# SegataLab/metamlst

Measured on AMD Instinct MI355X. Metric: Mreads/s aligned+ST-typed, metamlstDB_2022; ST concordance vs CPU ref, higher is better.
Workload: dtype int32

## Files before the change

include/mlst_debug.h:

```cpp
#ifndef MLST_DEBUG_H
#define MLST_DEBUG_H

#include "mlst.h"

#ifdef __cplusplus
extern "C" {
#endif

int mlst_selftest_inflate(const uint8_t* in, uint64_t n_in, uint8_t* out, uint64_t cap, uint64_t* produced);

int mlst_selftest_inflate_device(mlst_handle* h, const uint8_t* data, uint64_t n_bytes, uint8_t* out, uint64_t cap, uint64_t* produced, double* kernel_ms);

int mlst_debug_inflate_paths(mlst_handle* h, uint64_t* n_blocks, uint64_t* left_to_wave);

int mlst_selftest_bgzf_crc(mlst_handle* h, const uint8_t* data, uint64_t n_bytes, uint32_t* crc_out, uint64_t cap, uint64_t* n_blocks, double* kernel_ms);

int mlst_selftest_inflate_canon(const uint8_t* in, uint64_t n_in, uint8_t* out, uint64_t cap, uint64_t* produced, int* left_to_other_kernel);

int mlst_debug_bgzf_walk(const uint8_t* data, uint64_t n_bytes, uint64_t* n_blocks, uint64_t* text_bytes, int* lists_taken);

int mlst_get_route_trace(mlst_handle* h, uint64_t* out, uint64_t cap_words, uint64_t* n_words);
int mlst_debug_route_realloc(mlst_handle* h, uint64_t pad_bytes);

int mlst_debug_route_probe(mlst_handle* h, uint64_t* ring_full, uint32_t* cand, uint64_t cap, uint64_t* n_cand);

int mlst_debug_bam_split(mlst_handle* h, uint32_t force_miss_every, uint64_t* cells_rewalked_out);

int mlst_debug_last_packed(mlst_handle* h, uint32_t* packed, uint64_t cap_words, uint8_t* qrows, uint64_t cap_q, uint16_t* lens, uint64_t cap_reads,
                           uint64_t out[3] );

int mlst_debug_fasta_info(mlst_handle* h, uint64_t out[4]);

#ifdef __cplusplus
}
#endif
#endif
```

metamlst_amd/csrc/mlst_engine.hip:

```cpp
#include <hip/hip_runtime.h>
#include <algorithm>
#include <cmath>
#include <cstdarg>
#include <cstdio>
#include <cstdlib>
#include <cstring>
#include <cstddef>
#include <functional>
#include <atomic>
#include <memory>
#include <mutex>
#include <string>
#include <thread>
#include <vector>
#include <chrono>
#include <unistd.h>

#include "mlst.h"
#include "mlst_debug.h"
#include "bgzf_host.h"
#include "inflate_dev.h"
#include "inflate_wave.h"
#include "inflate_lane.h"
#include "inflate_canon.h"
// ... 1874 lines not shown
            auto rb = E.ret_bases.g() + (u64)ret_k * RW; auto rq = E.ret_quals.g() + (u64)ret_k * RQ;
            qmid[k] = k < n_live ? (u32)rq[n_k >> 1] : 0u;
            #pragma unroll
            for (int t = 0; t < KT; t++) {
                const int i = lane + 64 * t, sp = (k < n_live && i < n_k) ? (strand_k ? n_k - 1 - i : i) : 0;
                qv[k][t] = rq[sp]; bw[k][t] = rb[sp >> 4];
            }
        }
        const int kk = lane >> 4, tt = lane & 15;
        const int diag_g = __shfl(it.diag, kk); const u32 pbl_g = __shfl(L.pblocks, kk), hoff_g = __shfl(L.hblk_off, kk), hok_g = __shfl(L.hap_ok, kk);
        u32 hbv = 0;
        if (kk < n_live && tt <= X::NBA && hok_g) { int q = (diag_g >> 5) + tt; q = q < 0 ? 0 : (q > (int)pbl_g ? (int)pbl_g : q); hbv = E.hap_blk[hoff_g + (u32)q]; }
        #pragma unroll
        for (int k = 0; k < B; k++) { tie_all<KT>(qv[k]); tie_all<KT>(bw[k]); }
        tie_all<B>(qmid); TIE1(hbv);
        int pen_def_k[B];
        #pragma unroll
        for (int k = 0; k < B; k++) {
            const int n_k = __shfl(n_l, k); const int strand_k = __shfl((int)it.strand, k);
            const u8 pd = (qmid[k] >> 7) ? (u8)P.n_penalty : s_pentab[qmid[k] & 0x7Fu];
            pen_def_k[k] = (int)pd;
            #pragma unroll
            for (int t = 0; t < KT; t++) {
                const int i = lane + 64 * t; u32 b = 0, isn = 0, odd = 0;
                if (k < n_live && i < n_k) {
                    const int sp = strand_k ? n_k - 1 - i : i;
                    b = (bw[k][t] >> (2 * (sp & 15))) & 3u; if (strand_k) b ^= 3u;
                    isn = qv[k][t] >> 7;
                    const u8 pen = isn ? (u8)P.n_penalty : s_pentab[qv[k][t] & 0x7Fu];
                    odd = pen != pd;
                }
                const u64 bl = __ballot(b & 1u), bh = __ballot(b >> 1), bn = __ballot(isn != 0), bo = __ballot(odd != 0);
                if (lane == 0) {
                    s_pl[wv][k][0][2 * t] = (u32)bl; s_pl[wv][k][0][2 * t + 1] = (u32)(bl >> 32); s_pl[wv][k][1][2 * t] = (u32)bh; s_pl[wv][k][1][2 * t + 1] = (u32)(bh >> 32);
                    s_pl[wv][k][2][2 * t] = (u32)bn; s_pl[wv][k][2][2 * t + 1] = (u32)(bn >> 32); s_pl[wv][k][3][2 * t] = (u32)bo; s_pl[wv][k][3][2 * t + 1] = (u32)(bo >> 32);
                }
            }
        }
        u32 any = 0;
        const int n_g = __shfl(n_l, kk);
        if (kk < n_live) {
            u32* w = s_w[wv][kk];
            const u32 rs = 32u - ((u32)diag_g & 31u);
            if (tt <= X::NBA) w[X::HB + tt] = hbv;
            if (tt <= NB) {
                auto sh = [&](const u32* A) { const u64 v2 = ((u64)(tt < NB ? A[tt] : 0u) << 32) | (u64)(tt > 0 ? A[tt - 1] : 0u); return (u32)(v2 >> rs); };
                auto vw = [&](int j) { const int c = n_g - 32 * j; return (j < 0 || j >= NB) ? 0u : (c >= 32 ? 0xFFFFFFFFu : (c > 0 ? ((1u << c) - 1u) : 0u)); };
                const u32 rn_t = sh(s_pl[wv][kk][2]), od_t = sh(s_pl[wv][kk][3]);
                w[X::PL + 4 * tt] = sh(s_pl[wv][kk][0]); w[X::PL + 4 * tt + 1] = sh(s_pl[wv][kk][1]); w[X::PL + 4 * tt + 2] = rn_t; w[X::PL + 4 * tt + 3] = od_t;
                w[X::VR + tt] = (u32)((((u64)vw(tt) << 32) | (u64)vw(tt - 1)) >> rs);
                any = rn_t | od_t;
            }
        }
        #pragma unroll
        for (int o = 8; o > 0; o >>= 1) any |= __shfl_xor(any, o);
        const u32 special_l = __shfl(any, lane * 16);
        if (mine) {
            u32* w = s_w[wv][lane];
            if (!L.hap_ok) { for (int j = 0; j < 32; j++) w[j] = 0; }
            else {
                const bool res_ok = it.res_off + L.n_pad <= E.cap_res;
                w[0] = ((st & IS_SINGLE) ? XF_SINGLE : 0u) | (res_ok ? XF_RESOK : 0u) | XF_HAPOK | ((lw & 0x8000u) ? XF_READN : 0u)
                     | ((special_l || L.has_n) ? XF_SPECIAL : 0u) | (it.strand ? XF_STRAND : 0u);
                int pd = pen_def_k[0];
                #pragma unroll
                for (int k = 1; k < B; k++) pd = lane == k ? pen_def_k[k] : pd;
                w[1] = (u32)n_l | ((u32)pd << 16); w[2] = (u32)it.diag; w[3] = it.ret; w[4] = it.locus; w[5] = (u32)it.res_off; w[6] = (u32)(it.res_off >> 32);
                w[7] = L.a_begin; w[8] = L.n_alleles; w[9] = L.n_pad; w[10] = L.hap_off; w[11] = (u32)L.hid_off; w[12] = (u32)(L.hid_off >> 32);
                w[13] = (u32)floor_l; w[14] = L.pblocks; w[15] = L.hap_win[NB > 5 ? 1 : 0];
            }
            w[31] = (u32)(i0 + lane);
        }
        #pragma unroll
        for (int k = 0; k < B; k++) {
            if (k >= n_live) break;
            u32* dst = xrec + (i0 + k - begin) * X::WORDS;
            for (int j = lane; j < X::WORDS; j += 64) dst[j] = s_w[wv][k][j];
        }
    }
}

__device__ inline int4 hap_summary(const KParams& P, const HapRec h, u32 rl, u32 rh, u32 rn, u32 od, u32 vr, const u8* s_pen, int pen_base,
                                   int pen_def, bool special_any) {
    const int MA = P.match_bonus << MLST_P_SHIFT, negMA = -MA;
    const u32 lm = h.len >= 32u ? 0xFFFFFFFFu : ((1u << h.len) - 1u);
    const u32 valid = vr & lm;
    u32 M = ((h.lo ^ rl) | (h.hi ^ rh) | rn | h.nm) & valid;
    const int lo_c = __ffs((int)valid) - 1, hi_c = lo_c + __popc(valid);
    int gu = mad24(lo_c, negMA, 0), gf = NEGP, Pm = NEGP, B = NEGP;
    const int PDM = (pen_def << MLST_P_SHIFT) + 1 + MA, floorv = P0 - MA;
    if (special_any) {
        const u32 special = od | h.nm;
        while (M) {
            const int bit = __ffs((int)M) - 1; M &= M - 1;
            const int tu = mad24(bit, MA, gu), tf = mad24(bit, MA, gf);
            Pm = tu > Pm ? tu : Pm; B = tf > B ? tf : B;
            int dm = PDM;
            if ((special >> bit) & 1u) dm = ((((h.nm >> bit) & 1u) ? P.n_penalty : (int)s_pen[pen_base + bit]) << MLST_P_SHIFT) + 1 + MA;
            gu -= dm;
            int x = tf - dm; x = x > floorv ? x : floorv;
            gf = mad24(bit, negMA, x);
        }
    } else {
        while (M) {
            const int bit = __ffs((int)M) - 1; M &= M - 1;
            const int tu = mad24(bit, MA, gu), tf = mad24(bit, MA, gf);
            Pm = tu > Pm ? tu : Pm; B = tf > B ? tf : B;
            gu -= PDM;
            int x = tf - PDM; x = x > floorv ? x : floorv;
            gf = mad24(bit, negMA, x);
        }
    }
    return make_int4(mad24(hi_c, MA, gu), mad24(hi_c, MA, gf), Pm, B);
}

#ifdef MLST_EXT_TRACE
__device__ u32 g_ext_skip;
#define XSKIP(b) (xskip_ & (b))
extern "C" int mlst_debug_ext_skip(uint32_t v) { return hipMemcpyToSymbol(HIP_SYMBOL(g_ext_skip), &v, 4) == hipSuccess ? 0 : -1; }
__device__ u64 g_ext_trace[8];
__device__ u64 g_ext_cnt[8];
extern "C" int mlst_debug_ext_cnt(uint64_t out[8], int reset) {
    if (hipMemcpyFromSymbol(out, HIP_SYMBOL(g_ext_cnt), 64) != hipSuccess) return -1;
    if (reset) { u64 z[8] = {0, 0, 0, 0, 0, 0, 0, 0}; if (hipMemcpyToSymbol(HIP_SYMBOL(g_ext_cnt), z, 64) != hipSuccess) return -1; }
    return 0;
}
#define XC(k, v) do { if ((threadIdx.x & 63) == 0) atomicAdd(&g_ext_cnt[k], (u64)(v)); } while (0)
#if MLST_EXT_TRACE > 1
#define XT_DECL u64 xt_[6] = {0, 0, 0, 0, 0, 0}; u64 xt_items = 0; u64 xt_t = __builtin_readcyclecounter(); const u32 xskip_ = __builtin_amdgcn_readfirstlane(g_ext_skip)
#define XT(k) do { const u64 now_ = __builtin_readcyclecounter(); xt_[k] += now_ - xt_t; xt_t = now_; } while (0)
#define XT_ITEM xt_items++
#define XT_FLUSH do { if ((threadIdx.x & 63) == 0) { for (int k_ = 0; k_ < 6; k_++) atomicAdd(&g_ext_trace[k_], xt_[k_]); atomicAdd(&g_ext_trace[6], xt_items); atomicAdd(&g_ext_trace[7], 1ull); } } while (0)
#else
#define XT_DECL const u32 xskip_ = __builtin_amdgcn_readfirstlane(g_ext_skip)
#define XT(k)
#define XT_ITEM
#define XT_FLUSH
#endif
extern "C" int mlst_debug_ext_trace(uint64_t out[8], int reset) {
    if (hipMemcpyFromSymbol(out, HIP_SYMBOL(g_ext_trace), 64) != hipSuccess) return -1;
    if (reset) { u64 z[8] = {0, 0, 0, 0, 0, 0, 0, 0}; if (hipMemcpyToSymbol(HIP_SYMBOL(g_ext_trace), z, 64) != hipSuccess) return -1; }
    return 0;
}
#else
#define XC(k, v)
#define XSKIP(b) false
#define XT_DECL
#define XT(k)
#define XT_ITEM
#define XT_FLUSH
#endif
#define R_TRACK 0x10000000u

template <int NB>
__device__ __forceinline__ void extend_body(const EngineDev* __restrict__ Ep, const KParams& P, const u32 lds_recs, const u32 acc_cap, const u32* __restrict__ xrec, const u64 cap_xrec) {
    typedef XRec<NB> X;
    const EngineDev& E = *Ep;
    extern __shared__ int4 s_hap[];
    __shared__ u32 s_rl[RW / 2 + 2]; __shared__ u32 s_rh[RW / 2 + 2]; __shared__ u32 s_rn[RW / 2 + 2]; __shared__ u32 s_odd[RW / 2 + 2];
    __shared__ u8 s_pen[RQ]; __shared__ u8 s_pentab[128];
    __shared__ u32 s_cnt[16][3];
    __shared__ __attribute__((aligned(16))) u32 s_x[2][X::WORDS];
    __shared__ u64 s_ii[2];
    const int tid = threadIdx.x, nthr = blockDim.x, nwv = blockDim.x >> 6;
    for (int i = tid; i < 128; i += nthr) s_pentab[i] = E.pen_tab[i];
    u64 c_tot = 0, c_ign = 0;
    u64 N;
    { const u64 b0 = E.ctr->items_done, e0 = E.ctr->n_items < E.cap_items ? E.ctr->n_items : E.cap_items; N = e0 - b0; if (N > cap_xrec) N = cap_xrec; }
    const u64 QB = (N + EXT_Q - 1) / EXT_Q;
    u32 myq = blockIdx.x % EXT_Q, tried = 0;
    auto place = [&](u32 q, u64 ticket) -> u64 { const u64 pl = (u64)q * QB + ticket; return (ticket < QB && pl < N) ? pl : N; };
    auto resolve = [&](u64 ticket) -> u64 {
        u64 nx = place(myq, ticket);
        while (nx >= N && ++tried < EXT_Q) {
            myq = (myq + 1) % EXT_Q;
            const u64 seen = __hip_atomic_load((u64*)&E.ctr->ext_q[myq][0], __ATOMIC_RELAXED, __HIP_MEMORY_SCOPE_AGENT);
            nx = place(myq, seen) < N ? place(myq, atomicAdd(&E.ctr->ext_q[myq][0], 1ull)) : N;
        }
        if (nx < N) tried = 0;
        return nx;
    };
    if (tid == 0) {
        s_ii[0] = resolve(atomicAdd(&E.ctr->ext_q[myq][0], 1ull));
        s_ii[1] = tried < EXT_Q ? resolve(atomicAdd(&E.ctr->ext_q[myq][0], 1ull)) : N;
    }
    u16* const s_pend = reinterpret_cast<u16*>(s_hap + lds_recs + 1);
    const bool packed_acc = E.cap_items < (1ull << 24);
    __syncthreads();
    u64 pp = uniform_u64(s_ii[0]);
    if (pp < N) for (int j = tid; j < X::WORDS; j += nthr) s_x[0][j] = xrec[pp * X::WORDS + j];
    __syncthreads();
    int cur = 0;
    XT_DECL;
    while (pp < N) {
        XT_ITEM;
        const u64 pp_next = uniform_u64(s_ii[cur ^ 1]);
        u32 pf[(X::WORDS + 63) / 64];
        #pragma unroll
        for (int k = 0; k < (X::WORDS + 63) / 64; k++) { pf[k] = 0; if (pp_next < N && tid + 64 * k < X::WORDS && tid < 64) pf[k] = xrec[pp_next * X::WORDS + tid + 64 * k]; }
        u64 ticket = 0;
        if (tid == 0 && tried < EXT_Q) ticket = atomicAdd(&E.ctr->ext_q[myq][0], 1ull);
        asm volatile("" ::: "memory");
        const u32* x = s_x[cur];
        const uint4 h0 = *reinterpret_cast<const uint4*>(x), h1 = *reinterpret_cast<const uint4*>(x + 4), h2 = *reinterpret_cast<const uint4*>(x + 8), h3 = *reinterpret_cast<const uint4*>(x + 12);
        const u32 flags = __builtin_amdgcn_readfirstlane(h0.x);
        const u64 ii = (u64)(u32)__builtin_amdgcn_readfirstlane(x[31]);
        const int n = __builtin_amdgcn_readfirstlane(h0.y & 0xFFFFu), pen_def = __builtin_amdgcn_readfirstlane(h0.y >> 16);
        const int diag = __builtin_amdgcn_readfirstlane((int)h0.z);
        const u32 ret = __builtin_amdgcn_readfirstlane(h0.w);
        const u64 res_off = ((u64)(u32)__builtin_amdgcn_readfirstlane(h1.z) << 32) | (u32)__builtin_amdgcn_readfirstlane(h1.y);
        const u32 a_begin = __builtin_amdgcn_readfirstlane(h1.w), n_alleles = __builtin_amdgcn_readfirstlane(h2.x), n_pad = __builtin_amdgcn_readfirstlane(h2.y);
        const int floor_n = __builtin_amdgcn_readfirstlane((int)h3.y);
        const bool res_ok = flags & XF_RESOK, read_has_n = flags & XF_READN;
        const bool use_hap = res_ok && (flags & XF_HAPOK) && (u32)__builtin_amdgcn_readfirstlane(h3.w) <= lds_recs;
        u32 nrec = 0, ndp = 0, ntrack = 0;
        bool parked = false;
        auto park = [&]() {
            #pragma unroll
            for (int k = 0; k < (X::WORDS + 63) / 64; k++) if (tid < 64 && tid + 64 * k < X::WORDS) s_x[cur ^ 1][tid + 64 * k] = pf[k];
            if (tid == 0) s_ii[cur] = tried < EXT_Q ? resolve(ticket) : N;
            parked = true;
        };
        auto emit_pair = [&](const u32 a, const int score, const int xm, const int xo, bool need_dp, const bool valid) {
            u32 r = pack_result(score, xm, xo);
            need_dp = need_dp && valid;
            const bool is_rec = valid && !need_dp && score >= floor_n && score > 0;
            if (need_dp) r |= R_NEEDDP; else if (is_rec) r |= R_REC;
            nrec += (u32)__popcll(__ballot(is_rec));
            const u64 wm = __ballot(need_dp);
            if (wm) {
                ndp += (u32)__popcll(wm);
                int lane = tid & 63, leader = __ffsll((long long)wm) - 1; u64 base = 0;
                if (lane == leader) base = atomicAdd(&E.ctr->n_dp, (u64)__popcll(wm));
                base = __shfl(base, leader);
                if (need_dp) { u64 slot = base + __popcll(wm & ((1ull << lane) - 1));
                               if (slot < E.cap_dp) E.dp_list[slot] = (ii << 20) | (u64)a; else atomicOr(&E.ctr->err, 8ull); }
            }
            if (valid) E.res[res_off + a] = r;
        };
        auto stage_old = [&]() {
            ItemDev it; it.res_off = res_off; it.ret = ret; it.locus = __builtin_amdgcn_readfirstlane(h1.x); it.diag = diag; it.strand = (flags & XF_STRAND) ? 1 : 0; it.votes = 0;
            __syncthreads();
            stage_read_planes(E, P, it, n, s_rl, s_rh, s_rn, s_odd, s_pen, s_pentab, tid, nthr);
            __syncthreads();
        };
        auto pairs_loop = [&](const bool only_marked) {
            const LocusDev L = E.loci[__builtin_amdgcn_readfirstlane(h1.x)];
            u32 rl[NB], rh[NB], od[NB], rn[NB];
            #pragma unroll
            for (int w = 0; w < NB; w++) {
                rl[w] = __builtin_amdgcn_readfirstlane(s_rl[w]); rh[w] = __builtin_amdgcn_readfirstlane(s_rh[w]);
                od[w] = __builtin_amdgcn_readfirstlane(s_odd[w]);
                rn[w] = read_has_n ? __builtin_amdgcn_readfirstlane(s_rn[w]) : 0u;
            }
            for (u32 a = tid; a < n_alleles; a += nthr) {
                const bool valid = !only_marked || (E.res[res_off + a] & R_TRACK);
                int m = (int)E.allele_len[a_begin + a];
                int mm = 0, bs = 0, be = 0, best = P0;
                if (valid) best = L.has_n ? ungapped_planes<NB, false, true>(E, P, L, a, m, n, diag, rl, rh, od, rn, s_pen, pen_def, read_has_n, mm, bs, be)
                                         : ungapped_planes<NB, false, false>(E, P, L, a, m, n, diag, rl, rh, od, rn, s_pen, pen_def, read_has_n, mm, bs, be);
                const int score = best >> MLST_P_SHIFT, xm = 255 - (best & 0xFF), xo = 127 - ((best >> 8) & 0x7F);
                bool need_dp = P.trig < 0;
                if (valid && !need_dp && mm > P.trig && score >= floor_n) {
                    if (L.has_n) ungapped_planes<NB, true, true>(E, P, L, a, m, n, diag, rl, rh, od, rn, s_pen, pen_def, read_has_n, mm, bs, be);
                    else ungapped_planes<NB, true, false>(E, P, L, a, m, n, diag, rl, rh, od, rn, s_pen, pen_def, read_has_n, mm, bs, be);
                    need_dp = gap_trigger(P, mm, xm, score, floor_n, m, n, diag, bs, be);
                }
                emit_pair(a, score, xm, xo, need_dp, valid);
            }
        };
        XT(0);
        bool done_fast = false;
        if (use_hap) {
            const int q0 = diag >> 5;
            const u32 pblocks = __builtin_amdgcn_readfirstlane(h3.z);
            const u64 hid_off = ((u64)(u32)__builtin_amdgcn_readfirstlane(h3.x) << 32) | (u32)__builtin_amdgcn_readfirstlane(h2.w);
            constexpr int NR = (NB + 3) / 2;
            GP<const u32>::G* idrow[NR];
            #pragma unroll
            for (int j = 0; j < NR; j++) { int r = (q0 >> 1) + j; const int nrows = (int)((pblocks + 1) >> 1); r = r < 0 ? 0 : (r >= nrows ? nrows - 1 : r); idrow[j] = E.hap_id.g() + hid_off + (u64)(u32)r * n_pad; }
            const u32 odd16 = ((u32)q0 & 1u) * 16u;
            auto load_ids = [&](const u32 a, u32 (&w)[NR]) {
                const u32 ac = a < n_alleles ? a : n_alleles - 1;
                if (XSKIP(8u)) { for (int j = 0; j < NR; j++) w[j] = 0; return; }
                #pragma unroll
                for (int j = 0; j < NR; j++) w[j] = ld_row(idrow[j], ac * 4u);
            };
            u32 hb[NB + 2];
            #pragma unroll
            for (int t = 0; t <= NB + 1; t++) hb[t] = __builtin_amdgcn_readfirstlane(x[X::HB + t]);
            auto recs = E.hap_rec.g() + __builtin_amdgcn_readfirstlane(h2.z);
            u32 maxcnt = 0;
            #pragma unroll
            for (int t = 0; t <= NB; t++) { const u32 c = hb[t + 1] - hb[t]; maxcnt = c > maxcnt ? c : maxcnt; }
            const bool special_any = flags & XF_SPECIAL;
            if (special_any) {
                auto rq = E.ret_quals.g() + (u64)ret * RQ;
                for (int i = tid; i < n; i += nthr) { const u8 qb = rq[(flags & XF_STRAND) ? n - 1 - i : i]; s_pen[i] = (qb >> 7) ? (u8)P.n_penalty : s_pentab[qb & 0x7F]; }
            }
            u32 Wn[NR], Wn2[NR], Wn3[NR], Wn4[NR];
            load_ids((u32)tid, Wn); load_ids((u32)tid + nthr, Wn2); load_ids((u32)tid + 2 * nthr, Wn3); load_ids((u32)tid + 3 * nthr, Wn4);
            const u32 ident = hb[NB + 1] - hb[0];
            u32 sbase[NB + 1], wid[NB + 1];
            #pragma unroll
            for (int t = 0; t <= NB; t++) { const bool present = hb[t + 1] != hb[t]; sbase[t] = present ? hb[t] - hb[0] : ident; wid[t] = present ? 16u : 0u; }
            if (tid == 0) s_hap[ident] = make_int4(0, NEGP, NEGP, NEGP);
            if (special_any) lds_barrier();
            XT(1);
            for (u32 hb0 = 0; hb0 < maxcnt && !XSKIP(1u); hb0 += nthr) {
                const u32 hh = hb0 + tid;
                uint4 rc[NB + 1];
                #pragma unroll
                for (int t = 0; t <= NB; t++) {
                    rc[t] = make_uint4(0, 0, 0, 0);
                    if (hh < hb[t + 1] - hb[t]) rc[t] = *reinterpret_cast<GP<const uint4>::G*>(recs + hb[t] + hh);
                }
                #pragma unroll
                for (int t = 0; t <= NB; t++) { TIE4(rc[t].x, rc[t].y, rc[t].z, rc[t].w); }
                #pragma unroll
                for (int t = 0; t <= NB; t++) {
                    if (hh < hb[t + 1] - hb[t]) {
                        const uint4 sp = *reinterpret_cast<const uint4*>(x + X::PL + 4 * t); HapRec hr; hr.lo = rc[t].x; hr.hi = rc[t].y; hr.nm = rc[t].z; hr.len = rc[t].w;
                        s_hap[(hb[t] - hb[0]) + hh] = hap_summary(P, hr, sp.x, sp.y, sp.z, sp.w, x[X::VR + t], s_pen, 32 * t - (int)((u32)diag & 31u), pen_def, special_any);
                    }
                }
            }
            park();
            lds_barrier();
            XT(2);
            auto compose = [&](const u32 (&w)[NR], int& best, int& mm) {
                u32 wp[NB / 2 + 1];
                #pragma unroll
                for (int k = 0; k <= NB / 2; k++) wp[k] = __builtin_amdgcn_alignbit(k + 1 < NR ? w[k + 1 < NR ? k + 1 : 0] : 0u, w[k], odd16);
                int4 S[NB + 1];
                #pragma unroll
                for (int t = 0; t <= NB; t++) S[t] = s_hap[sbase[t] + __builtin_amdgcn_ubfe(wp[t >> 1], 16u * (t & 1), wid[t])];
                int v = P0, ts = 0; best = P0;
                #pragma unroll
                for (int t = 0; t <= NB; t++) {
                    const int c1 = v + S[t].z; best = c1 > best ? c1 : best; best = S[t].w > best ? S[t].w : best;
                    const int c2 = v + S[t].x; v = c2 > S[t].y ? c2 : S[t].y; ts += S[t].x;
                }
                best = v > best ? v : best;
                mm = (-ts) & 0xFFFF;
            };
            auto span_needs_dp = [&](const u32 (&w)[NR], const int mm, const int xm, const int score) -> bool {
                const int MA = P.match_bonus << MLST_P_SHIFT, PD = (pen_def << MLST_P_SHIFT) + 1;
                int cur = P0, best = P0, cs = 0, last = 0, blen = 0, overlap = 0, i1 = 0; bool first = true;
                #pragma unroll
                for (int t = 0; t <= NB; t++) {
                    if (hb[t + 1] == hb[t]) continue;
                    const u32 k = (u32)t + (odd16 >> 4);
                    const u32 id = (w[k >> 1] >> (16u * (k & 1u))) & 0xFFFFu;
                    const uint4 rc = *reinterpret_cast<GP<const uint4>::G*>(recs + hb[t] + id);
                    const uint4 sp = *reinterpret_cast<const uint4*>(x + X::PL + 4 * t);
                    const u32 lm = rc.w >= 32u ? 0xFFFFFFFFu : ((1u << rc.w) - 1u), valid = x[X::VR + t] & lm;
                    if (!valid) continue;
                    u32 M = ((rc.x ^ sp.x) | (rc.y ^ sp.y) | sp.z | rc.z) & valid;
                    const int lo_c = __ffs((int)valid) - 1, nv = __popc(valid);
                    if (first) { cs = last = 32 * t + lo_c; first = false; }
                    overlap += nv; i1 = 32 * t + lo_c + nv;
                    const u32 special = sp.w | rc.z;
                    while (M) {
                        const int bit = __ffs((int)M) - 1; M &= M - 1;
                        const int i = 32 * t + bit;
                        cur += (i - last) * MA;
                        if (cur > best) { best = cur; blen = i - cs; }
                        int dec = PD;
                        if ((special >> bit) & 1u) dec = ((((rc.z >> bit) & 1u) ? P.n_penalty : (int)s_pen[32 * t - (int)((u32)diag & 31u) + bit]) << MLST_P_SHIFT) + 1;
                        cur -= dec;
                        if (cur <= P0) { cur = P0; cs = i + 1; }
                        last = i + 1;
                    }
                }
                cur += (i1 - last) * MA;
                if (cur > best) blen = i1 - cs;
                const int clipped = overlap - blen;
                return mm > P.trig && score >= floor_n && clipped >= P.clip && 2 * (mm - xm) >= clipped;
            };
            const bool single = (flags & XF_SINGLE) != 0;
            bool slow = P.trig < 0 || n_alleles > acc_cap;
            if (!slow) {
                u16* const s_acc = s_pend;
                const bool n_ok = n >= P.min_read_len;
                u32 nacc = 0;
                for (u32 a = tid; a < n_alleles && !XSKIP(2u); a += nthr) {
                    u32 W[NR];
                    #pragma unroll
                    for (int j = 0; j < NR; j++) { W[j] = Wn[j]; Wn[j] = Wn2[j]; Wn2[j] = Wn3[j]; Wn3[j] = Wn4[j]; }
                    load_ids(a + 4 * nthr, Wn4);
                    asm volatile("" ::: "memory");
                    int best, mm; compose(W, best, mm);
                    const int score = best >> MLST_P_SHIFT, xm = 255 - (best & 0xFF);
                    const bool cand = score >= floor_n && score > 0;
                    bool track = cand && mm > P.trig;
                    if (track) track = span_needs_dp(W, mm, xm, score);
                    const bool rec = cand && !track, ok = rec && n_ok && score >= P.minscore && xm <= P.max_xm;
                    nrec += (u32)__popcll(__ballot(rec)); nacc += (u32)__popcll(__ballot(ok)); ntrack += (u32)__popcll(__ballot(track));
                    s_acc[a] = ok ? (u16)score : (u16)0;
                }
                u32 tot_rec = __builtin_amdgcn_readfirstlane(nrec), tot_acc = __builtin_amdgcn_readfirstlane(nacc), tot_track = __builtin_amdgcn_readfirstlane(ntrack);
                if (nwv > 1) {
                    if ((tid & 63) == 0) { s_cnt[tid >> 6][0] = tot_rec; s_cnt[tid >> 6][1] = tot_acc; s_cnt[tid >> 6][2] = tot_track; }
                    __syncthreads();
                    tot_rec = tot_acc = tot_track = 0;
                    for (int w = 0; w < nwv; w++) { tot_rec += s_cnt[w][0]; tot_acc += s_cnt[w][1]; tot_track += s_cnt[w][2]; }
                    __syncthreads();
                }
                if (tot_track == 0 && !(P.quirk && tot_rec == 1)) {
                    if (tot_acc) for (u32 a = tid; a < n_alleles; a += nthr) {
                        const u32 sc = s_acc[a];
                        if (sc && !XSKIP(4u)) {
                            if (packed_acc) atomicAdd(&E.acc64[a_begin + a], (1ull << 40) | (u64)sc);
                            else { atomicAdd((u64*)&E.sum_score[a_begin + a], (u64)sc); atomicAdd(&E.n_hits[a_begin + a], 1u); }
                        }
                    }
                    if (tid == 0) {
                        if (tot_rec) atomicAdd(&E.ret_nrec[ret], tot_rec);
                        c_tot += tot_rec; c_ign += tot_rec - tot_acc;
                        E.item_state[ii] = (u8)((single ? IS_SINGLE : 0) | IS_DONE | (tot_acc ? IS_ACC : 0));
                    }
                    done_fast = true;
                } else { slow = true; nrec = 0; ntrack = 0; }
            }
            if (slow) {
                load_ids((u32)tid, Wn);
                for (u32 a = tid; a < n_alleles; a += nthr) {
                    u32 W[NR];
                    #pragma unroll
                    for (int j = 0; j < NR; j++) W[j] = Wn[j];
                    load_ids(a + nthr, Wn);
                    asm volatile("" ::: "memory");
                    int best, mm; compose(W, best, mm);
                    const int score = best >> MLST_P_SHIFT, xm = 255 - (best & 0xFF), xo = 127 - ((best >> 8) & 0x7F);
                    const bool track = P.trig >= 0 && mm > P.trig && score >= floor_n;
                    const u64 tm = __ballot(track);
                    if (tm) { ntrack += (u32)__popcll(tm); if (track) E.res[res_off + a] = R_TRACK; }
                    emit_pair(a, score, xm, xo, P.trig < 0, !track);
                }
                ntrack = __builtin_amdgcn_readfirstlane(ntrack);
                if (nwv > 1) {
                    if ((tid & 63) == 0) s_cnt[tid >> 6][2] = ntrack;
                    __syncthreads();
                    ntrack = 0; for (int w = 0; w < nwv; w++) ntrack += s_cnt[w][2];
                }
                if (ntrack) { stage_old(); pairs_loop(true); }
            }
        }
        XT(3);
        if (!done_fast && use_hap) {
        if ((tid & 63) == 0) { s_cnt[tid >> 6][0] = nrec; s_cnt[tid >> 6][1] = ndp; }
        __syncthreads();
        u32 tot_rec = 0, tot_dp = 0;
        for (int w = 0; w < nwv; w++) { tot_rec += s_cnt[w][0]; tot_dp += s_cnt[w][1]; }
        if (tid == 0 && tot_rec) atomicAdd(&E.ret_nrec[ret], tot_rec);
        if (res_ok && tot_dp == 0 && ((flags & XF_SINGLE) || !P.quirk || tot_rec != 1)) {
            bool use_xo = P.quirk && tot_rec == 1;
            u32 acc = 0, ign = 0;
            for (u32 a = tid; a < n_alleles; a += nthr) {
                u32 r = E.res[res_off + a];
                const bool rec = r & R_REC, ok = rec && accept_rec(P, r, n, use_xo);
                if (ok) {
                    if (packed_acc) atomicAdd(&E.acc64[a_begin + a], (1ull << 40) | (u64)(r & 0x3FF));
                    else { atomicAdd((u64*)&E.sum_score[a_begin + a], (u64)(r & 0x3FF)); atomicAdd(&E.n_hits[a_begin + a], 1u); }
                }
                acc += (u32)__popcll(__ballot(ok)); ign += (u32)__popcll(__ballot(rec && !ok));
            }
            __syncthreads();
            if ((tid & 63) == 0) { s_cnt[tid >> 6][0] = acc; s_cnt[tid >> 6][1] = ign; }
            __syncthreads();
            if (tid == 0) {
                u32 A = 0, I = 0;
                for (int w = 0; w < nwv; w++) { A += s_cnt[w][0]; I += s_cnt[w][1]; }
                c_tot += tot_rec; c_ign += I;
                const u8 state = (u8)((flags & XF_SINGLE) ? IS_SINGLE : 0);
                E.item_state[ii] = (u8)(state | IS_DONE | (A ? IS_ACC : 0));
            }
        }
        }
        XT(4);
        if (!parked) park();
        lds_barrier();
        pp = pp_next; cur ^= 1;
        XT(5);
    }
    XT_FLUSH;
    if (tid == 0) {
        if (c_tot) atomicAdd(&E.ctr->cnt[MLST_CNT_TOTAL_RECORDS], c_tot);
        if (c_ign) atomicAdd(&E.ctr->cnt[MLST_CNT_IGNORED], c_ign);
    }
}

__global__ __launch_bounds__(1024) void k_extend_160(const EngineDev* __restrict__ Ep, KParams P, u32 lds_recs, u32 acc_cap, const u32* __restrict__ xrec, u64 cap_xrec) { extend_body<5>(Ep, P, lds_recs, acc_cap, xrec, cap_xrec); }
__global__ __launch_bounds__(512) void k_extend_320(const EngineDev* __restrict__ Ep, KParams P, u32 lds_recs, u32 acc_cap, const u32* __restrict__ xrec, u64 cap_xrec) { extend_body<RW / 2>(Ep, P, lds_recs, acc_cap, xrec, cap_xrec); }

template <int CTRL, int ROW_MASK = 0xF> __device__ inline int dpp_i32(int old, int src) {
    return __builtin_amdgcn_update_dpp(old, src, CTRL, ROW_MASK, 0xF, false);
}
__device__ inline int seg32_prefix_max(int v) {
    int t;
    t = dpp_i32<DPP_ROW_SHR(1)>(NEGP, v); v = t > v ? t : v;
    t = dpp_i32<DPP_ROW_SHR(2)>(NEGP, v); v = t > v ? t : v;
    t = dpp_i32<DPP_ROW_SHR(4)>(NEGP, v); v = t > v ? t : v;
    t = dpp_i32<DPP_ROW_SHR(8)>(NEGP, v); v = t > v ? t : v;
    t = dpp_i32<DPP_ROW_BCAST15, 0xA>(NEGP, v); v = t > v ? t : v;
    return v;
}

template <bool TRACE>
__device__ inline int banded(const EngineDev& E, const KParams& P, const ItemDev& it, const LocusDev& L, u32 a_local,
                             int n, const u8* s_pentab, u8* TB, int& bi, int& bb) {
    const int W = P.band_w, BW = 2 * W + 1, G = P.gbar, d = it.diag;
    const int m = (int)E.allele_len[L.a_begin + a_local];
    const int OPEN = P.open_p, EXT = P.ext_p, MA = P.match_bonus << MLST_P_SHIFT;
    auto rb = E.ret_bases.g() + (u64)it.ret * RW;
    auto rq = E.ret_quals.g() + (u64)it.ret * RQ;
    int Hp[2 * MAX_W + 2], Fp[2 * MAX_W + 2];
    #pragma unroll
    for (int b = 0; b < 2 * MAX_W + 2; b++) { Hp[b] = P0; Fp[b] = NEGP; }
    int best = P0; bi = -1; bb = -1;
    int jb = d - W;
    int q = jb >> 4;
    u32 w0 = arena_word(E, L, q, a_local), w1 = arena_word(E, L, q + 1, a_local), w2 = arena_word(E, L, q + 2, a_local);
    u8 qb_next = rq[it.strand ? n - 1 : 0];
    u32 rword = 0; int rword_idx = -1;
    for (int i = 0; i < n; i++, jb++) {
        int s = it.strand ? n - 1 - i : i;
        u8 qb = qb_next;
        if (i + 1 < n) qb_next = rq[it.strand ? n - 2 - i : i + 1];
        if ((s >> 4) != rword_idx) { rword_idx = s >> 4; rword = rb[rword_idx]; }
        bool rn = (qb & 0x80) != 0;
        u32 rbase = (rword >> (2 * (s & 15))) & 3u; if (it.strand) rbase ^= 3u;
        int pen = rn ? P.n_penalty : (int)s_pentab[qb & 0x7F];
        bool gap_ok = (i >= G && i < n - G);
        if ((jb >> 4) != q) { q++; w0 = w1; w1 = w2; w2 = arena_word(E, L, q + 2, a_local); }
        int sh = 2 * (jb - 16 * q);
        u64 lo64 = (u64)w0 | ((u64)w1 << 32);
        u64 rowbits = sh ? ((lo64 >> sh) | ((u64)w2 << (64 - sh))) : lo64;
        int Hleft = P0, Eleft = NEGP;
        #pragma unroll
        for (int b = 0; b < 2 * MAX_W + 1; b++) {
            if (b < BW) {
                int j = jb + b;
                bool exists = (j >= 0 && j < m);
                u32 ab = (u32)(rowbits >> (2 * b)) & 3u;
                bool an = L.has_n && exists && allele_is_n(E, L, j, a_local);
                int delta = (!rn && !an && rbase == ab) ? MA : -(((rn || an) ? P.n_penalty : pen) << MLST_P_SHIFT) - 1;
                int diag = Hp[b] + delta;
                int e = NEGP, f = NEGP; u8 tb = 0;
                if (gap_ok && b > 0) { int e1 = Hleft - OPEN, e2 = Eleft - EXT; if (e2 > e1) { e = e2; tb |= 4; } else e = e1; }
                if (gap_ok && b < BW - 1) { int f1 = Hp[b + 1] - OPEN, f2 = Fp[b + 1] - EXT; if (f2 > f1) { f = f2; tb |= 8; } else f = f1; }
                int h = P0; u8 src = 0;
                if (diag > h) { h = diag; src = 1; }
                if (e > h) { h = e; src = 2; }
                if (f > h) { h = f; src = 3; }
                if (!exists) { h = P0; e = NEGP; f = NEGP; src = 0; tb = 0; }
                if (TRACE) TB[i * (2 * MAX_W + 1) + b] = tb | src;
                if (h > best) { best = h; bi = i; bb = b; }
                Hp[b] = h; Fp[b] = f; Hleft = h; Eleft = e;
            }
        }
    }
    return best;
}

__global__ __launch_bounds__(256) void k_banded(const EngineDev* __restrict__ Ep, KParams P) {
    const EngineDev& E = *Ep;
    __shared__ u8 s_pentab[128];
    __shared__ u16 s_info[8][RQ];
    __shared__ u32 s_aw[8][32];
    if (threadIdx.x < 128) s_pentab[threadIdx.x] = E.pen_tab[threadIdx.x];
    __syncthreads();
    const int b = threadIdx.x & 31, gl = threadIdx.x >> 5;
    const u64 grp = ((u64)blockIdx.x * blockDim.x + threadIdx.x) >> 5, ngrp = ((u64)gridDim.x * blockDim.x) >> 5;
    const u64 begin = E.ctr->dp_done, end = E.ctr->n_dp < E.cap_dp ? E.ctr->n_dp : E.cap_dp;
    const int W = P.band_w, BW = 2 * W + 1, G = P.gbar;
    const int OPEN = P.open_p, EXT = P.ext_p, MA = P.match_bonus << MLST_P_SHIFT;
    const u64 n_iter = (end - begin + ngrp - 1) / ngrp;
    for (u64 itx = 0; itx < n_iter; itx++) {
        u64 k = begin + itx * ngrp + grp;
        bool live = k < end;
        u64 e = live ? E.dp_list[k] : 0; u64 ii = e >> 20; u32 a_local = (u32)(e & 0xFFFFFu);
        ItemDev it; it.res_off = 0; it.ret = 0; it.locus = 0; it.diag = 0; it.strand = 0; it.votes = 0;
        if (live) it = E.items[ii];
        const LocusDev L = E.loci[it.locus];
        int n = live ? (int)(E.ret_len[it.ret] & 0x7FFFu) : 0;
        int nmax = n; { int o = __shfl_xor(nmax, 32); nmax = o > nmax ? o : nmax; }
        const int d = it.diag;
        const int m = live ? (int)E.allele_len[L.a_begin + a_local] : 0;
        __syncthreads();
        {
            auto gq = E.ret_quals.g() + (u64)it.ret * RQ;
            auto gb = E.ret_bases.g() + (u64)it.ret * RW;
            for (int i = b; i < n; i += 32) {
                int s = it.strand ? n - 1 - i : i;
                u8 qb = gq[s]; u32 isn = qb >> 7;
                u32 rbase = (gb[s >> 4] >> (2 * (s & 15))) & 3u; if (it.strand) rbase ^= 3u;
                u32 pen = isn ? (u32)P.n_penalty : (u32)s_pentab[qb & 0x7F];
                s_info[gl][i] = (u16)(pen | (isn << 8) | (rbase << 9));
            }
            s_aw[gl][b] = arena_word(E, L, ((d - W) >> 4) + b, a_local);
        }
        __syncthreads();
        int Hp = P0, Fp = NEGP, best = P0;
        int jb = d - W, q = jb >> 4;
        const int q0 = q;
        u32 w0 = s_aw[gl][0], w1 = s_aw[gl][1], w2 = s_aw[gl][2], w3 = s_aw[gl][3];
        u32 info_next = n > 0 ? (u32)s_info[gl][0] : 0u;
        for (int i = 0; i < nmax; i++, jb++) {
            bool row = i < n;
            u32 info = info_next;
            if (i + 1 < n) info_next = s_info[gl][i + 1];
            bool rn = (info >> 8) & 1u;
            u32 rbase = (info >> 9) & 3u;
            int pen = (int)(info & 0xFFu);
            bool gap_ok = row && (i >= G && i < n - G);
            if (row && (jb >> 4) != q) { q++; w0 = w1; w1 = w2; w2 = w3; w3 = s_aw[gl][(q + 3 - q0) & 31]; }
            int sh = 2 * (jb - 16 * q);
            u64 lo64 = (u64)w0 | ((u64)w1 << 32);
            u64 rowbits = sh ? ((lo64 >> sh) | ((u64)w2 << (64 - sh))) : lo64;
            int j = jb + b;
            bool exists = row && b < BW && j >= 0 && j < m;
            u32 ab = (u32)(rowbits >> (2 * b)) & 3u;
            bool an = L.has_n && exists && allele_is_n(E, L, j, a_local);
            int delta = (!rn && !an && rbase == ab) ? MA : -(((rn || an) ? P.n_penalty : pen) << MLST_P_SHIFT) - 1;
            int diag = Hp + delta;
            int Hup = dpp_i32<DPP_WAVE_SHL1>(Hp, Hp), Fup = dpp_i32<DPP_WAVE_SHL1>(Fp, Fp);
            int f = NEGP;
            if (gap_ok && b < BW - 1) { int f1 = Hup - OPEN, f2 = Fup - EXT; f = f2 > f1 ? f2 : f1; }
            int h1 = P0; if (diag > h1) h1 = diag; if (f > h1) h1 = f;
            if (!exists) { h1 = P0; f = NEGP; }
            int g = h1 + EXT * b;
            int x = dpp_i32<DPP_WAVE_SHR1>(NEGP, g); if (b < 1) x = NEGP;
            x = seg32_prefix_max(x);
            int ee = (gap_ok && b > 0) ? x - OPEN - EXT * (b - 1) : NEGP;
            int h = h1; if (ee > h) h = ee;
            if (!exists) h = P0;
            if (row) { if (h > best) best = h; Hp = h; Fp = f; }
        }
        #pragma unroll
        for (int o = 16; o > 0; o >>= 1) { int y = __shfl_xor(best, o, 32); best = y > best ? y : best; }
        if (live && b == 0) {
            int score = best >> MLST_P_SHIFT, xm = 255 - (best & 0xFF), xo = 127 - ((best >> 8) & 0x7F);
            u32 r = pack_result(score, xm, xo) | R_USEDDP;
            if (score >= E.floor_tab[n] && score > 0) { r |= R_REC; atomicAdd(&E.ret_nrec[it.ret], 1u); }
            E.res[it.res_off + a_local] = r;
        }
// ... 462 lines not shown
        const u64 s0 = seq_off[k], sn = seq_off[k + 1] - s0;
        long long r = rec_pos[k]; u64 q = 0;
        for (u64 c = cig_off[k]; c < cig_off[k + 1]; c++) {
            const u32 ln = cig[c] >> 4, op = cig[c] & 15u;
            if (op == 0 || op == 7 || op == 8) {
                for (u32 t = 0; t < ln && q + t < sn; t++) {
                    const u8 ch = seq[s0 + q + t] & 0xDF;
                    const int b = ch == 'A' ? 0 : ch == 'C' ? 1 : ch == 'G' ? 2 : ch == 'T' ? 3 : -1;
                    const long long col = r + t;
                    if (b >= 0 && (int)qual[s0 + q + t] >= minqual && col >= 0 && col < alen)
                        atomicAdd(&counts[((u64)base + (u64)col) * 4 + b], 1u);
                }
                r += ln; q += ln;
            } else if (op == 1 || op == 4) q += ln;
            else if (op == 2 || op == 3) r += ln;
        }
    }
}

__host__ __device__ inline long long round_tenths(long long p, u32 q) {
    const long long p10 = 10 * p, qq = (long long)q;
    long long m = p10 / qq; if ((p10 % qq) < 0) m -= 1;
    const long long rem = p10 - m * qq;
    if (2 * rem < qq) return m;
    if (2 * rem > qq) return m + 1;
    const double d = (double)p / (double)q;
    const double sgn = fma(d, 20.0, -(double)(2 * m + 1));
    if (sgn > 0.0) return m + 1;
    if (sgn < 0.0) return m;
    return (m & 1) ? m + 1 : m;
}
__global__ __launch_bounds__(256) void k_choose(const EngineDev* __restrict__ Ep, const int* __restrict__ allele_no, int penalty,
                                                int* __restrict__ chosen) {
    const EngineDev& E = *Ep;
    __shared__ u32 s_max[4]; __shared__ long long s_r[4]; __shared__ int s_no[4]; __shared__ int s_a[4];
    const u32 l = blockIdx.x; const LocusDev L = E.loci[l];
    const int lane = threadIdx.x & 63, wv = threadIdx.x >> 6;
    if (l == 0 && threadIdx.x == 0) E.ctr->n_pl_dp = 0;
    u32 mx = 0;
    for (u32 k = threadIdx.x; k < L.n_alleles; k += 256) { u32 v = E.n_hits[L.a_begin + k]; mx = v > mx ? v : mx; }
    for (int o = 32; o > 0; o >>= 1) { u32 y = __shfl_xor(mx, o); mx = y > mx ? y : mx; }
    if (lane == 0) s_max[wv] = mx;
    __syncthreads();
    mx = s_max[0]; for (int k = 1; k < 4; k++) mx = s_max[k] > mx ? s_max[k] : mx;
    long long br = 0; int bno = 0x7FFFFFFF, ba = -1;
    for (u32 k = threadIdx.x; k < L.n_alleles; k += 256) {
        const u32 a = L.a_begin + k; const u32 nh = E.n_hits[a];
        if (!nh) continue;
        const long long local = E.sum_score[a] - (long long)(mx - nh) * (long long)penalty;
        const long long r = round_tenths(local, nh); const int no = allele_no[a];
        if (ba < 0 || r > br || (r == br && (no < bno || (no == bno && (int)a < ba)))) { br = r; bno = no; ba = (int)a; }
    }
    for (int o = 32; o > 0; o >>= 1) {
        long long r2 = __shfl_xor(br, o); int no2 = __shfl_xor(bno, o); int a2 = __shfl_xor(ba, o);
        if (a2 >= 0 && (ba < 0 || r2 > br || (r2 == br && (no2 < bno || (no2 == bno && a2 < ba))))) { br = r2; bno = no2; ba = a2; }
    }
    if (lane == 0) { s_r[wv] = br; s_no[wv] = bno; s_a[wv] = ba; }
    __syncthreads();
    if (threadIdx.x == 0) {
        for (int k = 1; k < 4; k++) if (s_a[k] >= 0 && (ba < 0 || s_r[k] > br || (s_r[k] == br && (s_no[k] < bno || (s_no[k] == bno && s_a[k] < ba))))) { br = s_r[k]; bno = s_no[k]; ba = s_a[k]; }
        chosen[l] = ba;
    }
}

__global__ __launch_bounds__(256) void k_hamming(const u8* __restrict__ ascii, const u64* __restrict__ aoff, u32 a_begin,
                                                 u32 n_alleles, const u8* __restrict__ query, u32 qlen, u32* __restrict__ dist) {
    extern __shared__ u8 s_q[];
    for (u32 i = threadIdx.x; i < qlen; i += blockDim.x) s_q[i] = query[i];
    __syncthreads();
    u32 a = blockIdx.x * blockDim.x + threadIdx.x;
    if (a >= n_alleles) return;
    u64 o = aoff[a_begin + a]; u32 m = (u32)(aoff[a_begin + a + 1] - o);
    u32 len = m < qlen ? m : qlen, c = 0;
    for (u32 i = 0; i < len; i++) c += (ascii[o + i] != s_q[i]);
    dist[a] = c;
}

__global__ void k_export(const EngineDev* __restrict__ Ep, long long* d_sum, long long* d_min) {
    const EngineDev& E = *Ep;
    u64 nA = E.n_alleles, nL = E.n_loci;
    u64 total = 2 * nA + nL + MLST_CNT_N;
    for (u64 i = (u64)blockIdx.x * blockDim.x + threadIdx.x; i < total + nL; i += (u64)gridDim.x * blockDim.x) {
        if (i < nA) d_sum[i] = E.sum_score[i];
        else if (i < 2 * nA) d_sum[i] = (long long)E.n_hits[i - nA];
        else if (i < 2 * nA + nL) d_sum[i] = (long long)E.locus_len[i - 2 * nA];
        else if (i < total) d_sum[i] = (long long)E.ctr->cnt[i - 2 * nA - nL];
        else { u64 l = i - total; u64 f = E.locus_first[l]; d_min[l] = f > 0x7FFFFFFFFFFFFFFFull ? 0x7FFFFFFFFFFFFFFFll : (long long)f; }
    }
}
__global__ void k_import(const EngineDev* __restrict__ Ep, const long long* d_sum, const long long* d_min) {
    const EngineDev& E = *Ep;
    u64 nA = E.n_alleles, nL = E.n_loci;
    u64 total = 2 * nA + nL + MLST_CNT_N;
    for (u64 i = (u64)blockIdx.x * blockDim.x + threadIdx.x; i < total + nL; i += (u64)gridDim.x * blockDim.x) {
        if (i < nA) E.sum_score[i] = d_sum[i];
        else if (i < 2 * nA) E.n_hits[i - nA] = (u32)d_sum[i];
        else if (i < 2 * nA + nL) E.locus_len[i - 2 * nA] = (u64)d_sum[i];
        else if (i < total) E.ctr->cnt[i - 2 * nA - nL] = (u64)d_sum[i];
        else { u64 l = i - total; long long f = d_min[l]; E.locus_first[l] = f == 0x7FFFFFFFFFFFFFFFll ? 0xFFFFFFFFFFFFFFFFull : (u64)f; }
    }
}
__global__ void k_fill_u64(u64* p, u64 n, u64 v) {
    for (u64 i = (u64)blockIdx.x * blockDim.x + threadIdx.x; i < n; i += (u64)gridDim.x * blockDim.x) p[i] = v;
}

#include "bam_dev.h"
#include "sam_dev.h"
#include "bam_reads.h"
#include "fasta_dev.h"
#include "fastq_tile.h"
#include "bam_tile.h"
#include "msa_dev.h"
#include "aln_export.h"
#include "read_names.h"
#include "aln_text.h"

struct EvPair { hipEvent_t a, b; int which; };

struct mlst_handle {
    int device = 0;
    hipStream_t stream = nullptr;
    mlst_params prm;
    KParams kp;
    std::string err;
    std::vector<LocusDev> loci;
    std::vector<u64> aoff;
    u32 n_alleles = 0, n_loci = 0;
    std::vector<u32> allele_locus;
    u32* d_arena = nullptr; u32* d_planes = nullptr; u32* d_nmask = nullptr; u16* d_allele_len = nullptr; u32* d_allele_locus = nullptr;
    LocusDev* d_loci = nullptr; uint4* d_sieve = nullptr; u32* d_bitmap = nullptr; u32* d_gbitmap = nullptr; u64* d_keys = nullptr; u32* d_vals = nullptr; u32* d_posts = nullptr;
    int* d_floor = nullptr; u8* d_pen = nullptr; u8* d_ascii = nullptr; u64* d_aoff = nullptr;
    HapRec* d_hap_rec = nullptr; u32* d_hap_blk = nullptr; u32* d_hap_id = nullptr; u64 bytes_hap = 0, n_hap_rec = 0; u32 hap_win_max[2] = {0, 0}, hap_loci = 0;
    u32 ext_lds_recs[2] = {0, 0};
    u32 ext_acc_cap = 0;
    u8* h_qc = nullptr; u8* d_qc = nullptr; u64 cap_hostq = 0, cap_qc = 0;
    u64* d_acc64 = nullptr;
    u32* d_xrec[2] = {nullptr, nullptr}; u64 cap_xrec[2] = {0, 0};
    u64 bytes_arena = 0, bytes_sieve = 0, bytes_table = 0; double bitmap_fill = 0.0;
    EngineDev E; EngineDev* d_E = nullptr;
    bool have_ref = false, have_state = false;
    u32* d_cand = nullptr; u64 cap_cand = 0;
    int sieve_kind = 0; u32 sieve_chain = 0; u64 n_keys = 0;
    u32* d_rfilter = nullptr; u32* d_rt_arena = nullptr; u64 cap_rt_arena = 0; u32* d_rt_counts = nullptr; u32* d_rt_emitted = nullptr; u64 cap_rt_emitted = 0;
    u32 rt_prod = 0, rt_cap = 0, rt_tiles_max = 0, rt_nw = 16, rt_pf = 2, rt_exam = RT_EXAM_DEFAULT, rt_wo = 1; u64 rt_slice = 0;
    u64* d_rt_parked = nullptr; u64 cap_rt_parked = 0;
    u64* d_rt_trace = nullptr; bool rt_trace_on = false; const void* rt_last_packed = nullptr;
    std::vector<void*> dbg_pads;
    u32* d_bin_flags = nullptr; u64 cap_bin_flags = 0;
    u8* d_in_bases = nullptr; u8* d_in_quals = nullptr; u64* d_in_off = nullptr; u64 cap_in_bytes = 0, cap_in_reads = 0;
    u32* d_packed = nullptr; u8* d_qrows = nullptr; u16* d_lens = nullptr; u64 cap_packed_words = 0, cap_qrow_bytes = 0, cap_lens = 0;
    u64 reads_seen = 0;
    u32 max_wpr = 0;
    int ext_threads = 64, ext_blocks = 5120;
    int extp_threads = 256, extp_blocks = 1792; u32 pair_loci = 0;
    int sieve_g_blocks = 256 * 5;
    u8* d_fq_text = nullptr;
    u32* d_fq_blk = nullptr; u64 cap_fq_blk = 0;
    u8* d_bgzf = nullptr; u64 cap_bgzf = 0; void* d_bgzf_blk = nullptr; u64 cap_bgzf_blk = 0; u8* d_fq_carry = nullptr; u64 cap_fq_carry = 0, fq_carry_len = 0;
    u64* d_fq_lines = nullptr; u64 cap_fq_lines = 0; u64* d_fq_soff = nullptr; u64* d_fq_qoff = nullptr; u64 cap_fq_reads = 0; u64* d_fq_meta = nullptr;
    int* d_locus_chosen = nullptr; u64* d_locus_colbase = nullptr; u64* d_pl_list = nullptr; u8* d_tb = nullptr;
    u32* d_itok = nullptr; u32* d_intok = nullptr; u64 cap_itok_blocks = 0; int inflate_mode = 0;
    u64 dbg_infl_blocks = 0, dbg_infl_left = 0; bool dbg_infl_known = false;
    struct BlkList { BgzfBlk* d = nullptr; BgzfBlk* h = nullptr; u64 cap = 0; };
    struct BzSlot { BlkList blk; hipEvent_t ev_copied = nullptr, ev_inflated = nullptr; u32* d_err = nullptr; u32* h_err = nullptr; };
    BzSlot bz[2]; int bz_slot = 0, bz_mode = -1; hipStream_t infl_stream = nullptr;
    bool bgzf_verify = false; struct { u32* d_out = nullptr; hipEvent_t e0 = nullptr, e1 = nullptr; } crc_hook;
    enum { BZ_SUB = 8 };
    struct BzChunk { u8* d = nullptr; u64 cap = 0; hipEvent_t ev[BZ_SUB] = {}; u64 upto[BZ_SUB] = {}; int n_ev = 0; hipEvent_t ev_used = nullptr; bool used = false; };
    BzChunk bzc[2]; int bz_chunk = 0;
    struct { bool on = false, counted = false; int slot = 0, tslot = 0, paired = 0; u64 text_bytes = 0; u32 blk_base = 0 ; } bz_pend;
    u8* d_pc[2] = {nullptr, nullptr}; u64 cap_pc[2] = {0, 0}, pc_len[2] = {0, 0}; bool pair_open = false; u64* d_pr_meta = nullptr;
    struct BzPair { bool on = false, counted = false; int slot = 0, tslot = 0; u32 nblk1 = 0; u64 base[2] = {0, 0}, head[2] = {0, 0}, text[2] = {0, 0}; } bzp;
    u32 depth_cap = 0; u64* d_capbuf = nullptr; u64 cap_capcols = 0;
    u32* d_counts = nullptr; u64 cap_counts = 0;
    int* d_allele_no = nullptr; int* d_auto_chosen = nullptr; u64* d_fixed_colbase = nullptr; std::vector<u64> fixed_colbase; u64 fixed_cols = 0;
    u32* d_auto_counts = nullptr; u8* d_auto_letters = nullptr; bool auto_pending = false;
    u8* h_tstats[2] = {nullptr, nullptr}; u8* h_tauto[2] = {nullptr, nullptr}; int t_slot = 0, t_last = 0, t_ready = -1;
    u64* d_compact_colbase = nullptr; int* d_compact_chosen = nullptr; u64* d_compact_info = nullptr; u64 off_compact_info = 0; bool compact_pending = false;
    hipStream_t copy_stream = nullptr; hipEvent_t stage_done = nullptr;
    u8* d_fq_slot[2] = {nullptr, nullptr}; u64 cap_fq_slot[2] = {0, 0}; hipEvent_t ev_packed[2] = {nullptr, nullptr}; int fq_slot = 0;
    u32* d_fq_nl[2] = {nullptr, nullptr};
    int cu_split = 1, cu_part = 0;
    hipStream_t own_stream = nullptr;
    u32* d_dist = nullptr; u8* d_query = nullptr; u64 cap_dist = 0, cap_query = 0;
    u8* d_stats = nullptr; u8* h_stats = nullptr; u64 stats_bytes = 0, stats_zero_bytes = 0;
    u64 off_sum = 0, off_len = 0, off_ctr = 0, off_hits = 0, off_first = 0;
    u8* h_pin = nullptr; u64 cap_pin = 0;
    bool profiling = false;
    bool window = false;
    struct GraphSlot { hipGraphExec_t exec = nullptr; std::vector<u64> sig; };
    GraphSlot g_submit, g_typing; bool use_graphs = true;
    std::vector<EvPair> events;
    std::vector<hipEvent_t> ev_pool;
    double k_ms[20] = {0}; u64 k_n[20] = {0};
    double wall_khz = 100000.0;
    struct BamStream* bam = nullptr;
    u32 bam_force_miss = 0; u64 bam_max_entries = 0;
    struct { u64 n_reads = 0; u32 wpr = 0, qstride = 0; } last_pack;
    struct { FaDev* d_desc = nullptr; FaMeta* d_meta = nullptr; u8* h_fa = nullptr; u8* d_flat = nullptr; u64 cap_flat = 0;
             u32* d_kind = nullptr; u64* d_cseq = nullptr; u64* d_chdr = nullptr; u64 cap_cells = 0; u64* d_cstart = nullptr; u64* d_wcnt = nullptr; u64 cap_contigs = 0;
             u64 last_cells = 0, last_contigs = 0; u32 last_passes = 0; } fa;
    struct { u32 read_len = 0, stride = 0; u64 round = 16ull << 20; u64 info[4] = {0, 0, 0, 0};
             FqtDev* d_desc = nullptr; FqtMeta* d_meta = nullptr; u8* h_fqt = nullptr; u64* d_rlen = nullptr; u64* d_wex = nullptr; u64 cap_recs = 0;
             u64* d_gsum = nullptr; u64 cap_groups = 0; u64* d_soff = nullptr; u64* d_qoff = nullptr; u64 cap_win = 0; } tile;
    struct { u64 batch_bytes = 1ull << 30; bool done = false; u32 n = 0, width = 0;
             u8* d_seq = nullptr; u64 cap_seq = 0; u64* d_off = nullptr; u64 cap_off = 0; u16* d_tab = nullptr; u64 cap_tab = 0;
             u32* d_slot = nullptr; u8* d_end = nullptr; u64 cap_end = 0; u32* d_tb = nullptr; u64 cap_tb = 0; u8* d_rows = nullptr; u64 cap_rows = 0;
             u32* h_width = nullptr; } msa;
    struct { bool done = false; u64 n_rec = 0, n_cig = 0, n_seq = 0; int* d_lc = nullptr; u64 cap_lc = 0; AxItem* d_meta = nullptr; u64* d_dp = nullptr;
             u64* d_off = nullptr; u64 cap_items = 0; u64* d_gs = nullptr; u64 cap_groups = 0; u8* d_desc = nullptr; u8* h_tot = nullptr;
             u8* d_out = nullptr; u64 cap_out = 0; AxOut out; } ax;
    struct AtState { bool open = false, ready = false, with_names = false, md = false, with_md = false; u16* d_mdw = nullptr; size_t next = 0; std::vector<AtRound> rounds; u64 round_bytes = 0, round_recs = 0, max_pairs = 0;
             u32* d_perm = nullptr; u64* d_pair_off = nullptr; u32* d_item_read = nullptr; u64* d_read_first = nullptr; u8* d_names = nullptr; u64* d_name_off = nullptr;
             AtPair* d_meta = nullptr; AtRead* d_reads = nullptr; u64* d_wex = nullptr; u64* d_gsum = nullptr; u64* d_dp = nullptr; u8* d_desc = nullptr;
             u8* d_text = nullptr; u64 cap_text = 0; u8* h_tot = nullptr; } at;
    struct { bool on = false; u64 want_bytes = 256ull << 20; RnCtr* d_ctr = nullptr; u8* d_bytes = nullptr; u64 cap_bytes = 0; u64* d_off = nullptr; u16* d_len = nullptr;
             RnSrc src = {nullptr, nullptr, 0}; } rn;
};

static std::string g_create_err;

static int fail(mlst_handle* h, int code, const char* fmt, ...) {
    char buf[512]; va_list ap; va_start(ap, fmt); vsnprintf(buf, sizeof buf, fmt, ap); va_end(ap);
    if (h) h->err = buf; else g_create_err = buf;
    return code;
}
#define HIPCHK(h, call) do { hipError_t e_ = (call); if (e_ != hipSuccess) return fail(h, MLST_E_HIP, "%s: %s", #call, hipGetErrorString(e_)); } while (0)

static int bz_flush(mlst_handle* h);
static int bzp_finish(mlst_handle* h, bool whole, uint64_t* n_reads_out);
static void bz_free(mlst_handle* h);
static int bam_flush(mlst_handle* h);
static void bam_drop(mlst_handle* h, bool release);
static bool bam_is_open(const mlst_handle* h);
static int rn_refuse(mlst_handle* h, const char* entry);
static void at_free(mlst_handle* h);
static const char* bam_kind(const mlst_handle* h);
template <typename T> static hipError_t dmalloc(T** p, u64 n) { return hipMalloc((void**)p, (n ? n : 1) * sizeof(T)); }
template <typename T> static hipError_t dmalloc(GP<T>* p, u64 n) { return hipMalloc((void**)&p->p, (n ? n : 1) * sizeof(T)); }

static hipEvent_t ev_get(mlst_handle* h) {
    if (!h->ev_pool.empty()) { hipEvent_t e = h->ev_pool.back(); h->ev_pool.pop_back(); return e; }
    hipEvent_t e; if (hipEventCreateWithFlags(&e, hipEventDisableSystemFence) != hipSuccess) hipEventCreate(&e); return e;
}
__global__ void k_nop() {}
struct Prof {
    mlst_handle* h; int which; hipEvent_t a = nullptr, b = nullptr;
    Prof(mlst_handle* h_, int w) : h(h_), which(w) {
        if (h->profiling) { a = ev_get(h); b = ev_get(h); hipLaunchKernelGGL(k_nop, dim3(1), dim3(64), 0, h->stream); hipEventRecord(a, h->stream); }
    }
    ~Prof() { if (h->profiling) { hipEventRecord(b, h->stream); h->events.push_back({a, b, which}); } }
};
static void drain_events(mlst_handle* h) {
    if (h->events.empty()) return;
    hipStreamSynchronize(h->stream);
    for (auto& e : h->events) { float ms = 0; hipEventElapsedTime(&ms, e.a, e.b); h->k_ms[e.which] += ms; h->k_n[e.which]++; h->ev_pool.push_back(e.a); h->ev_pool.push_back(e.b); }
    h->events.clear();
}

static int graph_enter(mlst_handle* h, mlst_handle::GraphSlot& g, const std::vector<u64>& sig) {
    if (!h->use_graphs || h->profiling || h->stream != h->own_stream) return 0;
    if (g.exec && g.sig == sig) return hipGraphLaunch(g.exec, h->stream) == hipSuccess ? 1 : 0;
    if (g.exec) { hipGraphExecDestroy(g.exec); g.exec = nullptr; }
    if (g.sig != sig) { g.sig = sig; return 0; }
    if (hipStreamBeginCapture(h->stream, hipStreamCaptureModeThreadLocal) != hipSuccess) { h->use_graphs = false; return 0; }
    return 2;
}
static int graph_leave(mlst_handle* h, mlst_handle::GraphSlot& g) {
    hipGraph_t graph = nullptr;
    if (hipStreamEndCapture(h->stream, &graph) != hipSuccess || !graph) { h->use_graphs = false; return fail(h, MLST_E_HIP, "hipStreamEndCapture failed"); }
    hipError_t e = hipGraphInstantiate(&g.exec, graph, nullptr, nullptr, 0);
    hipGraphDestroy(graph);
    if (e != hipSuccess) { g.exec = nullptr; h->use_graphs = false; return fail(h, MLST_E_HIP, "hipGraphInstantiate: %s", hipGetErrorString(e)); }
    HIPCHK(h, hipGraphLaunch(g.exec, h->stream));
    return MLST_OK;
}

extern "C" void mlst_default_params(mlst_params* p) {
    memset(p, 0, sizeof *p);
    p->minscore = MLST_DEF_MINSCORE; p->max_xm = MLST_DEF_MAX_XM; p->min_read_len = MLST_DEF_MIN_READ_LEN;
    p->minqual = MLST_DEF_MINQUAL; p->mincov = MLST_DEF_MINCOV; p->match_bonus = MLST_DEF_MATCH_BONUS;
    p->mm_max = MLST_DEF_MM_MAX; p->mm_min = MLST_DEF_MM_MIN; p->n_penalty = MLST_DEF_N_PENALTY;
    p->gap_open = MLST_DEF_GAP_OPEN; p->gap_ext = MLST_DEF_GAP_EXT; p->gbar = MLST_DEF_GBAR; p->band_w = MLST_DEF_BAND_W;
    p->gap_trigger_mm = MLST_DEF_GAP_TRIGGER_MM; p->xm_field_quirk = MLST_DEF_XM_FIELD_QUIRK; p->gap_trigger_clip = MLST_DEF_GAP_TRIGGER_CLIP;
    p->minscore_const = MLST_DEF_MINSCORE_CONST; p->minscore_coef = MLST_DEF_MINSCORE_COEF;
}

extern "C" const char* mlst_last_error(const mlst_handle* h) { return h ? h->err.c_str() : g_create_err.c_str(); }

extern "C" int mlst_create(int device, const mlst_params* p, mlst_handle** out) {
    if (!out) return fail(nullptr, MLST_E_INVALID, "out is NULL");
    *out = nullptr;
    int ndev = 0;
    if (hipGetDeviceCount(&ndev) != hipSuccess || ndev <= 0)
        return fail(nullptr, MLST_E_NOGPU, "no HIP device visible: this library has no CPU path");
    if (device < 0 || device >= ndev) return fail(nullptr, MLST_E_INVALID, "device %d out of range (%d devices)", device, ndev);
    mlst_params prm; if (p) prm = *p; else mlst_default_params(&prm);
    if (prm.band_w < 1 || prm.band_w > MAX_W) return fail(nullptr, MLST_E_INVALID, "band_w must be in 1..%d", MAX_W);
    if (prm.max_xm > 254 || prm.minscore > 1000) return fail(nullptr, MLST_E_INVALID, "max_xm/minscore out of range");
    if (prm.match_bonus < 1 || prm.match_bonus > 127) return fail(nullptr, MLST_E_INVALID, "match_bonus must be in 1..127");
    {
        const int pmin = std::min(prm.n_penalty, prm.mm_min), gap1 = prm.gap_open + prm.gap_ext;
        if (pmin < 0 || prm.mm_max < prm.mm_min || prm.gap_open < 0 || prm.gap_ext < 0) return fail(nullptr, MLST_E_INVALID, "penalties must not be negative, mm_max not below mm_min");
        if (prm.match_bonus * MLST_MAX_READ_LEN >= 1024)
            return fail(nullptr, MLST_E_LIMIT, "match_bonus %d: the score of a %d-base read does not fit 10 bits", prm.match_bonus, MLST_MAX_READ_LEN);
        if (prm.match_bonus > 4 * pmin)
// ... 282 lines not shown
            for (int k = 0; k < 2; k++) H->hap_win_max[k] = std::max(H->hap_win_max[k], L.hap_win[k]);
            H->hap_loci++;
            H->hap_rec.insert(H->hap_rec.end(), lhrec[l].begin(), lhrec[l].end()); H->hap_blk.insert(H->hap_blk.end(), hb.begin(), hb.end());
            H->hap_id.insert(H->hap_id.end(), lhid[l].begin(), lhid[l].end());
            std::vector<HapRec>().swap(lhrec[l]); std::vector<u32>().swap(lhid[l]);
        }
        if (H->hap_rec.empty()) H->hap_rec.push_back(HapRec{0, 0, 0, 0}); if (H->hap_blk.empty()) H->hap_blk.push_back(0); if (H->hap_id.empty()) H->hap_id.push_back(0);
    }
    for (u32 l = 0; l < n_loci; l++) if (!lnpos[l].empty()) { loci[l].has_n = 1; loci[l].nmask_off = nmask_words; nmask_words += (u64)loci[l].nwords * loci[l].n_pad; }
    std::vector<u32>& nmask = H->nmask; nmask.assign(nmask_words ? nmask_words : 1, 0);
    if (nmask.size() * 4 >= (1ull << 32)) return bad(MLST_E_LIMIT, "N-mask arena exceeds 4 GB (32-bit offsets in k_extend)");
    for (u32 l = 0; l < n_loci; l++) for (auto& ap : lnpos[l]) nmask[loci[l].nmask_off + (u64)(ap.second >> 5) * loci[l].n_pad + ap.first] |= 1u << (ap.second & 31);
    std::vector<KP> kp;
    { u64 tot = 0; for (auto& v : lkp) tot += v.size(); kp.reserve(tot); for (auto& v : lkp) { kp.insert(kp.end(), v.begin(), v.end()); std::vector<KP>().swap(v); } }
    std::sort(kp.begin(), kp.end(), [](const KP& x, const KP& y) { return x.key != y.key ? x.key < y.key : x.post < y.post; });
    std::vector<u64> ukeys; std::vector<u32> uval; std::vector<u32>& posts = H->posts;
    for (size_t i = 0; i < kp.size();) {
        size_t j = i; while (j < kp.size() && kp[j].key == kp[i].key) j++;
        size_t cnt = j - i;
        if (cnt <= MLST_MAX_POSTINGS) {
            ukeys.push_back(kp[i].key);
            if (cnt == 1) uval.push_back(0x80000000u | kp[i].post);
            else {
                if (posts.size() >= (1ull << 26)) return bad(MLST_E_LIMIT, "posting list exceeds 2^26 entries");
                uval.push_back(((u32)posts.size() << 5) | (u32)cnt);
                for (size_t t = i; t < j; t++) posts.push_back(kp[t].post);
            }
        }
        i = j;
    }
    std::vector<KP>().swap(kp);
    const u64 nk = ukeys.size(); H->n_keys = nk;
    u64 tcap = 1024; while (tcap < 2 * nk) tcap <<= 1;
    if (tcap > (1ull << 32)) return bad(MLST_E_LIMIT, "seed table too large");
    std::vector<u64>& tkeys = H->tkeys; std::vector<u32>& tvals = H->tvals; tkeys.assign(tcap, KEY_EMPTY); tvals.assign(tcap, 0);
    const u32 tmask = (u32)(tcap - 1); H->tmask = tmask;
    for (u64 i = 0; i < nk; i++) {
        u32 lo = (u32)ukeys[i], hi = (u32)(ukeys[i] >> 32);
        u32 hh = table_hash(lo, hi) & tmask;
        while (tkeys[hh] != KEY_EMPTY) hh = (hh + 1) & tmask;
        tkeys[hh] = ukeys[i]; tvals[hh] = uval[i];
    }
    u64 nb = 256; while (nb * 4 < nk) nb <<= 1;
    for (;;) {
        if (nb > (1ull << 31)) return bad(MLST_E_LIMIT, "sieve too large");
        std::vector<u16>& sv = H->sv; sv.assign(nb * 8, 0); const u32 smask = (u32)(nb - 1);
        u32 sshift_h = 32; for (u64 t = nb; t > 1; t >>= 1) sshift_h--;
        u32 longest = 0;
        for (u64 i = 0; i < nk; i++) {
            u32 lo = (u32)ukeys[i], hi = (u32)(ukeys[i] >> 32);
            u32 fp = sieve_fp(lo, hi); u32 b = sieve_bucket_hash(lo, hi) >> sshift_h;
            for (u64 step = 0; step < nb; step++) {
                u16* B = &sv[(u64)b * 8]; int k; bool done = false;
                for (k = 0; k < 8; k++) { if (B[k] == fp) { done = true; break; } if (B[k] == 0) { B[k] = (u16)fp; done = true; break; } }
                if (done) { if ((u32)step > longest) longest = (u32)step; break; }
                b = (b + 1) & smask;
            }
        }
        H->nb = nb; H->smask = smask; H->sieve_chain = longest;
        if (longest <= 32) break;
        nb <<= 1;
    }
    int kind = want_kind;
    if (kind < 0 || kind == MLST_SIEVE_LDS) {
        const u64 nbits = 1ull << BITMAP_BITS;
        if (nk <= 4 * nbits) {
            std::vector<u32>& bitmap = H->bitmap; bitmap.assign(nbits / 32, 0);
            u64 set = 0;
            for (u64 i = 0; i < nk; i++) {
                for (int o = 0; o < 2; o++) {
                    u32 L, R; sieve_halves_of(o ? revcomp40(ukeys[i]) : ukeys[i], L, R);
                    R += SV_HALF_BITS;
                    if (!((bitmap[L >> 5] >> (L & 31)) & 1u)) { bitmap[L >> 5] |= 1u << (L & 31); set++; }
                    if (!((bitmap[R >> 5] >> (R & 31)) & 1u)) { bitmap[R >> 5] |= 1u << (R & 31); set++; }
                }
            }
            H->bitmap_fill = (double)set / (double)nbits;
            if (set * 2 > nbits) { bitmap.clear(); H->bitmap_fill = 0.0; }
        }
        kind = H->bitmap.empty() ? MLST_SIEVE_ROUTED : MLST_SIEVE_LDS;
    }
    if (nk == 0) kind = H->bitmap.empty() ? MLST_SIEVE_GLOBAL : MLST_SIEVE_LDS;
    if (kind == MLST_SIEVE_GLOBAL && nk > 0) {
        const char* gsw = getenv("MLST_GBM_BITS");
        u32 gbits = gsw ? (u32)atoi(gsw) : 25u;
        if (gbits >= 16 && gbits <= 31 && nk <= (1ull << gbits)) {
            H->gbitmap.assign((1ull << gbits) / 32, 0); H->gbits = gbits;
            for (u64 i = 0; i < nk; i++) { u32 bi = bitmap_hash_bits((u32)ukeys[i], (u32)(ukeys[i] >> 32), gbits); H->gbitmap[bi >> 5] |= 1u << (bi & 31); }
        }
    }
    if (kind == MLST_SIEVE_ROUTED) {
        H->rfilter.assign((u64)RT_OWNERS * RT_FWORDS, 0u);
        for (u64 i = 0; i < nk; i++) {
            u32 ow, hh, b0, b1, k0, k1; rt_hash((u32)ukeys[i], (u32)(ukeys[i] >> 32), ow, hh); rt_filter_addr(hh, b0, k0, b1, k1);
            H->rfilter[(u64)ow * RT_FWORDS + b0] |= k0; H->rfilter[(u64)ow * RT_FWORDS + b1] |= k1;
        }
    }
    H->kind = kind;
    return H;
}

static std::mutex g_index_mu;
static std::shared_ptr<HostIndex> g_index_last; static u64 g_index_key[5] = {0, 0, 0, 0, 0};

static std::mutex g_refcache_mu; static std::string g_refcache_path;
extern "C" int mlst_set_reference_cache(const char* path) { std::lock_guard<std::mutex> lk(g_refcache_mu); g_refcache_path = path ? path : ""; return MLST_OK; }
#define REFCACHE_MAGIC 0x3146455254534C4Dull
#define REFCACHE_VERSION 3u
template <typename T> static bool rc_put(FILE* f, const std::vector<T>& v) { const u64 n = v.size(); return fwrite(&n, 8, 1, f) == 1 && (!n || fwrite(v.data(), sizeof(T), n, f) == n); }
template <typename T> static bool rc_get(FILE* f, std::vector<T>& v) {
    u64 n = 0; if (fread(&n, 8, 1, f) != 1 || n > (1ull << 36) / sizeof(T)) return false;
    v.resize(n); return !n || fread(v.data(), sizeof(T), n, f) == n;
}
struct RefCacheHead { u64 magic; u32 version, sz_locus, sz_hap, pad; u64 key[5]; u32 hap_win_max[2], hap_loci, tmask, smask, sieve_chain, gbits, n_loci; int kind; u32 pad2; u64 nb, n_keys; double bitmap_fill; };
static bool refcache_store(const std::string& path, const u64 key[5], const HostIndex& H) {
    const std::string tmp = path + "." + std::to_string((long)getpid()) + ".tmp";
    FILE* f = fopen(tmp.c_str(), "wb"); if (!f) return false;
    RefCacheHead hd; memset(&hd, 0, sizeof hd);
    hd.magic = REFCACHE_MAGIC; hd.version = REFCACHE_VERSION; hd.sz_locus = (u32)sizeof(LocusDev); hd.sz_hap = (u32)sizeof(HapRec); memcpy(hd.key, key, sizeof hd.key);
    hd.hap_win_max[0] = H.hap_win_max[0]; hd.hap_win_max[1] = H.hap_win_max[1]; hd.hap_loci = H.hap_loci; hd.tmask = H.tmask; hd.smask = H.smask; hd.sieve_chain = H.sieve_chain;
    hd.gbits = H.gbits; hd.n_loci = H.n_loci; hd.kind = H.kind; hd.nb = H.nb; hd.n_keys = H.n_keys; hd.bitmap_fill = H.bitmap_fill;
    bool ok = fwrite(&hd, sizeof hd, 1, f) == 1 && rc_put(f, H.loci) && rc_put(f, H.alen) && rc_put(f, H.arena) && rc_put(f, H.nmask) && rc_put(f, H.planes) && rc_put(f, H.hap_rec)
              && rc_put(f, H.hap_blk) && rc_put(f, H.hap_id) && rc_put(f, H.tkeys) && rc_put(f, H.tvals) && rc_put(f, H.posts) && rc_put(f, H.sv) && rc_put(f, H.bitmap)
              && rc_put(f, H.gbitmap) && rc_put(f, H.rfilter);
    ok = (fclose(f) == 0) && ok;
    if (ok) ok = rename(tmp.c_str(), path.c_str()) == 0;
    if (!ok) remove(tmp.c_str());
    return ok;
}
static std::shared_ptr<HostIndex> refcache_load(const std::string& path, const u64 key[5]) {
    FILE* f = fopen(path.c_str(), "rb"); if (!f) return nullptr;
    auto H = std::make_shared<HostIndex>();
    RefCacheHead hd;
    bool ok = fread(&hd, sizeof hd, 1, f) == 1 && hd.magic == REFCACHE_MAGIC && hd.version == REFCACHE_VERSION && hd.sz_locus == sizeof(LocusDev) && hd.sz_hap == sizeof(HapRec)
              && memcmp(hd.key, key, sizeof hd.key) == 0;
    ok = ok && rc_get(f, H->loci) && rc_get(f, H->alen) && rc_get(f, H->arena) && rc_get(f, H->nmask) && rc_get(f, H->planes) && rc_get(f, H->hap_rec) && rc_get(f, H->hap_blk)
         && rc_get(f, H->hap_id) && rc_get(f, H->tkeys) && rc_get(f, H->tvals) && rc_get(f, H->posts) && rc_get(f, H->sv) && rc_get(f, H->bitmap) && rc_get(f, H->gbitmap) && rc_get(f, H->rfilter);
    fclose(f);
    if (!ok || H->loci.size() != hd.n_loci) return nullptr;
    H->hap_win_max[0] = hd.hap_win_max[0]; H->hap_win_max[1] = hd.hap_win_max[1]; H->hap_loci = hd.hap_loci; H->tmask = hd.tmask; H->smask = hd.smask; H->sieve_chain = hd.sieve_chain;
    H->gbits = hd.gbits; H->n_loci = hd.n_loci; H->kind = hd.kind; H->nb = hd.nb; H->n_keys = hd.n_keys; H->bitmap_fill = hd.bitmap_fill;
    return H;
}

static int sieve_kind_from_env() {
    const char* s = getenv("MLST_SIEVE");
    if (!s || !s[0]) return -1;
    if (!strcmp(s, "lds")) return MLST_SIEVE_LDS;
    if (!strcmp(s, "global")) return MLST_SIEVE_GLOBAL;
    if (!strcmp(s, "routed")) return MLST_SIEVE_ROUTED;
    return -1;
}

static size_t ext_lds_bytes(const mlst_handle* h, int k) { return (size_t)(h->ext_lds_recs[k] + 1) * 16 + (size_t)h->ext_acc_cap * 2; }
extern "C" int mlst_load_reference(mlst_handle* h, const uint8_t* ascii, const uint64_t* off, const uint32_t* locus_id,
                                   const uint32_t* species_id, const int32_t* allele_no, uint32_t n_alleles) {
    if (!h || !off || !locus_id) return fail(h, MLST_E_INVALID, "NULL argument");
    hipSetDevice(h->device);
    hipStreamSynchronize(h->stream);
    free_ref(h); free_state(h);
    for (auto* g : {&h->g_submit, &h->g_typing}) { if (g->exec) { hipGraphExecDestroy(g->exec); g->exec = nullptr; } g->sig.clear(); }
    h->n_alleles = n_alleles;
    const int want_kind = sieve_kind_from_env();
    std::shared_ptr<HostIndex> HI;
    {
        u64 key[5];
        key[3] = n_alleles; key[4] = off[n_alleles];
        key[0] = fnv1a(off, ((u64)n_alleles + 1) * 8, 0xCBF29CE484222325ull ^ n_alleles);
        key[1] = fnv1a(ascii, off[n_alleles], fnv1a(locus_id, (u64)n_alleles * 4, 0x9E3779B97F4A7C15ull));
        key[2] = (u64)(want_kind + 2);
        for (const char* v : {"MLST_GBM_BITS"}) { const char* e = getenv(v); if (e) key[2] = fnv1a(e, strlen(e), key[2]); }
        if (species_id) key[2] = fnv1a(species_id, (u64)n_alleles * 4, key[2]);
        std::lock_guard<std::mutex> lk(g_index_mu);
        const char* nocache = getenv("MLST_INDEX_CACHE");
        if (nocache && nocache[0] == '0') g_index_last.reset();
        if (g_index_last && memcmp(g_index_key, key, sizeof key) == 0) HI = g_index_last;
        else {
            std::string rc_path; { std::lock_guard<std::mutex> lk2(g_refcache_mu); rc_path = g_refcache_path; }
            if (!rc_path.empty()) HI = refcache_load(rc_path, key);
            if (!HI) {
                HI = build_host_index(ascii, off, locus_id, species_id, n_alleles, want_kind);
                if (HI->err_code) return fail(h, HI->err_code, "%s", HI->err.c_str());
                if (!rc_path.empty()) refcache_store(rc_path, key, *HI);
            }
            if (!(nocache && nocache[0] == '0')) { g_index_last = HI; memcpy(g_index_key, key, sizeof key); }
        }
    }
    const u32 n_loci = HI->n_loci; h->n_loci = n_loci;
    const std::vector<LocusDev>& loci = HI->loci; const std::vector<u16>& alen = HI->alen;
    const std::vector<u32>&arena = HI->arena, &nmask = HI->nmask, &planes = HI->planes, &posts = HI->posts, &tvals = HI->tvals, &bitmap = HI->bitmap, &gbitmap = HI->gbitmap;
    const std::vector<u64>& tkeys = HI->tkeys; const std::vector<u16>& sv = HI->sv;
    const u64 tcap = tkeys.size(), nb = HI->nb; const u32 tmask = HI->tmask, smask = HI->smask, gbits = HI->gbits;
    h->allele_locus.assign(locus_id, locus_id + n_alleles);
    h->sieve_kind = HI->kind; h->sieve_chain = HI->sieve_chain; h->n_keys = HI->n_keys;
    std::vector<int> floor_tab(MLST_MAX_READ_LEN + 1);
    for (int n = 0; n <= MLST_MAX_READ_LEN; n++) {
        double f = h->prm.minscore_const + h->prm.minscore_coef * log((double)(n > 0 ? n : 1));
        long v = (long)f; if (v < 0) v = 0; floor_tab[n] = (int)v;
    }
    std::vector<u8> pen_tab(256);
    for (int q = 0; q < 256; q++) { int qq = q > 40 ? 40 : q; pen_tab[q] = (u8)(h->prm.mm_min + ((h->prm.mm_max - h->prm.mm_min) * qq) / 40); }
    HIPCHK(h, dmalloc(&h->d_arena, arena.size())); HIPCHK(h, hipMemcpy(h->d_arena, arena.data(), arena.size() * 4, hipMemcpyHostToDevice));
    HIPCHK(h, dmalloc(&h->d_planes, planes.size())); HIPCHK(h, hipMemcpy(h->d_planes, planes.data(), planes.size() * 4, hipMemcpyHostToDevice));
    HIPCHK(h, dmalloc(&h->d_nmask, nmask.size())); HIPCHK(h, hipMemcpy(h->d_nmask, nmask.data(), nmask.size() * 4, hipMemcpyHostToDevice));
    HIPCHK(h, dmalloc(&h->d_allele_len, (u64)n_alleles)); HIPCHK(h, hipMemcpy(h->d_allele_len, alen.data(), (u64)n_alleles * 2, hipMemcpyHostToDevice));
    HIPCHK(h, dmalloc(&h->d_allele_locus, (u64)n_alleles)); HIPCHK(h, hipMemcpy(h->d_allele_locus, locus_id, (u64)n_alleles * 4, hipMemcpyHostToDevice));
    HIPCHK(h, dmalloc(&h->d_loci, (u64)n_loci)); HIPCHK(h, hipMemcpy(h->d_loci, loci.data(), (u64)n_loci * sizeof(LocusDev), hipMemcpyHostToDevice));
    HIPCHK(h, dmalloc(&h->d_sieve, nb)); HIPCHK(h, hipMemcpy(h->d_sieve, sv.data(), nb * 16, hipMemcpyHostToDevice));
    if (!bitmap.empty()) { HIPCHK(h, dmalloc(&h->d_bitmap, (u64)bitmap.size())); HIPCHK(h, hipMemcpy(h->d_bitmap, bitmap.data(), bitmap.size() * 4, hipMemcpyHostToDevice)); }
    if (!HI->rfilter.empty()) { HIPCHK(h, dmalloc(&h->d_rfilter, (u64)HI->rfilter.size())); HIPCHK(h, hipMemcpy(h->d_rfilter, HI->rfilter.data(), HI->rfilter.size() * 4, hipMemcpyHostToDevice)); }
    if (!gbitmap.empty()) { HIPCHK(h, dmalloc(&h->d_gbitmap, (u64)gbitmap.size())); HIPCHK(h, hipMemcpy(h->d_gbitmap, gbitmap.data(), gbitmap.size() * 4, hipMemcpyHostToDevice)); }
    HIPCHK(h, dmalloc(&h->d_keys, tcap)); HIPCHK(h, hipMemcpy(h->d_keys, tkeys.data(), tcap * 8, hipMemcpyHostToDevice));
    HIPCHK(h, dmalloc(&h->d_vals, tcap)); HIPCHK(h, hipMemcpy(h->d_vals, tvals.data(), tcap * 4, hipMemcpyHostToDevice));
    HIPCHK(h, dmalloc(&h->d_posts, (u64)posts.size())); if (!posts.empty()) HIPCHK(h, hipMemcpy(h->d_posts, posts.data(), posts.size() * 4, hipMemcpyHostToDevice));
    HIPCHK(h, dmalloc(&h->d_floor, (u64)floor_tab.size())); HIPCHK(h, hipMemcpy(h->d_floor, floor_tab.data(), floor_tab.size() * 4, hipMemcpyHostToDevice));
    HIPCHK(h, dmalloc(&h->d_pen, (u64)256)); HIPCHK(h, hipMemcpy(h->d_pen, pen_tab.data(), 256, hipMemcpyHostToDevice));
    u64 abytes = off[n_alleles];
    HIPCHK(h, dmalloc(&h->d_ascii, abytes)); if (abytes) HIPCHK(h, hipMemcpy(h->d_ascii, ascii, abytes, hipMemcpyHostToDevice));
    HIPCHK(h, dmalloc(&h->d_aoff, (u64)n_alleles + 1)); HIPCHK(h, hipMemcpy(h->d_aoff, off, ((u64)n_alleles + 1) * 8, hipMemcpyHostToDevice));
    HIPCHK(h, dmalloc(&h->d_hap_rec, (u64)HI->hap_rec.size())); HIPCHK(h, hipMemcpy(h->d_hap_rec, HI->hap_rec.data(), HI->hap_rec.size() * sizeof(HapRec), hipMemcpyHostToDevice));
    HIPCHK(h, dmalloc(&h->d_hap_blk, (u64)HI->hap_blk.size())); HIPCHK(h, hipMemcpy(h->d_hap_blk, HI->hap_blk.data(), HI->hap_blk.size() * 4, hipMemcpyHostToDevice));
    HIPCHK(h, dmalloc(&h->d_hap_id, (u64)HI->hap_id.size())); HIPCHK(h, hipMemcpy(h->d_hap_id, HI->hap_id.data(), HI->hap_id.size() * 4, hipMemcpyHostToDevice));
    h->bytes_hap = HI->hap_rec.size() * sizeof(HapRec) + HI->hap_blk.size() * 4 + HI->hap_id.size() * 4; h->n_hap_rec = HI->hap_rec.size();
    h->hap_win_max[0] = HI->hap_win_max[0]; h->hap_win_max[1] = HI->hap_win_max[1]; h->hap_loci = HI->hap_loci;
    h->bytes_arena = arena.size() * 4 + planes.size() * 4 + nmask.size() * 4; h->bytes_sieve = nb * 16 + bitmap.size() * 4 + gbitmap.size() * 4 + HI->rfilter.size() * 4; h->bytes_table = tcap * 12 + posts.size() * 4;
    h->aoff.assign(off, off + n_alleles + 1);
    {
        HIPCHK(h, dmalloc(&h->d_allele_no, (u64)n_alleles)); HIPCHK(h, hipMemcpy(h->d_allele_no, allele_no, (u64)n_alleles * 4, hipMemcpyHostToDevice));
        h->fixed_colbase.assign(n_loci + 1, 0);
        for (u32 l = 0; l < n_loci; l++) h->fixed_colbase[l + 1] = h->fixed_colbase[l] + loci[l].max_len;
        h->fixed_cols = h->fixed_colbase[n_loci];
        HIPCHK(h, dmalloc(&h->d_fixed_colbase, (u64)n_loci + 1)); HIPCHK(h, hipMemcpy(h->d_fixed_colbase, h->fixed_colbase.data(), ((u64)n_loci + 1) * 8, hipMemcpyHostToDevice));
        HIPCHK(h, dmalloc(&h->d_auto_chosen, (u64)n_loci));
        HIPCHK(h, dmalloc(&h->d_auto_counts, h->fixed_cols * 4 + 4)); HIPCHK(h, dmalloc(&h->d_auto_letters, h->fixed_cols + 16));
        h->off_compact_info = (((u64)n_loci * 4 + 15) & ~15ull) + ((h->fixed_cols + 15) & ~15ull);
        for (int k = 0; k < 2; k++) { if (h->h_tauto[k]) hipHostFree(h->h_tauto[k]); HIPCHK(h, hipHostMalloc((void**)&h->h_tauto[k], h->off_compact_info + 64, hipHostMallocDefault)); }
        HIPCHK(h, dmalloc(&h->d_compact_colbase, (u64)n_loci + 1)); HIPCHK(h, dmalloc(&h->d_compact_chosen, (u64)n_loci + 1)); HIPCHK(h, dmalloc(&h->d_compact_info, 2));
    }
    EngineDev& E = h->E;
    E.arena = h->d_arena; E.planes = h->d_planes; E.nmask = h->d_nmask; E.allele_len = h->d_allele_len; E.allele_locus = h->d_allele_locus; E.loci = h->d_loci;
    h->bitmap_fill = HI->bitmap_fill;
    E.sieve = h->d_sieve; E.sieve_mask = smask; E.bitmap = h->d_bitmap; E.gbitmap = h->d_gbitmap; E.gbitmap_bits = gbitmap.empty() ? 0 : gbits; E.keys = h->d_keys; E.vals = h->d_vals; E.posts = h->d_posts; E.table_mask = tmask;
    E.floor_tab = h->d_floor; E.pen_tab = h->d_pen; E.n_alleles = n_alleles; E.n_loci = n_loci;
    E.hap_rec = h->d_hap_rec; E.hap_blk = h->d_hap_blk; E.hap_id = h->d_hap_id;
    E.cap_ret = h->prm.max_retained_reads; E.cap_items = h->prm.max_items; E.cap_res = h->prm.max_pair_results; E.cap_dp = h->prm.max_items * 4;
    {
        u64 o = 0;
        h->off_sum = o; o += (u64)n_alleles * 8;
        h->off_len = o; o += (u64)n_loci * 8;
        h->off_ctr = o; o += (sizeof(Counters) + 7) & ~7ull;
        h->off_hits = o; o += ((u64)n_alleles * 4 + 7) & ~7ull;
        h->stats_zero_bytes = o;
        h->off_first = o; o += (u64)n_loci * 8;
        h->stats_bytes = o ? o : 8;
        HIPCHK(h, dmalloc(&h->d_stats, h->stats_bytes));
        HIPCHK(h, hipHostMalloc((void**)&h->h_stats, h->stats_bytes, hipHostMallocDefault));
        for (int k = 0; k < 2; k++) { if (h->h_tstats[k]) hipHostFree(h->h_tstats[k]); HIPCHK(h, hipHostMalloc((void**)&h->h_tstats[k], h->stats_bytes, hipHostMallocDefault)); }
        h->t_slot = 0; h->t_ready = -1;
        E.sum_score = (long long*)(h->d_stats + h->off_sum); E.locus_len = (u64*)(h->d_stats + h->off_len);
        E.ctr = (Counters*)(h->d_stats + h->off_ctr); E.n_hits = (u32*)(h->d_stats + h->off_hits);
        E.locus_first = (u64*)(h->d_stats + h->off_first);
    }
    HIPCHK(h, dmalloc(&E.ret_bases, E.cap_ret * RW)); HIPCHK(h, dmalloc(&E.ret_quals, E.cap_ret * RQ));
    HIPCHK(h, dmalloc(&E.ret_len, E.cap_ret)); HIPCHK(h, dmalloc(&E.ret_ridx, E.cap_ret)); HIPCHK(h, dmalloc(&E.ret_nrec, E.cap_ret));
    HIPCHK(h, dmalloc(&E.ret_mate, E.cap_ret)); HIPCHK(h, dmalloc(&E.ret_item0, E.cap_ret)); HIPCHK(h, dmalloc(&E.ret_nitems, E.cap_ret)); HIPCHK(h, dmalloc(&E.ret_cpos, E.cap_ret));
    HIPCHK(h, dmalloc(&E.items, E.cap_items)); HIPCHK(h, dmalloc(&E.item_state, E.cap_items)); HIPCHK(h, dmalloc(&E.res, E.cap_res)); HIPCHK(h, dmalloc(&E.dp_list, E.cap_dp));
    HIPCHK(h, dmalloc(&h->d_locus_colbase, (u64)n_loci * 2 + 2));
    HIPCHK(h, dmalloc(&h->d_pl_list, E.cap_items));
    HIPCHK(h, dmalloc(&h->d_tb, (u64)64 * 64 * MLST_MAX_READ_LEN * (2 * MAX_W + 1)));
    HIPCHK(h, dmalloc(&h->d_acc64, (u64)n_alleles)); HIPCHK(h, hipMemset(h->d_acc64, 0, (u64)(n_alleles ? n_alleles : 1) * 8)); E.acc64 = h->d_acc64;
    HIPCHK(h, dmalloc(&h->d_E, (u64)1)); HIPCHK(h, hipMemcpy(h->d_E, &h->E, sizeof(EngineDev), hipMemcpyHostToDevice));
    {
        u32 hap_max = 512; const char* e0 = getenv("MLST_EXT_HAP_MAX"); if (e0 && atoi(e0) >= 0) hap_max = (u32)atoi(e0);
        u32 budget_kb = 96; const char* e4 = getenv("MLST_EXT_LDS_KB"); if (e4 && atoi(e4) >= 0 && atoi(e4) <= 150) budget_kb = (u32)atoi(e4);
        std::vector<LocusDev> lc = loci;
        u32 mx_hap = 0, mx_pair = 0, n_hap = 0, n_pair = 0; h->hap_win_max[0] = h->hap_win_max[1] = 0;
        for (auto& L : lc) {
            const bool take = L.hap_ok && L.n_alleles <= hap_max && (u64)L.hap_win[1] * 16 <= (u64)budget_kb * 1024;
            L.hap_ok = take ? 1u : 0u;
            if (take) { n_hap++; mx_hap = std::max(mx_hap, L.n_alleles); for (int k = 0; k < 2; k++) h->hap_win_max[k] = std::max(h->hap_win_max[k], L.hap_win[k]); }
            else { n_pair++; mx_pair = std::max(mx_pair, L.n_alleles); }
        }
        h->loci = lc; h->hap_loci = n_hap; h->pair_loci = n_pair;
        HIPCHK(h, hipMemcpy(h->d_loci, lc.data(), (u64)n_loci * sizeof(LocusDev), hipMemcpyHostToDevice));
        int thr = mx_hap <= 512 ? 64 : 256;
        const char* e1 = getenv("MLST_EXT_THREADS"); if (e1 && atoi(e1) >= 64 && atoi(e1) <= 1024 && atoi(e1) % 64 == 0) thr = atoi(e1);
        int blocks = 1280 * 256 / thr;
        const char* e2 = getenv("MLST_EXT_BLOCKS"); if (e2 && atoi(e2) > 0) blocks = atoi(e2);
        h->ext_threads = thr; h->ext_blocks = blocks;
        int thr2 = mx_pair <= 512 ? 64 : 256;
        const char* e5 = getenv("MLST_EXTP_THREADS"); if (e5 && atoi(e5) >= 64 && atoi(e5) <= 1024 && atoi(e5) % 64 == 0) thr2 = atoi(e5);
        int blocks2 = 1792 * 256 / thr2;
        const char* e6 = getenv("MLST_EXTP_BLOCKS"); if (e6 && atoi(e6) > 0) blocks2 = atoi(e6);
        h->extp_threads = thr2; h->extp_blocks = blocks2;
        h->ext_acc_cap = std::min<u32>((mx_hap + 63u) & ~63u, 16384u);
        for (int k = 0; k < 2; k++) {
            h->ext_lds_recs[k] = h->hap_win_max[k];
            if (ext_lds_bytes(h, k) > 48u * 1024u)
                HIPCHK(h, hipFuncSetAttribute(k ? (const void*)k_extend_320 : (const void*)k_extend_160, hipFuncAttributeMaxDynamicSharedMemorySize, (int)ext_lds_bytes(h, k)));
        }
        const char* e3 = getenv("MLST_SIEVE_BLOCKS"); if (e3 && atoi(e3) > 0) h->sieve_g_blocks = atoi(e3);
        const char* e7 = getenv("MLST_RT_SLICE"); h->rt_slice = (e7 && atoll(e7) > 0) ? (u64)atoll(e7) : 0;
    }
    h->have_ref = h->have_state = true;
    int rc = reset_sample_state(h); if (rc) return rc;
    HIPCHK(h, hipStreamSynchronize(h->stream));
    return MLST_OK;
}

extern "C" int mlst_set_read_index_base(mlst_handle* h, uint64_t base) {
    if (!h || !h->have_state) return fail(h, MLST_E_INVALID, "no reference loaded");
    h->reads_seen = base;
    return MLST_OK;
}

extern "C" int mlst_reset_sample(mlst_handle* h) {
    if (!h || !h->have_state) return fail(h, MLST_E_INVALID, "no reference loaded");
    hipSetDevice(h->device);
    drain_events(h);
    if (h->bz_pend.on || h->bzp.on) { if (h->infl_stream) hipStreamSynchronize(h->infl_stream); h->bz_pend.on = false; h->bzp.on = false; }
    return reset_sample_state(h);
}

static int grid_for(u64 n_units, int per_block, int cap = 2048) {
    u64 g = (n_units + per_block - 1) / per_block; if (g < 1) g = 1; if (g > (u64)cap) g = cap; return (int)g;
}
static void zero_words(mlst_handle* h, void* p, u64 n_words) {
    if (!n_words) return;
    hipLaunchKernelGGL(k_zero, dim3(grid_for((n_words + 255) / 256, 1, 1024)), dim3(256), 0, h->stream, (u32*)p, n_words);
}

extern "C" int mlst_pack_reads_device(mlst_handle* h, const uint8_t* d_bases, const uint8_t* d_quals, const uint64_t* d_off,
                                      uint64_t n_reads, uint32_t* d_packed, uint8_t* d_qrows, uint16_t* d_lens,
                                      uint32_t wpr, uint32_t qstride) {
    if (!h) return MLST_E_INVALID;
    hipSetDevice(h->device);
    if (wpr == 0 || wpr > RW || (wpr & 1)) return fail(h, MLST_E_INVALID, "words_per_read must be even and in 2..%d", RW);
    if (qstride < 4 || qstride > RQ || (qstride & 3)) return fail(h, MLST_E_INVALID, "qual_stride must be a multiple of 4 in 4..%d", RQ);
    if (((uintptr_t)d_qrows & 3) != 0) return fail(h, MLST_E_INVALID, "quality rows must be 4-byte aligned");
    if (n_reads == 0) return MLST_OK;
    Prof pf(h, 6);
    hipLaunchKernelGGL(k_pack, dim3(grid_for((n_reads + 63) / 64, 1, 8192)), dim3(256), 0, h->stream, d_bases, d_quals, (const u64*)d_off, (u64)n_reads,
                       d_packed, d_qrows, d_lens, wpr, qstride);
    HIPCHK(h, hipGetLastError());
    return MLST_OK;
}

static int ensure_route_buffers(mlst_handle* h, u64 n_reads, u32 wpr, u64 n_reads_flags = 0) {
    u32 nw = 16;
    { const char* e = getenv("MLST_ROUTE_WAVES"); if (e && atoi(e) == 8) nw = 8; }
    { const char* e = getenv("MLST_ROUTE_WRITEOUT"); h->rt_wo = (e && e[0] == '0' && e[1] == 0) ? 0u : 1u; }
    { const char* e = getenv("MLST_PROBE_PF"); h->rt_pf = (e && atoi(e) == 4) ? 4u : 2u; }
    { const char* e = getenv("MLST_PROBE_EXAM_WAVES"); const int v = e ? atoi(e) : RT_EXAM_DEFAULT; h->rt_exam = (v == 0 || v == 1 || v == 2 || v == 4) ? (u32)v : (u32)RT_EXAM_DEFAULT; }
    const u64 tile = (u64)nw * 64, n_tiles = (n_reads + tile - 1) / tile;
    u32 prod = (wpr <= 10 ? 512u : 256u) * (16u / nw) / (u32)h->cu_split;
    { const char* e = getenv("MLST_ROUTE_BLOCKS"); if (e && atoi(e) > 0) prod = (u32)atoi(e); }
    if (prod > RT_MAXP) prod = RT_MAXP;
    if (prod > n_tiles) prod = (u32)(n_tiles ? n_tiles : 1);
    u64 tiles_max = (n_tiles + prod - 1) / prod * 3 / 2 + 8;
    u64 cap = (u64)((double)tiles_max * ((double)tile / 256.0 * (wpr - 1) + 0.15 * nw + 2.0) * 1.25) + 256; cap = (cap + 31) & ~31ull;
    if (h->rt_prod == prod && h->rt_nw == nw && h->rt_cap >= cap && h->rt_tiles_max >= tiles_max) { cap = h->rt_cap; tiles_max = h->rt_tiles_max; }
    if (cap >= (1ull << 31) || tiles_max > 0xFFFFull || (u64)RT_OWNERS * prod * (cap / 16) >= (1ull << 32)) return fail(h, MLST_E_LIMIT, "batch too large for the routed sieve (%llu tiles per producer workgroup)", (unsigned long long)tiles_max);
    const u64 need = (u64)RT_OWNERS * prod * cap;
    if (h->cap_rt_arena < need || h->rt_prod != prod || h->rt_cap != (u32)cap) {
        hipStreamSynchronize(h->stream);
        if (h->cap_rt_arena < need) { hipFree(h->d_rt_arena); h->d_rt_arena = nullptr; HIPCHK(h, dmalloc(&h->d_rt_arena, need)); h->cap_rt_arena = need; }
        hipFree(h->d_rt_counts); h->d_rt_counts = nullptr; HIPCHK(h, dmalloc(&h->d_rt_counts, (u64)RT_OWNERS * prod));
        h->rt_prod = prod; h->rt_cap = (u32)cap;
    }
    const u64 need_e = (u64)prod * (tiles_max + 1);
    if (h->cap_rt_emitted < need_e) { hipStreamSynchronize(h->stream); hipFree(h->d_rt_emitted); h->d_rt_emitted = nullptr; HIPCHK(h, dmalloc(&h->d_rt_emitted, need_e)); h->cap_rt_emitted = need_e; }
    h->rt_tiles_max = (u32)tiles_max; h->rt_nw = nw;
    if (h->rt_trace_on && !h->d_rt_trace) { hipStreamSynchronize(h->stream); HIPCHK(h, dmalloc(&h->d_rt_trace, (u64)(RT_MAXP + RT_OWNERS) * 4)); HIPCHK(h, hipMemsetAsync(h->d_rt_trace, 0, (u64)(RT_MAXP + RT_OWNERS) * 32, h->stream)); }
    const u64 need_p = std::max<u64>(n_reads / 4, 1ull << 16);
    if (h->cap_rt_parked < need_p) { hipStreamSynchronize(h->stream); hipFree(h->d_rt_parked); h->d_rt_parked = nullptr; HIPCHK(h, dmalloc(&h->d_rt_parked, need_p)); h->cap_rt_parked = need_p; }
    const u64 n_flag_words = ((n_reads_flags > n_reads ? n_reads_flags : n_reads) + 31) >> 5;
    if (h->cap_bin_flags < n_flag_words) { hipStreamSynchronize(h->stream); hipFree(h->d_bin_flags); h->d_bin_flags = nullptr; HIPCHK(h, dmalloc(&h->d_bin_flags, n_flag_words)); h->cap_bin_flags = n_flag_words;
                                            HIPCHK(h, hipMemsetAsync(h->d_bin_flags, 0, n_flag_words * 4, h->stream)); }
    return MLST_OK;
}

static int submit_impl(mlst_handle* h, const uint32_t* d_packed, const uint8_t* d_qrows, const uint16_t* d_lens,
                       uint64_t n_reads, uint32_t wpr, uint32_t qstride, int paired, int phase);
extern "C" int mlst_submit_packed_device(mlst_handle* h, const uint32_t* d_packed, const uint8_t* d_qrows, const uint16_t* d_lens,
                                         uint64_t n_reads, uint32_t wpr, uint32_t qstride, int paired) {
    { int rc_ = rn_refuse(h, "mlst_submit_packed_device"); if (rc_) return rc_; }
    return submit_impl(h, d_packed, d_qrows, d_lens, n_reads, wpr, qstride, paired, 0);
}
static int submit_impl(mlst_handle* h, const uint32_t* d_packed, const uint8_t* d_qrows, const uint16_t* d_lens,
                       uint64_t n_reads, uint32_t wpr, uint32_t qstride, int paired, int phase) {
    if (!h || !h->have_state) return fail(h, MLST_E_INVALID, "no reference loaded");
    hipSetDevice(h->device);
    if (wpr == 0 || wpr > RW || (wpr & 1)) return fail(h, MLST_E_INVALID, "words_per_read must be even and in 2..%d", RW);
    if (qstride < 4 || qstride > RQ || (qstride & 3)) return fail(h, MLST_E_INVALID, "qual_stride must be a multiple of 4 in 4..%d", RQ);
    if (phase != 1 && (!d_qrows || ((uintptr_t)d_qrows & 3) != 0)) return fail(h, MLST_E_INVALID, "quality rows must be 4-byte aligned");
    if (n_reads >= (1ull << 32)) return fail(h, MLST_E_LIMIT, "a batch holds at most 2^32-1 reads");
    if (((uintptr_t)d_packed & 15) != 0) return fail(h, MLST_E_INVALID, "packed rows must be 16-byte aligned");
    if (n_reads == 0) return MLST_OK;
    paired = paired ? 1 : 0;
    if (paired && ((n_reads | h->reads_seen) & 1ull)) return fail(h, MLST_E_INVALID, "paired submissions hold whole pairs (reads 2k, 2k+1) and start at an even read index");
    if (h->cap_cand < n_reads) { hipStreamSynchronize(h->stream); hipFree(h->d_cand); h->d_cand = nullptr; HIPCHK(h, dmalloc(&h->d_cand, n_reads)); h->cap_cand = n_reads; }
    EngineDev& E = h->E;
    if (wpr > h->max_wpr) h->max_wpr = wpr;
    u64 rt_slice = 0;
    if (h->sieve_kind == MLST_SIEVE_ROUTED && h->rt_slice) { rt_slice = (h->rt_slice + 1023) & ~1023ull; if (rt_slice >= n_reads) rt_slice = 0; }
    if (h->sieve_kind == MLST_SIEVE_ROUTED) { int rc = ensure_route_buffers(h, rt_slice ? rt_slice : n_reads, wpr, n_reads); if (rc) return rc; }
    {
        const int k = wpr <= 10 ? 0 : 1; const u64 words = k ? (u64)XRec<RW / 2>::WORDS : (u64)XRec<5>::WORDS;
        if (h->hap_loci && !h->d_xrec[k]) { hipStreamSynchronize(h->stream); HIPCHK(h, dmalloc(&h->d_xrec[k], h->E.cap_items * words)); h->cap_xrec[k] = h->E.cap_items; }
    }
    const int gs = phase ? 0 : graph_enter(h, h->g_submit, {(u64)(uintptr_t)d_packed, (u64)(uintptr_t)d_qrows, (u64)(uintptr_t)d_lens, (u64)n_reads, (u64)wpr,
                                               (u64)qstride, (u64)h->reads_seen, (u64)(uintptr_t)h->d_cand,
                                               (u64)(uintptr_t)h->d_bin_flags, (u64)(uintptr_t)h->d_rt_arena, (u64)(uintptr_t)h->d_rt_counts,
                                               (u64)(uintptr_t)h->d_rt_emitted, (u64)h->rt_cap, (u64)h->rt_prod, (u64)h->rt_nw, (u64)paired, (u64)(uintptr_t)h->d_rt_trace, (u64)(uintptr_t)h->d_rt_parked, (u64)h->cap_rt_parked, (u64)h->rt_pf, rt_slice, (u64)h->rt_exam, (u64)h->rt_wo});
    if (gs == 1) { h->reads_seen += n_reads; return MLST_OK; }
    if (phase != 2) { Prof pf(h, 0);
      if (h->sieve_kind == MLST_SIEVE_LDS) {
        dim3 grid(grid_for((n_reads + 1023) / 1024, 1, 256)), block(1024);
#define SIEVE_CASE(W) case W: hipLaunchKernelGGL((k_sieve_q<W, true>), grid, block, 0, h->stream, d_packed, d_lens, (u64)n_reads, E.sieve, E.sieve_mask, E.bitmap, 0u, h->d_cand, E.ctr, paired); break;
        switch (wpr) { SIEVE_CASE(2) SIEVE_CASE(4) SIEVE_CASE(6) SIEVE_CASE(8) SIEVE_CASE(10) SIEVE_CASE(12) SIEVE_CASE(14)
                       SIEVE_CASE(16) SIEVE_CASE(18) SIEVE_CASE(20) default: return fail(h, MLST_E_INVALID, "words_per_read %u unsupported", wpr); }
#undef SIEVE_CASE
      } else if (h->sieve_kind == MLST_SIEVE_ROUTED) {
        const u64 n_flag_words = (n_reads + 31) >> 5;
        for (u64 sl_first = 0; sl_first < n_reads; sl_first += (rt_slice ? rt_slice : n_reads)) {
        const u64 sl_n = rt_slice ? std::min<u64>(rt_slice, n_reads - sl_first) : n_reads;
        const u32* sl_packed = d_packed + (sl_first >> 6) * 64 * wpr; const u16* sl_lens = d_lens + sl_first;
        if (sl_first) hipLaunchKernelGGL(k_rt_reset, dim3(1), dim3(1), 0, h->stream, E.ctr);
        RouteDev R; R.arena = h->d_rt_arena; R.counts = h->d_rt_counts; R.emitted = h->d_rt_emitted; R.filter = h->d_rfilter; R.flags = h->d_bin_flags + (sl_first >> 5); R.trace = h->d_rt_trace; R.parked = h->d_rt_parked; R.parked_cap = h->cap_rt_parked;
        h->rt_last_packed = d_packed;
        R.cap = h->rt_cap; R.n_prod = h->rt_prod; R.tiles_max = h->rt_tiles_max; R.nw = h->rt_nw;
        { const char* e = getenv("MLST_RT_DEBUG"); R.dbg = e ? (u32)atoi(e) : 0u; if (R.dbg & 2u) R.parked_cap = 0; }
        { Prof pa(h, 9);
#define ROUTE_LAUNCH(W, N, WO) hipLaunchKernelGGL((k_route<W, N, WO>), dim3(h->rt_prod), dim3(N * 64), 0, h->stream, sl_packed, sl_lens, (u64)sl_n, R, E.ctr)
#define SIEVE_CASE(W) case W: if (h->rt_nw == 8) { if (h->rt_wo) ROUTE_LAUNCH(W, 8, true); else ROUTE_LAUNCH(W, 8, false); } \
                              else { if (h->rt_wo) ROUTE_LAUNCH(W, 16, true); else ROUTE_LAUNCH(W, 16, false); } break;
        switch (wpr) { SIEVE_CASE(2) SIEVE_CASE(4) SIEVE_CASE(6) SIEVE_CASE(8) SIEVE_CASE(10) SIEVE_CASE(12) SIEVE_CASE(14)
                       SIEVE_CASE(16) SIEVE_CASE(18) SIEVE_CASE(20) default: return fail(h, MLST_E_INVALID, "words_per_read %u unsupported", wpr); }
#undef SIEVE_CASE
#undef ROUTE_LAUNCH
        }
        { Prof pb(h, 10);
#define PROBE_LAUNCH(W, PF, EX) hipLaunchKernelGGL((k_route_probe<W, PF, EX>), dim3(RT_OWNERS), dim3(1024), 0, h->stream, sl_packed, (u64)sl_n, E.sieve, E.sieve_mask, R, E.ctr)
#define SIEVE_CASE(W) case W: if (h->rt_exam == 1) PROBE_LAUNCH(W, 2, 1); else if (h->rt_exam == 2) PROBE_LAUNCH(W, 2, 2); else if (h->rt_exam == 4) PROBE_LAUNCH(W, 2, 4); \
                              else if (h->rt_pf == 4) PROBE_LAUNCH(W, 4, 0); else PROBE_LAUNCH(W, 2, 0); break;
        switch (wpr) { SIEVE_CASE(2) SIEVE_CASE(4) SIEVE_CASE(6) SIEVE_CASE(8) SIEVE_CASE(10) SIEVE_CASE(12) SIEVE_CASE(14)
                       SIEVE_CASE(16) SIEVE_CASE(18) SIEVE_CASE(20) default: return fail(h, MLST_E_INVALID, "words_per_read %u unsupported", wpr); }
#undef SIEVE_CASE
#undef PROBE_LAUNCH
        }
        { Prof pc(h, 11);
#define SIEVE_CASE(W) case W: hipLaunchKernelGGL(k_route_verify<W>, dim3(2048), dim3(256), 0, h->stream, sl_packed, (u64)sl_n, E.sieve, E.sieve_mask, R, E.ctr); break;
        switch (wpr) { SIEVE_CASE(2) SIEVE_CASE(4) SIEVE_CASE(6) SIEVE_CASE(8) SIEVE_CASE(10) SIEVE_CASE(12) SIEVE_CASE(14)
                       SIEVE_CASE(16) SIEVE_CASE(18) SIEVE_CASE(20) default: return fail(h, MLST_E_INVALID, "words_per_read %u unsupported", wpr); }
#undef SIEVE_CASE
        }
        }
        hipLaunchKernelGGL(k_flag_compact, dim3(grid_for((n_flag_words + FLAG_U - 1) / FLAG_U, 1024, 512)), dim3(1024), 0, h->stream, h->d_bin_flags, (u64)n_reads, h->d_cand, E.ctr, paired);
      } else {
        dim3 grid(grid_for((n_reads + 255) / 256, 1, h->sieve_g_blocks)), block(256);
#define SIEVE_CASE(W) case W: hipLaunchKernelGGL((k_sieve_q<W, false>), grid, block, 0, h->stream, d_packed, d_lens, (u64)n_reads, E.sieve, E.sieve_mask, E.gbitmap.p, E.gbitmap_bits, h->d_cand, E.ctr, paired); break;
        switch (wpr) { SIEVE_CASE(2) SIEVE_CASE(4) SIEVE_CASE(6) SIEVE_CASE(8) SIEVE_CASE(10) SIEVE_CASE(12) SIEVE_CASE(14)
                       SIEVE_CASE(16) SIEVE_CASE(18) SIEVE_CASE(20) default: return fail(h, MLST_E_INVALID, "words_per_read %u unsupported", wpr); }
#undef SIEVE_CASE
      }
    }
    if (phase == 1) { HIPCHK(h, hipGetLastError()); return MLST_OK; }
    { Prof pf(h, 1);
      hipLaunchKernelGGL(k_seed, dim3(1024), dim3(256), 0, h->stream, h->d_E, d_packed, d_qrows, d_lens, wpr, qstride, h->reads_seen, h->d_cand, paired, phase == 2 ? 1 : 0);
      hipLaunchKernelGGL(k_retain, dim3(2048), dim3(256), 0, h->stream, h->d_E, d_packed, d_qrows, wpr, qstride, h->reads_seen, phase == 2 ? 1 : 0); }
    if (h->hap_loci) {
      { Prof pf(h, 12);
        if (wpr <= 10) hipLaunchKernelGGL(k_ext_prep<5>, dim3(2048), dim3(256), 0, h->stream, h->d_E, h->kp, h->d_xrec[0], h->cap_xrec[0]);
        else hipLaunchKernelGGL(k_ext_prep<RW / 2>, dim3(2048), dim3(256), 0, h->stream, h->d_E, h->kp, h->d_xrec[1], h->cap_xrec[1]); }
      { Prof pf(h, 2);
        const int thr = h->ext_threads, blocks = h->ext_blocks;
        if (wpr <= 10) hipLaunchKernelGGL(k_extend_160, dim3(blocks), dim3(thr), ext_lds_bytes(h, 0), h->stream, h->d_E, h->kp, h->ext_lds_recs[0], h->ext_acc_cap, h->d_xrec[0], h->cap_xrec[0]);
        else hipLaunchKernelGGL(k_extend_320, dim3(blocks), dim3(std::min(thr, 512)), ext_lds_bytes(h, 1), h->stream, h->d_E, h->kp, h->ext_lds_recs[1], h->ext_acc_cap, h->d_xrec[1], h->cap_xrec[1]); }
    }
    if (h->pair_loci) { Prof pf(h, 2);
      const int thr = h->extp_threads, blocks = h->extp_blocks;
      if (wpr <= 10) hipLaunchKernelGGL(k_extend_pairs_160, dim3(blocks), dim3(thr), 0, h->stream, h->d_E, h->kp);
      else hipLaunchKernelGGL(k_extend_pairs_320, dim3(blocks), dim3(thr), 0, h->stream, h->d_E, h->kp); }
    { Prof pf(h, 3); hipLaunchKernelGGL(k_banded, dim3(1024), dim3(256), 0, h->stream, h->d_E, h->kp); }
    { Prof pf(h, 4); hipLaunchKernelGGL(k_accumulate, dim3(1024), dim3(256), 0, h->stream, h->d_E, h->kp);
      hipLaunchKernelGGL(k_locus, dim3(128), dim3(1024), 0, h->stream, h->d_E, paired); }
    hipLaunchKernelGGL(k_advance, dim3(1), dim3(1), 0, h->stream, E.ctr, n_reads);
    if (gs == 2) { int rc = graph_leave(h, h->g_submit); if (rc) return rc; }
    HIPCHK(h, hipGetLastError());
    h->reads_seen += n_reads;
    return MLST_OK;
}

static int ensure_pack_buffers(mlst_handle* h, u64 n_reads, u32 wpr, u32 qstride) {
    h->last_pack.n_reads = 0; h->last_pack.wpr = h->last_pack.qstride = 0;
    if (h->cap_packed_words < packed_words(n_reads, wpr) + 4 || h->cap_qrow_bytes < n_reads * qstride || h->cap_lens < n_reads + 2) {
        hipStreamSynchronize(h->stream);
        hipFree(h->d_packed); hipFree(h->d_qrows); hipFree(h->d_lens); h->d_packed = nullptr; h->d_qrows = nullptr; h->d_lens = nullptr;
        HIPCHK(h, dmalloc(&h->d_packed, packed_words(n_reads, wpr) + 4)); HIPCHK(h, dmalloc(&h->d_qrows, n_reads * qstride)); HIPCHK(h, dmalloc(&h->d_lens, n_reads + 2));
        h->cap_packed_words = packed_words(n_reads, wpr) + 4; h->cap_qrow_bytes = n_reads * qstride; h->cap_lens = n_reads + 2;
    }
    return MLST_OK;
}

static int h2d_overlapped(mlst_handle* h, void* d_dst, const void* src, u64 n, hipEvent_t before) {
    if (n == 0) return MLST_OK;
    if (!h->copy_stream) HIPCHK(h, hipStreamCreateWithFlags(&h->copy_stream, hipStreamNonBlocking));
    if (!h->stage_done) HIPCHK(h, hipEventCreateWithFlags(&h->stage_done, hipEventDisableTiming));
    if (before) HIPCHK(h, hipStreamWaitEvent(h->copy_stream, before, 0));
    HIPCHK(h, hipMemcpyAsync(d_dst, src, n, hipMemcpyHostToDevice, h->copy_stream));
    HIPCHK(h, hipEventRecord(h->stage_done, h->copy_stream));
    HIPCHK(h, hipStreamWaitEvent(h->stream, h->stage_done, 0));
    HIPCHK(h, hipStreamSynchronize(h->copy_stream));
    return MLST_OK;
}

extern "C" int mlst_submit_reads_device(mlst_handle* h, const uint8_t* d_bases, const uint8_t* d_quals, const uint64_t* d_off,
                                        uint64_t n_reads, uint32_t max_len, int paired) {
    if (!h || !h->have_state) return fail(h, MLST_E_INVALID, "no reference loaded");
    { int rc_ = rn_refuse(h, "mlst_submit_reads_device"); if (rc_) return rc_; }
    if (bam_is_open(h)) return fail(h, MLST_E_INVALID, "a %s stream is open (its last chunk was not marked final)", bam_kind(h));
    { int rc_ = bz_flush(h); if (rc_) return rc_; }
    hipSetDevice(h->device);
    if (n_reads == 0) return MLST_OK;
    if (max_len > MLST_MAX_READ_LEN) return fail(h, MLST_E_LIMIT, "read longer than %d bases", MLST_MAX_READ_LEN);
    u32 wpr = (max_len + 15) / 16; if (wpr < 2) wpr = 2; wpr = (wpr + 1) & ~1u;
    u32 qstride = (max_len + 7) & ~7u; if (qstride < 8) qstride = 8;
    int rc = ensure_pack_buffers(h, n_reads, wpr, qstride); if (rc) return rc;
    rc = mlst_pack_reads_device(h, d_bases, d_quals, d_off, n_reads, h->d_packed, h->d_qrows, h->d_lens, wpr, qstride); if (rc) return rc;
    return mlst_submit_packed_device(h, h->d_packed, h->d_qrows, h->d_lens, n_reads, wpr, qstride, paired);
}

extern "C" int mlst_submit_reads(mlst_handle* h, const uint8_t* bases, const uint8_t* quals, const uint64_t* off,
                                 uint64_t n_reads, int paired) {
    if (!h || !h->have_state) return fail(h, MLST_E_INVALID, "no reference loaded");
    { int rc_ = rn_refuse(h, "mlst_submit_reads"); if (rc_) return rc_; }
    if (bam_is_open(h)) return fail(h, MLST_E_INVALID, "a %s stream is open (its last chunk was not marked final)", bam_kind(h));
    { int rc_ = bz_flush(h); if (rc_) return rc_; }
    if (n_reads == 0) return MLST_OK;
    if (!bases || !quals || !off) return fail(h, MLST_E_INVALID, "NULL argument");
    hipSetDevice(h->device);
    u64 nbytes = off[n_reads] - off[0]; u32 max_len = 0;
    for (u64 r = 0; r < n_reads; r++) { u64 l = off[r + 1] - off[r]; if (l > MLST_MAX_READ_LEN) return fail(h, MLST_E_LIMIT, "read %llu longer than %d bases", (unsigned long long)r, MLST_MAX_READ_LEN); max_len = std::max(max_len, (u32)l); }
    if (h->cap_in_bytes < nbytes || h->cap_in_reads < n_reads + 1) {
        hipStreamSynchronize(h->stream);
        hipFree(h->d_in_bases); hipFree(h->d_in_quals); hipFree(h->d_in_off); h->d_in_bases = h->d_in_quals = nullptr; h->d_in_off = nullptr;
        HIPCHK(h, dmalloc(&h->d_in_bases, nbytes)); HIPCHK(h, dmalloc(&h->d_in_quals, nbytes)); HIPCHK(h, dmalloc(&h->d_in_off, n_reads + 1));
        h->cap_in_bytes = nbytes; h->cap_in_reads = n_reads + 1;
    }
    hipStreamSynchronize(h->stream);
    std::vector<u64> rel(n_reads + 1); for (u64 r = 0; r <= n_reads; r++) rel[r] = off[r] - off[0];
    HIPCHK(h, hipMemcpyAsync(h->d_in_bases, bases + off[0], nbytes, hipMemcpyHostToDevice, h->stream));
    HIPCHK(h, hipMemcpyAsync(h->d_in_quals, quals + off[0], nbytes, hipMemcpyHostToDevice, h->stream));
    HIPCHK(h, hipMemcpyAsync(h->d_in_off, rel.data(), (n_reads + 1) * 8, hipMemcpyHostToDevice, h->stream));
    HIPCHK(h, hipStreamSynchronize(h->stream));
    return mlst_submit_reads_device(h, h->d_in_bases, h->d_in_quals, (const uint64_t*)h->d_in_off, n_reads, max_len, paired);
}

static int next_text_slot(mlst_handle* h, u64 bytes) {
    const int slot = h->fq_slot ^= 1;
    if (!h->ev_packed[slot]) HIPCHK(h, hipEventCreateWithFlags(&h->ev_packed[slot], hipEventDisableTiming));
    if (h->cap_fq_slot[slot] < bytes) {
        HIPCHK(h, hipEventSynchronize(h->ev_packed[slot]));
        hipFree(h->d_fq_slot[slot]); h->d_fq_slot[slot] = nullptr; HIPCHK(h, dmalloc(&h->d_fq_slot[slot], bytes + 16)); h->cap_fq_slot[slot] = bytes;
        hipFree(h->d_fq_nl[slot]); h->d_fq_nl[slot] = nullptr; HIPCHK(h, dmalloc(&h->d_fq_nl[slot], bytes / 4096 + 8));
    }
    h->d_fq_text = h->d_fq_slot[slot];
    return MLST_OK;
}

static int fq_pack_submit(mlst_handle* h, u64 n_reads, u32 max_len, int tslot, int paired, uint64_t* n_reads_out);
static int rn_ensure(mlst_handle* h) {
    auto& N = h->rn;
    if (N.d_ctr) return MLST_OK;
    HIPCHK(h, dmalloc(&N.d_ctr, (u64)1)); HIPCHK(h, dmalloc(&N.d_bytes, N.want_bytes)); N.cap_bytes = N.want_bytes;
    HIPCHK(h, dmalloc(&N.d_off, h->E.cap_ret)); HIPCHK(h, dmalloc(&N.d_len, h->E.cap_ret));
    HIPCHK(h, hipMemsetAsync(N.d_ctr, 0, sizeof(RnCtr), h->stream));
    return MLST_OK;
}
static int rn_refuse(mlst_handle* h, const char* entry) {
    if (h && h->rn.on) return fail(h, MLST_E_INVALID, "%s: read names are on (mlst_set_read_names) and only the FASTQ text and BGZF entries carry names", entry);
    return MLST_OK;
}
static int rn_fetch(mlst_handle* h, RnCtr* c) {
    memset(c, 0, sizeof *c);
    if (!h->rn.d_ctr) return MLST_OK;
    HIPCHK(h, hipMemcpyAsync(c, h->rn.d_ctr, sizeof *c, hipMemcpyDeviceToHost, h->stream));
    HIPCHK(h, hipStreamSynchronize(h->stream));
    if (c->err) return fail(h, MLST_E_LIMIT, "the read names need %llu bytes and the arena holds %llu: raise MLST_NAMES_BYTES", (unsigned long long)c->bytes, (unsigned long long)h->rn.cap_bytes);
    return MLST_OK;
}
static int fq_tile_submit(mlst_handle* h, u64 n_bytes, u64 n_lines, u64 n_recs, int tslot, uint64_t* n_reads_out);
static int fastq_pipeline(mlst_handle* h, u64 n_bytes, int paired, bool whole, uint64_t* n_reads_out, u64 pair_boundary = 0, int tslot = -1, u64 skip = 0,
                          u32* ext_blk = nullptr, u64 count_bytes = 0) {
    if (tslot < 0) tslot = h->fq_slot;
    const u64 n_blocks = (n_bytes + FQ_BLOCK - 1) / FQ_BLOCK;
    if (!ext_blk && h->cap_fq_blk < n_blocks) { hipFree(h->d_fq_blk); h->d_fq_blk = nullptr; HIPCHK(h, dmalloc(&h->d_fq_blk, n_blocks + 1)); h->cap_fq_blk = n_blocks; }
    u32* const blk = ext_blk ? ext_blk : h->d_fq_blk;
    HIPCHK(h, hipMemsetAsync(h->d_fq_meta, 0, 16, h->stream));
    Prof pf(h, 6);
    if (!ext_blk) hipLaunchKernelGGL(k_fq_count, dim3((u32)n_blocks), dim3(256), 0, h->stream, h->d_fq_text, (u64)n_bytes, blk);
    else if (count_bytes) hipLaunchKernelGGL(k_fq_count, dim3((u32)(count_bytes / FQ_BLOCK)), dim3(256), 0, h->stream, h->d_fq_text, (u64)count_bytes, blk);
    hipLaunchKernelGGL(k_fq_scan, dim3(1), dim3(1024), 0, h->stream, blk, (u32)n_blocks, h->d_fq_meta, (u64)n_bytes, h->d_fq_text, whole ? 1 : 0);
    u64 n_lines = 0;
    HIPCHK(h, hipMemcpyAsync(&n_lines, h->d_fq_meta, 8, hipMemcpyDeviceToHost, h->stream));
    HIPCHK(h, hipStreamSynchronize(h->stream));
    if (n_lines >= (1ull << 32)) return fail(h, MLST_E_LIMIT, "more than 2^32 lines in one FASTQ chunk");
    if (whole && n_lines % 4 != 0) return fail(h, MLST_E_INVALID, "FASTQ chunk holds %llu lines: not a whole number of 4-line records", (unsigned long long)n_lines);
    const u64 n_reads = n_lines / 4;
    if (h->cap_fq_lines < n_lines + 2) { hipFree(h->d_fq_lines); h->d_fq_lines = nullptr; HIPCHK(h, dmalloc(&h->d_fq_lines, n_lines + 2)); h->cap_fq_lines = n_lines + 2; }
    hipLaunchKernelGGL(k_fq_lines, dim3((u32)n_blocks), dim3(256), 0, h->stream, h->d_fq_text, (u64)n_bytes, blk, h->d_fq_lines, skip);
    h->fq_carry_len = 0;
    if (!whole) {
        u64 end_off = 0;
        HIPCHK(h, hipMemcpyAsync(&end_off, h->d_fq_lines + 4 * n_reads, 8, hipMemcpyDeviceToHost, h->stream));
        HIPCHK(h, hipStreamSynchronize(h->stream));
        if (end_off > n_bytes) return fail(h, MLST_E_HIP, "FASTQ line table inconsistent");
        const u64 keep = n_bytes - end_off;
        if (keep) {
            if (h->cap_fq_carry < keep) { hipFree(h->d_fq_carry); h->d_fq_carry = nullptr; HIPCHK(h, dmalloc(&h->d_fq_carry, keep + 16)); h->cap_fq_carry = keep; }
            HIPCHK(h, hipMemcpyAsync(h->d_fq_carry, h->d_fq_text + end_off, keep, hipMemcpyDeviceToDevice, h->stream));
            h->fq_carry_len = keep;
        }
        n_bytes = end_off; n_lines = 4 * n_reads;
    }
    if (n_reads == 0) { HIPCHK(h, hipEventRecord(h->ev_packed[tslot], h->stream)); return MLST_OK; }
    u64 pair_k = 0;
    if (pair_boundary) {
        if (n_reads & 1) return fail(h, MLST_E_INVALID, "mate files hold different numbers of records (%llu records in all)", (unsigned long long)n_reads);
        pair_k = n_reads / 2;
// ... 2330 lines not shown
    h->cu_split = (int)n_parts; h->cu_part = (int)part;
    for (auto* g : {&h->g_submit, &h->g_typing}) { if (g->exec) { hipGraphExecDestroy(g->exec); g->exec = nullptr; } g->sig.clear(); }
    return MLST_OK;
}
extern "C" int mlst_get_stream(mlst_handle* h, void** stream) {
    if (!h || !stream) return MLST_E_INVALID;
    *stream = (void*)h->own_stream;
    return MLST_OK;
}
extern "C" int mlst_busy(mlst_handle* h) {
    if (!h) return MLST_E_INVALID;
    hipSetDevice(h->device);
    const hipError_t e = hipStreamQuery(h->stream);
    if (e == hipSuccess) return 0;
    if (e == hipErrorNotReady) return 1;
    return fail(h, MLST_E_HIP, "hipStreamQuery: %s", hipGetErrorString(e));
}

extern "C" int mlst_set_stream(mlst_handle* h, void* stream) {
    if (!h) return MLST_E_INVALID;
    hipSetDevice(h->device);
    { int rc_ = bz_flush(h); if (rc_) return rc_; }
    drain_events(h);
    HIPCHK(h, hipStreamSynchronize(h->stream));
    h->stream = stream ? (hipStream_t)stream : h->own_stream;
    return MLST_OK;
}
extern "C" int mlst_export_stats_device_async(mlst_handle* h, int64_t* d_sum, int64_t* d_min) {
    if (!h || !h->have_state) return fail(h, MLST_E_INVALID, "no reference loaded");
    { int rc_ = bz_flush(h); if (rc_) return rc_; }
    hipSetDevice(h->device);
    hipLaunchKernelGGL(k_export, dim3(256), dim3(256), 0, h->stream, h->d_E, (long long*)d_sum, (long long*)d_min);
    HIPCHK(h, hipGetLastError());
    return MLST_OK;
}
extern "C" int mlst_import_stats_device_async(mlst_handle* h, const int64_t* d_sum, const int64_t* d_min) {
    if (!h || !h->have_state) return fail(h, MLST_E_INVALID, "no reference loaded");
    hipSetDevice(h->device);
    hipLaunchKernelGGL(k_import, dim3(256), dim3(256), 0, h->stream, h->d_E, (const long long*)d_sum, (const long long*)d_min);
    HIPCHK(h, hipGetLastError());
    return MLST_OK;
}

static int typing_hand_over(mlst_handle* h, int slot, int64_t* sum_score, uint32_t* n_hits, uint64_t* locus_len, uint64_t* locus_first,
                            uint64_t* counters, int32_t* chosen, uint8_t* letters) {
    const u8* hs = h->h_tstats[slot]; const u8* ha = h->h_tauto[slot];
    Counters* c = (Counters*)(hs + h->off_ctr);
    if (c->err) return fail(h, MLST_E_CAPACITY, "capacity exceeded (flags 0x%llx); raise mlst_params.max_*", (unsigned long long)c->err);
    const u64 nl = h->n_loci;
    if (sum_score) memcpy(sum_score, hs + h->off_sum, (u64)h->n_alleles * 8);
    if (n_hits) memcpy(n_hits, hs + h->off_hits, (u64)h->n_alleles * 4);
    if (locus_len) memcpy(locus_len, hs + h->off_len, nl * 8);
    if (locus_first) memcpy(locus_first, hs + h->off_first, nl * 8);
    note_sieve_window(h, c);
    if (counters) { for (int i = 0; i < MLST_CNT_N; i++) counters[i] = c->cnt[i]; counters[MLST_CNT_RETAINED] = c->n_ret; counters[MLST_CNT_ITEMS] = c->n_items; }
    if (chosen) memcpy(chosen, ha, nl * 4);
    if (letters) memcpy(letters, ha + ((nl * 4 + 15) & ~15ull), h->fixed_cols);
    return MLST_OK;
}
extern "C" int mlst_typing_fetch(mlst_handle* h, int64_t* sum_score, uint32_t* n_hits, uint64_t* locus_len, uint64_t* locus_first,
                                 uint64_t* counters, int32_t* chosen, uint8_t* letters) {
    if (!h || !h->have_state) return fail(h, MLST_E_INVALID, "no reference loaded");
    if (!h->auto_pending) return fail(h, MLST_E_INVALID, "mlst_typing_fetch without mlst_typing_enqueue");
    hipSetDevice(h->device);
    HIPCHK(h, hipStreamSynchronize(h->stream));
    h->auto_pending = false; h->t_ready = h->t_last;
    return typing_hand_over(h, h->t_ready, sum_score, n_hits, locus_len, locus_first, counters, chosen, letters);
}
extern "C" int mlst_typing_wait(mlst_handle* h) {
    if (!h || !h->have_state) return fail(h, MLST_E_INVALID, "no reference loaded");
    if (!h->auto_pending) return fail(h, MLST_E_INVALID, "mlst_typing_wait without mlst_typing_enqueue");
    hipSetDevice(h->device);
    HIPCHK(h, hipStreamSynchronize(h->stream));
    h->auto_pending = false; h->t_ready = h->t_last;
    return MLST_OK;
}
extern "C" int mlst_typing_fetch_waited(mlst_handle* h, int64_t* sum_score, uint32_t* n_hits, uint64_t* locus_len, uint64_t* locus_first,
                                        uint64_t* counters, int32_t* chosen, uint8_t* letters) {
    if (!h || !h->have_state) return fail(h, MLST_E_INVALID, "no reference loaded");
    if (h->t_ready < 0) return fail(h, MLST_E_INVALID, "mlst_typing_fetch_waited without mlst_typing_wait");
    return typing_hand_over(h, h->t_ready, sum_score, n_hits, locus_len, locus_first, counters, chosen, letters);
}

extern "C" int mlst_hamming_all(mlst_handle* h, uint32_t locus, const uint8_t* query, uint32_t len, uint32_t* dist) {
    if (!h || !h->have_ref) return fail(h, MLST_E_INVALID, "no reference loaded");
    if (locus >= h->n_loci) return fail(h, MLST_E_INVALID, "locus %u out of range", locus);
    hipSetDevice(h->device);
    const LocusDev& L = h->loci[locus];
    if (h->cap_dist < L.n_alleles) { hipFree(h->d_dist); h->d_dist = nullptr; HIPCHK(h, dmalloc(&h->d_dist, (u64)L.n_alleles)); h->cap_dist = L.n_alleles; }
    if (h->cap_query < (u64)len + 1) { hipFree(h->d_query); h->d_query = nullptr; HIPCHK(h, dmalloc(&h->d_query, (u64)len + 1)); h->cap_query = (u64)len + 1; }
    if (len > 60000) return fail(h, MLST_E_LIMIT, "query longer than 60000 bytes");
    if (len) HIPCHK(h, hipMemcpyAsync(h->d_query, query, len, hipMemcpyHostToDevice, h->stream));
    hipLaunchKernelGGL(k_hamming, dim3((L.n_alleles + 255) / 256), dim3(256), len ? len : 1, h->stream, h->d_ascii, h->d_aoff, L.a_begin,
                       L.n_alleles, h->d_query, len, h->d_dist);
    HIPCHK(h, hipGetLastError());
    HIPCHK(h, hipMemcpyAsync(dist, h->d_dist, (u64)L.n_alleles * 4, hipMemcpyDeviceToHost, h->stream));
    HIPCHK(h, hipStreamSynchronize(h->stream));
    return MLST_OK;
}

extern "C" int mlst_hamming_le(mlst_handle* h, uint32_t locus, const uint8_t* query, uint32_t len, uint32_t z,
                               int32_t* first_allele_idx, uint32_t* n_within) {
    if (!h || !h->have_ref) return fail(h, MLST_E_INVALID, "no reference loaded");
    if (locus >= h->n_loci) return fail(h, MLST_E_INVALID, "locus %u out of range", locus);
    std::vector<u32> d(h->loci[locus].n_alleles);
    int rc = mlst_hamming_all(h, locus, query, len, d.data()); if (rc) return rc;
    int first = -1; u32 nw = 0;
    for (u32 a = 0; a < d.size(); a++) if (d[a] <= z) { if (first < 0) first = (int)(h->loci[locus].a_begin + a); nw++; }
    if (first_allele_idx) *first_allele_idx = first;
    if (n_within) *n_within = nw;
    return MLST_OK;
}

extern "C" int mlst_get_items(mlst_handle* h, mlst_item* out, uint64_t cap, uint64_t* n) {
    if (!h || !h->have_state) return fail(h, MLST_E_INVALID, "no reference loaded");
    hipSetDevice(h->device);
    Counters c; HIPCHK(h, hipMemcpy(&c, h->E.ctr, sizeof c, hipMemcpyDeviceToHost));
    u64 ni = std::min<u64>(c.n_items, h->E.cap_items);
    if (n) *n = ni;
    u64 k = std::min<u64>(ni, cap);
    if (!k || !out) return MLST_OK;
    std::vector<ItemDev> items(k); HIPCHK(h, hipMemcpy(items.data(), h->E.items, k * sizeof(ItemDev), hipMemcpyDeviceToHost));
    u64 nr = std::min<u64>(c.n_ret, h->E.cap_ret);
    std::vector<u64> ridx(nr ? nr : 1); if (nr) HIPCHK(h, hipMemcpy(ridx.data(), h->E.ret_ridx, nr * 8, hipMemcpyDeviceToHost));
    for (u64 i = 0; i < k; i++) {
        out[i].read_index = items[i].ret < nr ? ridx[items[i].ret] : ~0ull; out[i].locus = items[i].locus; out[i].diag = items[i].diag;
        out[i].strand = items[i].strand; out[i].votes = items[i].votes; out[i].reserved = 0;
    }
    return MLST_OK;
}

extern "C" int mlst_set_profiling(mlst_handle* h, int on) { if (!h) return MLST_E_INVALID; drain_events(h); h->profiling = on == 1; h->window = on != 0; return MLST_OK; }
extern "C" int mlst_get_kernel_time(mlst_handle* h, int which, double* total_ms, uint64_t* launches) {
    if (!h || which < 0 || which >= 20) return MLST_E_INVALID;
    hipSetDevice(h->device); drain_events(h);
    if (total_ms) *total_ms = h->k_ms[which];
    if (launches) *launches = h->k_n[which];
    return MLST_OK;
}
extern "C" int mlst_reset_kernel_time(mlst_handle* h) { if (!h) return MLST_E_INVALID; drain_events(h); for (int i = 0; i < 20; i++) { h->k_ms[i] = 0; h->k_n[i] = 0; } return MLST_OK; }
extern "C" int mlst_get_index_bytes(mlst_handle* h, uint64_t out[4]) {
    if (!h || !out) return MLST_E_INVALID;
    out[0] = h->bytes_arena + h->bytes_hap; out[1] = h->bytes_sieve; out[2] = h->bytes_table; out[3] = (u64)(h->bitmap_fill * 1e6); return MLST_OK;
}
extern "C" int mlst_get_sieve_info(mlst_handle* h, uint64_t out[4]) {
    if (!h || !out || !h->have_ref) return fail(h, MLST_E_INVALID, "no reference loaded");
    out[0] = (u64)h->sieve_kind; out[1] = h->n_keys; out[2] = h->sieve_chain; out[3] = (u64)h->E.sieve_mask + 1; return MLST_OK;
}
extern "C" int mlst_get_extend_info(mlst_handle* h, uint64_t out[8]) {
    if (!h || !out || !h->have_ref) return fail(h, MLST_E_INVALID, "no reference loaded");
    out[0] = h->n_hap_rec; out[1] = h->bytes_hap; out[2] = h->hap_loci; out[3] = h->hap_win_max[0]; out[4] = h->hap_win_max[1];
    out[5] = h->ext_lds_recs[0] ? (u64)ext_lds_bytes(h, 0) : 0; out[6] = h->ext_lds_recs[1] ? (u64)ext_lds_bytes(h, 1) : 0; out[7] = (u64)h->ext_threads; return MLST_OK;
}
extern "C" void mlst_release_index_cache(void) { std::lock_guard<std::mutex> lk(g_index_mu); g_index_last.reset(); memset(g_index_key, 0, sizeof g_index_key); }
extern "C" int mlst_get_route_trace(mlst_handle* h, uint64_t* out, uint64_t cap_words, uint64_t* n_words) {
    if (!h) return MLST_E_INVALID;
    hipSetDevice(h->device);
    if (n_words) *n_words = 0;
    if (!h->rt_trace_on) { h->rt_trace_on = true; return MLST_OK; }
    if (!h->d_rt_trace || !h->rt_prod) return MLST_OK;
    HIPCHK(h, hipStreamSynchronize(h->stream));
    const u64 n_wg = (u64)h->rt_prod + RT_OWNERS, need = 8 + n_wg * 4;
    if (n_words) *n_words = need;
    if (!out || cap_words < need) return MLST_OK;
    out[0] = h->rt_prod; out[1] = (u64)(uintptr_t)h->d_rt_arena; out[2] = (u64)(uintptr_t)h->rt_last_packed; out[3] = (u64)h->wall_khz;
    out[4] = h->rt_cap; out[5] = (u64)(uintptr_t)h->d_rfilter; out[6] = (u64)(uintptr_t)h->d_bin_flags; out[7] = h->cap_rt_arena;
    HIPCHK(h, hipMemcpy(out + 8, h->d_rt_trace, n_wg * 32, hipMemcpyDeviceToHost));
    return MLST_OK;
}
extern "C" int mlst_debug_route_probe(mlst_handle* h, uint64_t* ring_full, uint32_t* cand, uint64_t cap, uint64_t* n_cand) {
    if (!h || !h->have_state) return fail(h, MLST_E_INVALID, "no reference loaded");
    hipSetDevice(h->device);
    Counters* c = nullptr;
    int rc = fetch_stats(h, &c); if (rc) return rc;
    if (ring_full) *ring_full = c->rt_ring_full;
    const u64 n = c->cnt[MLST_CNT_CANDIDATES];
    if (n_cand) *n_cand = n;
    if (cand && n) {
        if (cap < n || h->cap_cand < n || !h->d_cand) return fail(h, MLST_E_INVALID, "candidate list: %llu entries, room for %llu", (unsigned long long)n, (unsigned long long)cap);
        HIPCHK(h, hipMemcpy(cand, h->d_cand, n * 4, hipMemcpyDeviceToHost));
    }
    return MLST_OK;
}
extern "C" int mlst_debug_route_realloc(mlst_handle* h, uint64_t pad_bytes) {
    if (!h) return MLST_E_INVALID;
    hipSetDevice(h->device);
    HIPCHK(h, hipStreamSynchronize(h->stream));
    if (h->g_submit.exec) { hipGraphExecDestroy(h->g_submit.exec); h->g_submit.exec = nullptr; h->g_submit.sig.clear(); }
    if (pad_bytes == ~0ull) { if (h->d_rt_arena) h->dbg_pads.push_back(h->d_rt_arena); }
    else hipFree(h->d_rt_arena);
    h->d_rt_arena = nullptr; h->cap_rt_arena = 0;
    if (pad_bytes && pad_bytes != ~0ull) { void* q = nullptr; HIPCHK(h, hipMalloc(&q, pad_bytes)); h->dbg_pads.push_back(q); }
    return MLST_OK;
}
template <typename T> static int msa_grow(mlst_handle* h, T** p, u64* cap, u64 need) {
    if (*cap >= need && *p) return MLST_OK;
    hipFree(*p); *p = nullptr; *cap = 0;
    HIPCHK(h, dmalloc(p, need)); *cap = need;
    return MLST_OK;
}
extern "C" int mlst_msa_align(mlst_handle* h, const uint8_t* seqs, const uint64_t* off, uint32_t n, uint32_t* center_out, uint32_t* width_out) {
    if (!h) return MLST_E_INVALID;
    if (h->bz_pend.on || h->bzp.on || h->pair_open || h->fq_carry_len) return fail(h, MLST_E_INVALID, "a FASTQ stream is open (its last chunk was not marked final)");
    if (bam_is_open(h)) return fail(h, MLST_E_INVALID, "a %s stream is open (its last chunk was not marked final)", bam_kind(h));
    auto& S = h->msa;
    S.done = false;
    if (n == 0) return fail(h, MLST_E_INVALID, "no sequence to align");
    if (!seqs || !off) return fail(h, MLST_E_INVALID, "NULL argument");
    std::vector<u32> by_len(MLST_MAX_ALLELE_LEN + 1, 0);
    u32 nmax = 0;
    for (u32 r = 0; r < n; r++) {
        if (off[r + 1] < off[r]) return fail(h, MLST_E_INVALID, "offsets must not decrease");
        const u64 len = off[r + 1] - off[r];
        if (len == 0) return fail(h, MLST_E_INVALID, "sequence %u is empty", r);
        if (len > (u64)MLST_MAX_ALLELE_LEN) return fail(h, MLST_E_LIMIT, "sequence %u is longer than %d bases", r, MLST_MAX_ALLELE_LEN);
        for (u64 x = off[r]; x < off[r + 1]; x++) { const u8 c = seqs[x] | 0x20; if (c < 'a' || c > 'z') return fail(h, MLST_E_INVALID, "sequence %u holds a byte that is not an ASCII letter", r); }
        by_len[len]++; nmax = std::max(nmax, (u32)len);
    }
    u32 m = 1;
    for (u32 len = 1; len <= (u32)MLST_MAX_ALLELE_LEN; len++) if (by_len[len] && by_len[len] >= by_len[m]) m = len;
    u32 center = 0;
    while (off[center + 1] - off[center] != m) center++;
    hipSetDevice(h->device);
    const u64 n_bytes = off[n] - off[0], cells = (u64)n * (m + 1);
    { int rc = msa_grow(h, &S.d_seq, &S.cap_seq, n_bytes); if (rc) return rc; }
    { int rc = msa_grow(h, &S.d_off, &S.cap_off, (u64)n + 1); if (rc) return rc; }
    { int rc = msa_grow(h, &S.d_tab, &S.cap_tab, cells * 3); if (rc) return rc; }
    { int rc = msa_grow(h, &S.d_end, &S.cap_end, (u64)n); if (rc) return rc; }
    if (!S.d_slot) HIPCHK(h, dmalloc(&S.d_slot, (u64)2 * (MLST_MAX_ALLELE_LEN + 1) + 1));
    if (!S.h_width) { void* p = nullptr; HIPCHK(h, hipHostMalloc(&p, 4, hipHostMallocDefault)); S.h_width = (u32*)p; }
    MsaDev A;
    A.seq = S.d_seq - off[0]; A.off = S.d_off; A.n = n; A.center = center; A.m = m; A.nmax = nmax;
    A.col = S.d_tab; A.ins_start = S.d_tab + cells; A.ins_len = S.d_tab + 2 * cells;
    A.slot_w = S.d_slot; A.slot_at = S.d_slot + (MLST_MAX_ALLELE_LEN + 1); A.width = S.d_slot + 2 * (MLST_MAX_ALLELE_LEN + 1);
    A.end_state = S.d_end;
    A.T4 = (nmax + 63) / 4 + 1; A.tb_words = (u64)((m + 63) / 64) * A.T4 * 64;
    const u64 per_batch = std::min<u64>(n, std::max<u64>(1, S.batch_bytes / (A.tb_words * 4)));
    { int rc = msa_grow(h, &S.d_tb, &S.cap_tb, per_batch * A.tb_words); if (rc) return rc; }
    A.tb = S.d_tb;
    HIPCHK(h, hipMemcpyAsync(S.d_seq, seqs + off[0], n_bytes, hipMemcpyHostToDevice, h->stream));
    HIPCHK(h, hipMemcpyAsync(S.d_off, off, ((u64)n + 1) * 8, hipMemcpyHostToDevice, h->stream));
    HIPCHK(h, hipMemsetAsync(A.ins_len, 0, cells * 2, h->stream));
    HIPCHK(h, hipMemsetAsync(A.slot_w, 0, (u64)(m + 1) * 4, h->stream));
    u32 wpb = MSA_WPB;
    while (wpb > 1 && (u64)wpb * (nmax + 1) * sizeof(int2) > 49152) wpb >>= 1;
    const size_t lds = (size_t)wpb * (nmax + 1) * sizeof(int2);
    for (u64 r0 = 0; r0 < n; r0 += per_batch) {
        const u32 r1 = (u32)std::min<u64>(n, r0 + per_batch), cnt = r1 - (u32)r0;
        hipLaunchKernelGGL(k_msa_dp, dim3((cnt + wpb - 1) / wpb), dim3(64 * wpb), lds, h->stream, A, (u32)r0, r1);
        hipLaunchKernelGGL(k_msa_trace, dim3((cnt + 63) / 64), dim3(64), 0, h->stream, A, (u32)r0, r1);
    }
    hipLaunchKernelGGL(k_msa_scan, dim3(1), dim3(1024), 0, h->stream, A);
    HIPCHK(h, hipGetLastError());
    HIPCHK(h, hipMemcpyAsync(S.h_width, A.width, 4, hipMemcpyDeviceToHost, h->stream));
    HIPCHK(h, hipStreamSynchronize(h->stream));
    const u32 width = *S.h_width;
    if ((u64)n * width >= (1ull << 32)) return fail(h, MLST_E_LIMIT, "%u rows of %u columns: the alignment does not fit 2^32 bytes", n, width);
    { int rc = msa_grow(h, &S.d_rows, &S.cap_rows, (u64)n * width); if (rc) return rc; }
    hipLaunchKernelGGL(k_msa_rows, dim3(grid_for((u64)n * width, 256, 65536)), dim3(256), 0, h->stream, A, width, S.d_rows);
    HIPCHK(h, hipGetLastError());
    S.n = n; S.width = width; S.done = true;
    if (center_out) *center_out = center;
    if (width_out) *width_out = width;
    return MLST_OK;
}
extern "C" int mlst_msa_fetch(mlst_handle* h, uint8_t* rows) {
    if (!h) return MLST_E_INVALID;
    if (h->bz_pend.on || h->bzp.on || h->pair_open || h->fq_carry_len) return fail(h, MLST_E_INVALID, "a FASTQ stream is open (its last chunk was not marked final)");
    if (bam_is_open(h)) return fail(h, MLST_E_INVALID, "a %s stream is open (its last chunk was not marked final)", bam_kind(h));
    if (!h->msa.done) return fail(h, MLST_E_INVALID, "no finished alignment (mlst_msa_align comes first)");
    if (!rows) return fail(h, MLST_E_INVALID, "NULL argument");
    hipSetDevice(h->device);
    HIPCHK(h, hipMemcpyAsync(rows, h->msa.d_rows, (u64)h->msa.n * h->msa.width, hipMemcpyDeviceToHost, h->stream));
    HIPCHK(h, hipStreamSynchronize(h->stream));
    return MLST_OK;
}

extern "C" int mlst_synchronize(mlst_handle* h) { if (!h) return MLST_E_INVALID; hipSetDevice(h->device); { int rc_ = bz_flush(h); if (rc_) return rc_; } HIPCHK(h, hipStreamSynchronize(h->stream)); return MLST_OK; }
```

metamlst_amd/engine.py:

```python
from __future__ import annotations

import ctypes as C
import dataclasses
import os

import numpy as np

from .index import AlleleIndex
from .typing import SampleStats

_HERE = os.path.dirname(os.path.abspath(__file__))
LIB_PATH = os.environ.get("MLST_LIB", os.path.join(_HERE, "libmlst_hip.so"))

MLST_CNT_N = 8
CNT_TOTAL_RECORDS, CNT_IGNORED, CNT_READS_SEEN, CNT_CANDIDATES, CNT_RETAINED, CNT_ITEMS, CNT_DP_PAIRS = range(7)
KERNELS = ("sieve", "seed", "extend", "banded_sw", "accumulate", "pileup", "pack", "sieve_inkernel", "sieve_wg_longest",
           "sieve_route", "sieve_probe", "sieve_verify", "extend_prep")
SIEVE_KINDS = ("lds", "global", "binned (round 1, removed)", "routed")


class MlstParams(C.Structure):
    _fields_ = [("minscore", C.c_int32), ("max_xm", C.c_int32), ("min_read_len", C.c_int32),
                ("minqual", C.c_int32), ("mincov", C.c_int32), ("match_bonus", C.c_int32),
                ("mm_max", C.c_int32), ("mm_min", C.c_int32), ("n_penalty", C.c_int32),
# ... 44 lines not shown
    def pileup_arrays(self) -> tuple:
        return (self.allele, self.pos0, self.as_, self.xm, self.cigar_off, self.cigar, self.seq_off, self.seq, self.qual)


class BgzfCrcMismatch(MlstError):

    def __init__(self, text: str, file: int | None):
        super().__init__(text)
        self.file = file


class HostPathNeeded(MlstError):
    """The library's "host path needed: <reason> at record <n>" (mlst_submit_bam_bgzf, mlst_submit_sam_text): the BAM or the SAM
    text holds a record the device does not treat; the caller runs samin.AlignmentSample on the file, which raises or answers as
    the reference would.  Also "... at byte
    <n>" (mlst_submit_fasta): a sequence line only Python's strip() treats; the caller tiles the file with fastq.tile_fasta."""


class CorruptInput(Exception):

    def __init__(self, path: str, message: str):
        super().__init__("%s: %s" % (path, message))
        self.path = path


def crc_checked(paths, fn):
    from .fastq import BgzfCrcError
    try:
        return fn()
    except BgzfCrcMismatch as e:
        raise CorruptInput(paths[1] if e.file == 2 else paths[0], str(e)) from e
    except BgzfCrcError as e:
        raise CorruptInput(paths[0], str(e)) from e


_lib = None


def load_library(path: str | None = None):
    global _lib
    if _lib is not None and path is None:
        return _lib
    path = path or LIB_PATH
    try:
        import torch
    except Exception:
        pass
    if not os.path.exists(path):
        raise MlstError("HIP engine library not built: %s is missing (run __graft_entry__.build()); "
                        "there is no CPU fallback" % path)
    lib = C.CDLL(path)
    vp, u8p, u64p, u32p, i32p, i64p, u16p = (C.c_void_p, C.c_void_p, C.c_void_p, C.c_void_p, C.c_void_p, C.c_void_p, C.c_void_p)
    H = C.c_void_p
    sig = {
        "mlst_default_params": (None, [C.POINTER(MlstParams)]),
        "mlst_create": (C.c_int, [C.c_int, C.POINTER(MlstParams), C.POINTER(H)]),
        "mlst_destroy": (None, [H]),
        "mlst_last_error": (C.c_char_p, [H]),
        "mlst_load_reference": (C.c_int, [H, u8p, u64p, u32p, u32p, i32p, C.c_uint32]),
        "mlst_set_reference_cache": (C.c_int, [C.c_char_p]),
        "mlst_submit_reads": (C.c_int, [H, u8p, u8p, u64p, C.c_uint64, C.c_int]),
        "mlst_submit_fastq": (C.c_int, [H, u8p, C.c_uint64, C.c_int, C.POINTER(C.c_uint64)]),
        "mlst_submit_fasta": (C.c_int, [H, u8p, C.c_uint64, C.c_uint32, C.c_uint32, C.c_uint32, C.POINTER(C.c_uint64), C.POINTER(C.c_uint64)]),
        "mlst_submit_fastq_bgzf": (C.c_int, [H, u8p, C.c_uint64, C.c_int, C.c_int, C.POINTER(C.c_uint64), C.POINTER(C.c_uint64)]),
        "mlst_submit_fastq_bgzf_pair": (C.c_int, [H, u8p, C.c_uint64, u8p, C.c_uint64, C.c_int, C.POINTER(C.c_uint64), C.POINTER(C.c_uint64),
                                                  C.POINTER(C.c_uint64)]),
        "mlst_selftest_inflate": (C.c_int, [u8p, C.c_uint64, u8p, C.c_uint64, C.POINTER(C.c_uint64)]),
        "mlst_selftest_inflate_canon": (C.c_int, [u8p, C.c_uint64, u8p, C.c_uint64, C.POINTER(C.c_uint64), C.POINTER(C.c_int)]),
        "mlst_debug_bgzf_walk": (C.c_int, [u8p, C.c_uint64, C.POINTER(C.c_uint64), C.POINTER(C.c_uint64), C.POINTER(C.c_int)]),
        "mlst_selftest_inflate_device": (C.c_int, [H, u8p, C.c_uint64, u8p, C.c_uint64, C.POINTER(C.c_uint64), C.POINTER(C.c_double)]),
        "mlst_selftest_bgzf_crc": (C.c_int, [H, u8p, C.c_uint64, u32p, C.c_uint64, C.POINTER(C.c_uint64), C.POINTER(C.c_double)]),
        "mlst_debug_inflate_paths": (C.c_int, [H, C.POINTER(C.c_uint64), C.POINTER(C.c_uint64)]),
        "mlst_set_bgzf_verify": (C.c_int, [H, C.c_int]),
        "mlst_get_bgzf_verify": (C.c_int, [H, C.POINTER(C.c_int)]),
        "mlst_set_read_tiling": (C.c_int, [H, C.c_uint32, C.c_uint32]),
        "mlst_get_read_tiling": (C.c_int, [H, C.POINTER(C.c_uint32), C.POINTER(C.c_uint32)]),
        "mlst_get_read_tiling_info": (C.c_int, [H, C.POINTER(C.c_uint64)]),
        "mlst_set_read_names": (C.c_int, [H, C.c_int]),
        "mlst_get_read_names": (C.c_int, [H, C.POINTER(C.c_int)]),
        "mlst_set_export_md": (C.c_int, [H, C.c_int]),
        "mlst_get_export_md": (C.c_int, [H, C.POINTER(C.c_int)]),
        "mlst_read_names_info": (C.c_int, [H, C.POINTER(C.c_uint64)]),
        "mlst_read_names_fetch": (C.c_int, [H, C.POINTER(C.c_uint64), C.POINTER(C.c_uint64), C.POINTER(C.c_uint8)]),
        "mlst_submit_reads_device": (C.c_int, [H, u8p, u8p, u64p, C.c_uint64, C.c_uint32, C.c_int]),
        "mlst_pack_reads_device": (C.c_int, [H, u8p, u8p, u64p, C.c_uint64, u32p, u8p, u16p, C.c_uint32, C.c_uint32]),
        "mlst_submit_packed_device": (C.c_int, [H, u32p, u8p, u16p, C.c_uint64, C.c_uint32, C.c_uint32, C.c_int]),
        "mlst_pack_fastq_host": (C.c_int, [u8p, C.c_uint64, C.c_uint32, C.c_uint32, u32p, u8p, u16p, C.c_uint64, C.POINTER(C.c_uint64), C.c_int]),
        "mlst_submit_packed_host": (C.c_int, [H, u32p, u8p, u16p, C.c_uint64, C.c_uint32, C.c_uint32, C.c_int]),
        "mlst_alloc_host": (C.c_int, [C.c_uint64, C.POINTER(C.c_void_p)]),
        "mlst_free_host": (C.c_int, [C.c_void_p]),
        "mlst_get_allele_stats": (C.c_int, [H, i64p, u32p, u64p, u64p, u64p]),
        "mlst_stats_flat_sizes": (C.c_int, [H, C.POINTER(C.c_uint64), C.POINTER(C.c_uint64)]),
        "mlst_export_stats_device": (C.c_int, [H, i64p, i64p]),
        "mlst_import_stats_device": (C.c_int, [H, i64p, i64p]),
        "mlst_pileup": (C.c_int, [H, u32p, C.c_uint32, u32p]),
        "mlst_set_depth_cap": (C.c_int, [H, C.c_uint32]),
        "mlst_pileup_device": (C.c_int, [H, u32p, C.c_uint32, u32p, C.POINTER(C.c_uint64)]),
        "mlst_consensus": (C.c_int, [H, u32p, C.c_uint32, C.c_uint32, C.c_char, u8p, u32p]),
        "mlst_consensus_from_counts_device": (C.c_int, [H, u32p, C.c_uint64, C.c_uint32, C.c_char, u8p]),
        "mlst_pileup_alignments": (C.c_int, [H, u32p, C.c_uint32, C.c_uint64, u32p, i32p, i32p, i32p, u64p, u32p, u64p, u8p, u8p,
                                             C.c_int32, C.c_int32, C.c_int32, u32p]),
        "mlst_alignments_export": (C.c_int, [H, u32p, C.c_uint32, C.POINTER(C.c_uint64), C.POINTER(C.c_uint64), C.POINTER(C.c_uint64)]),
        "mlst_alignments_fetch": (C.c_int, [H, u64p, u32p, i32p, i32p, i32p, i32p, u8p, u64p, u32p, u64p, u8p, u8p]),
        "mlst_alignments_text_open": (C.c_int, [H, u8p, u64p, C.c_int, C.c_uint64]),
        "mlst_alignments_text_next": (C.c_int, [H, u8p, C.c_uint64, C.POINTER(C.c_uint64), C.POINTER(C.c_uint64), C.POINTER(C.c_int)]),
        "mlst_alignments_text_close": (C.c_int, [H]),
        "mlst_typing_layout": (C.c_int, [H, u64p, C.POINTER(C.c_uint64)]),
        "mlst_typing_enqueue": (C.c_int, [H, C.c_int32, C.c_uint32, C.c_char]),
        "mlst_typing_choose_pileup": (C.c_int, [H, C.c_int32, u32p]),
        "mlst_typing_finish": (C.c_int, [H, C.c_uint32, C.c_char, u32p]),
        "mlst_typing_choose_pileup_compact": (C.c_int, [H, C.c_int32, u32p, C.c_uint64]),
        "mlst_typing_finish_compact": (C.c_int, [H, C.c_uint32, C.c_char, u32p]),
        "mlst_typing_compact_info": (C.c_int, [H, C.POINTER(C.c_uint64), C.POINTER(C.c_uint32)]),
        "mlst_set_stream": (C.c_int, [H, C.c_void_p]),
        "mlst_set_cu_partition": (C.c_int, [H, C.c_uint32, C.c_uint32]),
        "mlst_get_stream": (C.c_int, [H, C.POINTER(C.c_void_p)]),
        "mlst_busy": (C.c_int, [H]),
        "mlst_export_stats_device_async": (C.c_int, [H, i64p, i64p]),
        "mlst_import_stats_device_async": (C.c_int, [H, i64p, i64p]),
        "mlst_typing_fetch": (C.c_int, [H, i64p, u32p, u64p, u64p, u64p, i32p, u8p]),
        "mlst_typing_wait": (C.c_int, [H]),
        "mlst_typing_fetch_waited": (C.c_int, [H, i64p, u32p, u64p, u64p, u64p, i32p, u8p]),
        "mlst_round_tenths": (C.c_longlong, [C.c_longlong, C.c_uint32]),
        "mlst_hamming_le": (C.c_int, [H, C.c_uint32, u8p, C.c_uint32, C.c_uint32, C.POINTER(C.c_int32), C.POINTER(C.c_uint32)]),
        "mlst_hamming_all": (C.c_int, [H, C.c_uint32, u8p, C.c_uint32, u32p]),
        "mlst_msa_align": (C.c_int, [H, u8p, u64p, C.c_uint32, C.POINTER(C.c_uint32), C.POINTER(C.c_uint32)]),
        "mlst_msa_fetch": (C.c_int, [H, u8p]),
        "mlst_reset_sample": (C.c_int, [H]),
        "mlst_set_read_index_base": (C.c_int, [H, C.c_uint64]),
        "mlst_get_items": (C.c_int, [H, C.c_void_p, C.c_uint64, C.POINTER(C.c_uint64)]),
        "mlst_set_profiling": (C.c_int, [H, C.c_int]),
        "mlst_get_kernel_time": (C.c_int, [H, C.c_int, C.POINTER(C.c_double), C.POINTER(C.c_uint64)]),
        "mlst_reset_kernel_time": (C.c_int, [H]),
        "mlst_get_index_bytes": (C.c_int, [H, C.POINTER(C.c_uint64)]),
        "mlst_get_sieve_info": (C.c_int, [H, C.POINTER(C.c_uint64)]),
        "mlst_get_extend_info": (C.c_int, [H, C.POINTER(C.c_uint64)]),
        "mlst_release_index_cache": (None, []),
        "mlst_submit_fastq_stream": (C.c_int, [H, u8p, C.c_uint64, C.c_int, C.c_int, C.POINTER(C.c_uint64)]),
        "mlst_submit_fastq_pair": (C.c_int, [H, u8p, C.c_uint64, u8p, C.c_uint64, C.POINTER(C.c_uint64)]),
        "mlst_get_route_trace": (C.c_int, [H, u64p, C.c_uint64, C.POINTER(C.c_uint64)]),
        "mlst_debug_route_realloc": (C.c_int, [H, C.c_uint64]),
        "mlst_debug_route_probe": (C.c_int, [H, C.POINTER(C.c_uint64), u32p, C.c_uint64, C.POINTER(C.c_uint64)]),
        "mlst_bam_open": (C.c_int, [H, C.c_int, i32p, i32p, u8p, C.c_uint32, C.c_uint32, u32p, C.c_uint32]),
        "mlst_submit_bam_bgzf": (C.c_int, [H, u8p, C.c_uint64, C.c_int, C.POINTER(C.c_uint64), C.POINTER(C.c_uint64)]),
        "mlst_bam_set_capacity": (C.c_int, [H, C.c_uint64]),
        "mlst_bam_pileup_fetch": (C.c_int, [H, u32p]),
        "mlst_debug_bam_split": (C.c_int, [H, C.c_uint32, C.POINTER(C.c_uint64)]),
        "mlst_sam_open": (C.c_int, [H, C.c_int, u8p, u64p, i32p, i32p, u8p, C.c_uint32, u32p, C.c_uint32]),
        "mlst_submit_sam_text": (C.c_int, [H, u8p, C.c_uint64, C.c_int, C.POINTER(C.c_uint64)]),
        "mlst_bam_reads_open": (C.c_int, [H, C.c_uint32, C.c_uint32, C.c_int]),
        "mlst_bam_reads_info": (C.c_int, [H, C.POINTER(C.c_uint64)]),
        "mlst_debug_last_packed": (C.c_int, [H, u32p, C.c_uint64, u8p, C.c_uint64, u16p, C.c_uint64, C.POINTER(C.c_uint64)]),
        "mlst_debug_fasta_info": (C.c_int, [H, C.POINTER(C.c_uint64)]),
        "mlst_synchronize": (C.c_int, [H]),
    }
    tolerant = bool(os.environ.get("MLST_LIB_ALLOW_MISSING"))
    for name, (res, args) in sig.items():
        if tolerant and not hasattr(lib, name):
            continue
        fn = getattr(lib, name)
        fn.restype, fn.argtypes = res, args
    lib._mlst_symbols = tuple(sig)
    if path == LIB_PATH:
        _lib = lib
    return lib


def _ptr(a: np.ndarray):
    return a.ctypes.data_as(C.c_void_p)


def pack_fastq_host(text, read_len_max: int = 160, threads: int = 0):
    lib = load_library()
    buf = np.frombuffer(text, dtype=np.uint8) if not isinstance(text, np.ndarray) else text
    wpr = ((int(read_len_max) + 31) // 32) * 2
    qstride = (int(read_len_max) + 7) // 8 * 8
    cap = int(buf.size // 8 + 64)
    cap = min(cap, int(np.count_nonzero(buf[:1 << 20] == 10) * (buf.size / max(1, min(buf.size, 1 << 20))) / 4 * 1.1) + 4096)
    packed = np.zeros(((cap + 63) // 64) * 64 * wpr, np.uint32)
    qrows = np.empty((cap, qstride), np.uint8)
    lens = np.empty(cap, np.uint16)
    n = C.c_uint64()
    rc = lib.mlst_pack_fastq_host(_ptr(buf), buf.size, wpr, qstride, _ptr(packed), _ptr(qrows), _ptr(lens), cap, C.byref(n), int(threads))
    if rc == -4:
        cap = int(buf.size // 8 + 64)
        packed = np.zeros(((cap + 63) // 64) * 64 * wpr, np.uint32); qrows = np.empty((cap, qstride), np.uint8); lens = np.empty(cap, np.uint16)
        rc = lib.mlst_pack_fastq_host(_ptr(buf), buf.size, wpr, qstride, _ptr(packed), _ptr(qrows), _ptr(lens), cap, C.byref(n), int(threads))
    if rc != 0:
        raise MlstError("mlst_pack_fastq_host failed (%d): not whole 4-line FASTQ records, or a read longer than %d bases" % (rc, read_len_max))
    return packed, qrows, lens, int(n.value), wpr, qstride


def pinned_array(n_bytes: int) -> np.ndarray:
    import weakref
    lib = load_library()
    p = C.c_void_p()
    rc = lib.mlst_alloc_host(int(n_bytes), C.byref(p))
    if rc != 0 or not p.value:
        raise MlstError("mlst_alloc_host(%d) failed (%d)" % (n_bytes, rc))
    arr = np.frombuffer((C.c_uint8 * int(n_bytes)).from_address(p.value), np.uint8)
    weakref.finalize(arr, lib.mlst_free_host, C.c_void_p(p.value)).atexit = False
    return arr


def pair_file_cuts(size1: int, size2: int, chunk_bytes: int) -> list[tuple[int, int, int, int]]:
    total = size1 + size2
    if total == 0:
        return [(0, 0, 0, 0)]
    chunk = max(1, int(chunk_bytes))
    marks = [0.0]
    step = min(1.0, chunk / 4 / total)
    while marks[-1] < 1.0:
        marks.append(min(1.0, marks[-1] + step))
        step = min(1.0, chunk / total)
    cuts = []
    for a, b in zip(marks, marks[1:]):
        cuts.append((int(size1 * a), int(size1 * b) if b < 1.0 else size1, int(size2 * a), int(size2 * b) if b < 1.0 else size2))
    return cuts


class Engine:

    def __init__(self, device: int = 0, params: MlstParams | None = None):
        self.lib = load_library()
        self.params = params or default_params()
        self._h = C.c_void_p()
        rc = self.lib.mlst_create(int(device), C.byref(self.params), C.byref(self._h))
        if rc != 0:
            msg = self.lib.mlst_last_error(None)
            raise MlstError("mlst_create failed (%d): %s" % (rc, msg.decode() if msg else "?"))
        self.device = device
        self.depth_cap = 0
        self.index: AlleleIndex | None = None

    def close(self):
        if self._h:
            self.lib.mlst_destroy(self._h)
            self._h = C.c_void_p()

    def __del__(self):
        try:
            self.close()
        except Exception:
            pass

    def _check(self, rc: int, what: str):
        if rc != 0:
            msg = self.lib.mlst_last_error(self._h)
            text = msg.decode() if msg else "?"
            if rc == -1 and text.startswith("CRC mismatch in BGZF block"):
                raise BgzfCrcMismatch("%s failed (%d): %s" % (what, rc, text), 1 if " of file 1 " in text else 2 if " of file 2 " in text else None)
            if rc == -1 and text.startswith("host path needed"):
                raise HostPathNeeded("%s: %s" % (what, text))
            raise MlstError("%s failed (%d): %s" % (what, rc, text))

    def load_reference(self, index: AlleleIndex, cache_path: str | None = None):
        self.index = index
        if cache_path is not None:
            self.lib.mlst_set_reference_cache(cache_path.encode() if cache_path else None)
        self._check(self.lib.mlst_load_reference(self._h, _ptr(index.ascii_concat), _ptr(index.off), _ptr(index.locus_id),
                                                 _ptr(index.species_id), _ptr(index.allele_no), index.n_alleles),
                    "mlst_load_reference")

    def submit_reads(self, bases: np.ndarray, quals: np.ndarray, off: np.ndarray, paired: bool = False):
        bases = np.ascontiguousarray(bases, dtype=np.uint8)
        quals = np.ascontiguousarray(quals, dtype=np.uint8)
        off = np.ascontiguousarray(off, dtype=np.uint64)
        self._check(self.lib.mlst_submit_reads(self._h, _ptr(bases), _ptr(quals), _ptr(off), len(off) - 1, int(paired)),
                    "mlst_submit_reads")

    def submit_fastq(self, text, paired: bool = False) -> int:
        buf = np.frombuffer(text, dtype=np.uint8) if not isinstance(text, np.ndarray) else np.ascontiguousarray(text, np.uint8)
        n = C.c_uint64()
        self._check(self.lib.mlst_submit_fastq(self._h, _ptr(buf) if buf.size else None, buf.size, int(paired), C.byref(n)), "mlst_submit_fastq")
        return int(n.value)

    def submit_fasta(self, text, read_len: int = 150, stride: int = 25, min_len: int = 50) -> tuple[int, int]:
        for v in (read_len, stride, min_len):
            if not 0 <= int(v) < (1 << 32):
                raise ValueError("read_len, stride and min_len are unsigned 32-bit numbers")
        buf = np.frombuffer(text, dtype=np.uint8) if not isinstance(text, np.ndarray) else np.ascontiguousarray(text, np.uint8)
        nc, nr = C.c_uint64(), C.c_uint64()
        self._check(self.lib.mlst_submit_fasta(self._h, _ptr(buf) if buf.size else None, buf.size, int(read_len), int(stride), int(min_len),
                                               C.byref(nc), C.byref(nr)), "mlst_submit_fasta")
        return int(nc.value), int(nr.value)

    def submit_fasta_file(self, path: str, read_len: int = 150, stride: int = 25, min_len: int = 50, chunk_bytes: int = 64 << 20) -> tuple[int, int]:
        from .fastq import fasta_chunks, prefetch, release_buffers
        ring: list = []
        nc = nr = 0
        try:
            for chunk in prefetch(fasta_chunks(path, chunk_bytes, reuse=True, ring=ring)):
                c, r = self.submit_fasta(chunk, read_len, stride, min_len)
                nc += c
                nr += r
        finally:
            release_buffers(ring)
        return nc, nr

    def submit_fastq_bgzf(self, data, final: bool, paired: bool = False) -> int:
        buf = np.frombuffer(data, dtype=np.uint8) if not isinstance(data, np.ndarray) else np.ascontiguousarray(data, np.uint8)
        n = C.c_uint64()
        self._check(self.lib.mlst_submit_fastq_bgzf(self._h, _ptr(buf) if buf.size else None, buf.size, int(final), int(paired), C.byref(n), None),
                    "mlst_submit_fastq_bgzf")
        return int(n.value)

# ... 34 lines not shown

    def submit_bam_bgzf(self, data, final: bool, partial: bool = False):
        buf = np.frombuffer(data, dtype=np.uint8) if not isinstance(data, np.ndarray) else np.ascontiguousarray(data, np.uint8)
        n, used = C.c_uint64(), C.c_uint64()
        self._check(self.lib.mlst_submit_bam_bgzf(self._h, _ptr(buf) if buf.size else None, buf.size, int(final), C.byref(n), C.byref(used) if partial else None),
                    "mlst_submit_bam_bgzf")
        return int(n.value), int(used.value) if partial else buf.size

    def _bam_stream_file(self, path: str, lo: int, chunk_bytes: int) -> int:
        from .fastq import prefetch, raw_chunks, release_buffers
        margin, hi = 1 << 17, os.path.getsize(path)
        total, carry, at = 0, None, lo
        n, used = C.c_uint64(), C.c_uint64()
        if hi <= lo:
            self._check(self.lib.mlst_submit_bam_bgzf(self._h, None, 0, 1, C.byref(n), None), "mlst_submit_bam_bgzf")
            return int(n.value)
        ring: list = []
        try:
            for buf, got in prefetch(raw_chunks(path, chunk_bytes, lo, hi, margin, reuse=True, ring=ring)):
                at += got
                c = 0 if carry is None else carry.size
                if c > margin:
                    raise MlstError("a BGZF block of more than %d bytes?" % margin)
                if c:
                    buf[margin - c:margin] = carry
                view = buf[margin - c:margin + got]
                last = at >= hi
                self._check(self.lib.mlst_submit_bam_bgzf(self._h, _ptr(view), view.size, int(last), C.byref(n), None if last else C.byref(used)),
                            "mlst_submit_bam_bgzf")
                total += int(n.value)
                carry = None if last else view[int(used.value):].copy()
        finally:
            release_buffers(ring)
        return total

    def submit_bam_file(self, path: str, species_filter: str | None = None, chunk_bytes: int = 64 << 20) -> int:
        from .samin import bam_ref_table, read_bam_header
        names, lo, skip = read_bam_header(path, self.bgzf_verify)
        self.bam_open(1, *bam_ref_table(self.index, names, species_filter), skip_bytes=skip)
        return self._bam_stream_file(path, lo, chunk_bytes)

    def pileup_bam_file(self, path: str, chosen, chunk_bytes: int = 64 << 20) -> dict[int, np.ndarray]:
        from .samin import bam_ref_table, read_bam_header
        names, lo, skip = read_bam_header(path, self.bgzf_verify)
        ch = np.ascontiguousarray(chosen, np.uint32)
        self.bam_open(2, *bam_ref_table(self.index, names, None), skip_bytes=skip, chosen=ch)
        self._bam_stream_file(path, lo, chunk_bytes)
        lens = [int(self.index.off[a + 1] - self.index.off[a]) for a in ch]
        counts = np.zeros((max(1, sum(lens)), 4), np.uint32)
        self._check(self.lib.mlst_bam_pileup_fetch(self._h, _ptr(counts)), "mlst_bam_pileup_fetch")
        out, at = {}, 0
        for a, L in zip(ch, lens):
            out[int(a)] = counts[at:at + L]
            at += L
        return out

    def sam_open(self, which: int, names, ref_allele, ref_locus, ref_flags, chosen=None) -> None:
        enc = [n.encode("utf-8", "surrogateescape") if isinstance(n, str) else bytes(n) for n in names]
        off = np.zeros(len(enc) + 1, np.uint64)
        off[1:] = np.cumsum([len(n) for n in enc], dtype=np.uint64)
        arena = np.frombuffer(b"".join(enc) or b"\0", np.uint8)
        ra, rl, rf = np.ascontiguousarray(ref_allele, np.int32), np.ascontiguousarray(ref_locus, np.int32), np.ascontiguousarray(ref_flags, np.uint8)
        if not ra.size == rl.size == rf.size == len(enc):
            raise ValueError("one (allele, locus, flags) triple per name")
        ch = np.ascontiguousarray([] if chosen is None else chosen, np.uint32)
        self._check(self.lib.mlst_sam_open(self._h, int(which), _ptr(arena), _ptr(off), _ptr(ra), _ptr(rl), _ptr(rf), len(enc),
                                           _ptr(ch) if ch.size else None, ch.size), "mlst_sam_open")

    def submit_sam_text(self, text, final: bool) -> int:
        buf = np.frombuffer(text, dtype=np.uint8) if not isinstance(text, np.ndarray) else np.ascontiguousarray(text, np.uint8)
        n = C.c_uint64()
        self._check(self.lib.mlst_submit_sam_text(self._h, _ptr(buf) if buf.size else None, buf.size, int(final), C.byref(n)), "mlst_submit_sam_text")
        return int(n.value)

    def _sam_stream_file(self, path: str, chunk_bytes: int) -> int:
        from .fastq import prefetch, raw_chunks, release_buffers
        if chunk_bytes < 1:
            raise ValueError("chunk_bytes must be positive")
        chunk_bytes = min(int(chunk_bytes), (1 << 30) - 1)
        with open(path, "rb") as f:
            zipped = f.read(2) == b"\x1f\x8b"
        total = 0
        if zipped:
            import gzip

            def pieces():
                with gzip.open(path, "rb") as z:
                    while True:
                        piece = z.read(chunk_bytes)
                        if not piece:
                            return
                        yield piece
            for piece in prefetch(pieces()):
                total += self.submit_sam_text(piece, False)
            return total + self.submit_sam_text(b"", True)
        size = os.path.getsize(path)
        if size == 0:
            return self.submit_sam_text(b"", True)
        ring: list = []
        at = 0
        try:
            for buf, got in prefetch(raw_chunks(path, chunk_bytes, 0, size, 0, reuse=True, ring=ring)):
                at += got
                total += self.submit_sam_text(buf[:got], at >= size)
        finally:
            release_buffers(ring)
        return total

    def submit_sam_file(self, path: str, species_filter: str | None = None, chunk_bytes: int = 64 << 20) -> int:
        from .samin import bam_ref_table, read_sam_header
        names = read_sam_header(path)
        self.sam_open(1, names, *bam_ref_table(self.index, names, species_filter))
        return self._sam_stream_file(path, chunk_bytes)

    def pileup_sam_file(self, path: str, chosen, chunk_bytes: int = 64 << 20) -> dict[int, np.ndarray]:
        from .samin import bam_ref_table, read_sam_header
        names = read_sam_header(path)
        ch = np.ascontiguousarray(chosen, np.uint32)
        self.sam_open(2, names, *bam_ref_table(self.index, names, None), chosen=ch)
        self._sam_stream_file(path, chunk_bytes)
        lens = [int(self.index.off[a + 1] - self.index.off[a]) for a in ch]
        counts = np.zeros((max(1, sum(lens)), 4), np.uint32)
        self._check(self.lib.mlst_bam_pileup_fetch(self._h, _ptr(counts)), "mlst_bam_pileup_fetch")
        out, at = {}, 0
        for a, L in zip(ch, lens):
            out[int(a)] = counts[at:at + L]
            at += L
        return out

    def bam_reads_open(self, n_ref: int, skip_bytes: int = 0, paired: bool = False) -> None:
        self._check(self.lib.mlst_bam_reads_open(self._h, int(n_ref), int(skip_bytes), int(paired)), "mlst_bam_reads_open")

    def submit_bam_reads_file(self, path: str, paired: bool = False, chunk_bytes: int = 64 << 20) -> int:
        from .samin import read_bam_header
        names, lo, skip = read_bam_header(path, self.bgzf_verify)
        self.bam_reads_open(len(names), skip, paired)
        self._bam_stream_file(path, lo, chunk_bytes)
        return self.bam_reads_info()[0]

    def bam_reads_info(self) -> tuple[int, int, int, int]:
        out = (C.c_uint64 * 4)()
        self._check(self.lib.mlst_bam_reads_info(self._h, out), "mlst_bam_reads_info")
        return tuple(int(x) for x in out)

    def debug_last_packed(self):
        out = (C.c_uint64 * 3)()
        self._check(self.lib.mlst_debug_last_packed(self._h, None, 0, None, 0, None, 0, out), "mlst_debug_last_packed")
        n, wpr, qs = (int(x) for x in out)
        packed = np.zeros(((n + 63) // 64) * 64 * wpr, np.uint32); qrows = np.zeros((n, qs), np.uint8); lens = np.zeros(n, np.uint16)
        if n:
            self._check(self.lib.mlst_debug_last_packed(self._h, _ptr(packed), packed.size, _ptr(qrows), qrows.size, _ptr(lens), lens.size, out),
                        "mlst_debug_last_packed")
        return packed, qrows, lens, wpr, qs

    def fasta_info(self) -> tuple[int, int, int, int]:
        out = (C.c_uint64 * 4)()
        self._check(self.lib.mlst_debug_fasta_info(self._h, out), "mlst_debug_fasta_info")
        return tuple(int(x) for x in out)

    def bam_set_capacity(self, max_entries: int) -> None:
        self._check(self.lib.mlst_bam_set_capacity(self._h, int(max_entries)), "mlst_bam_set_capacity")

    def debug_bam_split(self, force_miss_every: int = 0) -> int:
        n = C.c_uint64()
        self._check(self.lib.mlst_debug_bam_split(self._h, int(force_miss_every), C.byref(n)), "mlst_debug_bam_split")
        return int(n.value)

    def submit_fastq_bgzf_pair(self, data1, data2, final: bool) -> int:
        b1 = np.frombuffer(data1, dtype=np.uint8) if not isinstance(data1, np.ndarray) else np.ascontiguousarray(data1, np.uint8)
        b2 = np.frombuffer(data2, dtype=np.uint8) if not isinstance(data2, np.ndarray) else np.ascontiguousarray(data2, np.uint8)
        n = C.c_uint64()
        self._check(self.lib.mlst_submit_fastq_bgzf_pair(self._h, _ptr(b1) if b1.size else None, b1.size, _ptr(b2) if b2.size else None, b2.size,
                                                         int(final), C.byref(n), None, None), "mlst_submit_fastq_bgzf_pair")
        return int(n.value)

    def submit_fastq_bgzf_pair_files(self, path1: str, path2: str, chunk_bytes: int = (512 << 20) - (1 << 18)) -> int:
        from .fastq import prefetch, raw_chunks, release_buffers
        margin = 1 << 17
        s1, s2 = os.path.getsize(path1), os.path.getsize(path2)
        n, used1, used2 = C.c_uint64(), C.c_uint64(), C.c_uint64()
        if s1 + s2 == 0:
            self._check(self.lib.mlst_submit_fastq_bgzf_pair(self._h, None, 0, None, 0, 1, C.byref(n), None, None), "mlst_submit_fastq_bgzf_pair")
            return int(n.value)
        cuts = pair_file_cuts(s1, s2, chunk_bytes)
        ring1: list = []
        ring2: list = []

        def span(path, lo, hi, ring):
            for buf, got in raw_chunks(path, hi - lo, lo, hi, margin, reuse=True, ring=ring):
                return buf, got
            return None, 0

        def pieces():
            for a1, b1, a2, b2 in cuts:
                yield span(path1, a1, b1, ring1), span(path2, a2, b2, ring2)

        total = 0
        carry = [None, None]
        for k, (p1, p2) in enumerate(prefetch(pieces())):
            last = k == len(cuts) - 1
            views = []
            for f, (buf, got) in enumerate((p1, p2)):
                c = 0 if carry[f] is None else carry[f].size
                if c > margin:
                    raise MlstError("a BGZF block of more than %d bytes?" % margin)
                if buf is None:
                    views.append(carry[f] if c else np.empty(0, np.uint8))
                    continue
                if c:
                    buf[margin - c:margin] = carry[f]
                views.append(buf[margin - c:margin + got])
            v1, v2 = views
            self._check(self.lib.mlst_submit_fastq_bgzf_pair(self._h, _ptr(v1) if v1.size else None, v1.size, _ptr(v2) if v2.size else None, v2.size,
                                                             int(last), C.byref(n), None if last else C.byref(used1), None if last else C.byref(used2)),
                        "mlst_submit_fastq_bgzf_pair")
            total += int(n.value)
            if not last:
                carry = [v1[int(used1.value):].copy(), v2[int(used2.value):].copy()]
        release_buffers(ring1)
        release_buffers(ring2)
        return total

    def inflate_bgzf(self, data) -> bytes:
        buf = np.frombuffer(data, dtype=np.uint8) if not isinstance(data, np.ndarray) else np.ascontiguousarray(data, np.uint8)
        room, off = 0, 0
        while off + 18 <= buf.size:
            size = int(buf[off + 16]) + (int(buf[off + 17]) << 8) + 1
            plain = buf[off:off + 16].tobytes() == b"\x1f\x8b\x08\x04" + buf[off + 4:off + 10].tobytes() + b"\x06\x00BC\x02\x00"
            if not plain or size < 26 or off + size > buf.size:
                room = (buf.size // 18 + 1) * 65536
                break
            room += min(int.from_bytes(buf[off + size - 4:off + size].tobytes(), "little"), 65536)
            off += size
        if off != buf.size:
            room = (buf.size // 18 + 1) * 65536
        out = np.empty(max(1, room), np.uint8)
        n, ms = C.c_uint64(), C.c_double()
        self._check(self.lib.mlst_selftest_inflate_device(self._h, _ptr(buf), buf.size, _ptr(out), out.size, C.byref(n), C.byref(ms)), "mlst_selftest_inflate_device")
        self.last_inflate_ms = float(ms.value)
        return out[:int(n.value)].tobytes()

    def inflate_paths(self):
        n, left = C.c_uint64(), C.c_uint64()
        self._check(self.lib.mlst_debug_inflate_paths(self._h, C.byref(n), C.byref(left)), "mlst_debug_inflate_paths")
        return int(n.value), int(left.value)

    def bgzf_block_crcs(self, data) -> np.ndarray:
        buf = np.frombuffer(data, dtype=np.uint8) if not isinstance(data, np.ndarray) else np.ascontiguousarray(data, np.uint8)
        out = np.zeros(max(1, buf.size // 26 + 1), np.uint32)
        n, ms = C.c_uint64(), C.c_double()
        self._check(self.lib.mlst_selftest_bgzf_crc(self._h, _ptr(buf), buf.size, _ptr(out), out.size, C.byref(n), C.byref(ms)), "mlst_selftest_bgzf_crc")
        self.last_crc_ms = float(ms.value)
        return out[:int(n.value)].copy()

    def set_bgzf_verify(self, on: bool) -> None:
        self._check(self.lib.mlst_set_bgzf_verify(self._h, int(bool(on))), "mlst_set_bgzf_verify")

    def set_read_tiling(self, read_len: int = 150, stride: int = 25) -> None:
        self._check(self.lib.mlst_set_read_tiling(self._h, int(read_len), int(stride)), "mlst_set_read_tiling")

    def get_read_tiling(self) -> tuple[int, int]:
        a, b = C.c_uint32(0), C.c_uint32(0)
        self._check(self.lib.mlst_get_read_tiling(self._h, C.byref(a), C.byref(b)), "mlst_get_read_tiling")
        return int(a.value), int(b.value)

    def read_tiling_info(self) -> dict:
        out = (C.c_uint64 * 4)()
        self._check(self.lib.mlst_get_read_tiling_info(self._h, out), "mlst_get_read_tiling_info")
        return {"records": int(out[0]), "cut": int(out[1]), "windows": int(out[2]), "longest": int(out[3])}

    def set_read_names(self, on: bool = True) -> None:
        self._check(self.lib.mlst_set_read_names(self._h, int(bool(on))), "mlst_set_read_names")

    def get_read_names(self) -> bool:
        on = C.c_int()
        self._check(self.lib.mlst_get_read_names(self._h, C.byref(on)), "mlst_get_read_names")
        return bool(on.value)

    def read_names_info(self) -> dict:
        out = (C.c_uint64 * 4)()
        self._check(self.lib.mlst_read_names_info(self._h, out), "mlst_read_names_info")
        return {"named": int(out[0]), "bytes": int(out[1]), "fallbacks": int(out[2]), "longest": int(out[3])}

    def read_names(self) -> dict:
        info = self.read_names_info()
        n = info["named"]
        ridx = np.zeros(max(n, 1), np.uint64); off = np.zeros(n + 1, np.uint64); data = np.zeros(max(info["bytes"], 1), np.uint8)
        self._check(self.lib.mlst_read_names_fetch(self._h, ridx.ctypes.data_as(C.POINTER(C.c_uint64)), off.ctypes.data_as(C.POINTER(C.c_uint64)),
                                                   data.ctypes.data_as(C.POINTER(C.c_uint8))), "mlst_read_names_fetch")
        raw = data.tobytes()
        return {int(ridx[i]): raw[int(off[i]):int(off[i + 1])] for i in range(n)}

    def set_export_md(self, on: bool = True) -> None:
        self._check(self.lib.mlst_set_export_md(self._h, int(bool(on))), "mlst_set_export_md")

    def get_export_md(self) -> bool:
        on = C.c_int()
        self._check(self.lib.mlst_get_export_md(self._h, C.byref(on)), "mlst_get_export_md")
        return bool(on.value)

    @property
    def bgzf_verify(self) -> bool:
        on = C.c_int()
        self._check(self.lib.mlst_get_bgzf_verify(self._h, C.byref(on)), "mlst_get_bgzf_verify")
        return bool(on.value)

# ... 339 lines not shown
```

Baseline: 21540.

## Add single-wave extend kernel variant with LDS aliasing and occupancy-sized grid

Adds a one-wave (64-thread) specialization of the extend kernel. It aliases the read-plane scratch arrays into dynamic LDS, drops the double-buffered record slot and the cross-wave count reductions, and computes penalty columns on the fly. The aim is to cut static LDS per workgroup and barriers so more workgroups fit per CU. The grid size is now derived from hipOccupancy queries times the CU count instead of a fixed block count. The risks are extra recomputation (penalty lookups from global memory, the block_slots readfirstlane calls) and LDS atomics for the counters. A debug occupancy query is also added.

Result: faster. 22110, median of 6 (+2.6%).

```diff
diff --git a/include/mlst_debug.h b/include/mlst_debug.h
--- a/include/mlst_debug.h
+++ b/include/mlst_debug.h
@@ -31,6 +31,8 @@
 
 int mlst_debug_fasta_info(mlst_handle* h, uint64_t out[4]);
 
+int mlst_debug_kernel_occupancy(mlst_handle* h, uint64_t out[8]);
+
 #ifdef __cplusplus
 }
 #endif
diff --git a/metamlst_amd/csrc/mlst_engine.hip b/metamlst_amd/csrc/mlst_engine.hip
--- a/metamlst_amd/csrc/mlst_engine.hip
+++ b/metamlst_amd/csrc/mlst_engine.hip
@@ -2050,18 +2050,30 @@
 #endif
 #define R_TRACK 0x10000000u
 
-template <int NB>
+template <int NB, int NT>
 __device__ __forceinline__ void extend_body(const EngineDev* __restrict__ Ep, const KParams& P, const u32 lds_recs, const u32 acc_cap, const u32* __restrict__ xrec, const u64 cap_xrec) {
     typedef XRec<NB> X;
+    constexpr bool W1 = NT == 64;
+    static_assert(NT == 0 || (NT == 64 && X::WORDS <= 64), "a compile-time thread count means one wave, whose lanes hold a record");
     const EngineDev& E = *Ep;
     extern __shared__ int4 s_hap[];
-    __shared__ u32 s_rl[RW / 2 + 2]; __shared__ u32 s_rh[RW / 2 + 2]; __shared__ u32 s_rn[RW / 2 + 2]; __shared__ u32 s_odd[RW / 2 + 2];
-    __shared__ u8 s_pen[RQ]; __shared__ u8 s_pentab[128];
-    __shared__ u32 s_cnt[16][3];
-    __shared__ __attribute__((aligned(16))) u32 s_x[2][X::WORDS];
+    u16* const s_pend = reinterpret_cast<u16*>(s_hap + lds_recs + 1);
+    u32 *s_rl, *s_rh, *s_rn, *s_odd; u8* s_pen; u32 (*s_cnt)[3]; u64* s_c;
+    if constexpr (W1) {
+        s_rl = reinterpret_cast<u32*>(s_hap); s_rh = s_rl + (RW / 2 + 2); s_rn = s_rh + (RW / 2 + 2); s_odd = s_rn + (RW / 2 + 2);
+        s_pen = reinterpret_cast<u8*>(s_pend); s_cnt = nullptr;
+        __shared__ u64 a_c[2]; s_c = a_c;
+    } else {
+        __shared__ u32 a_rl[RW / 2 + 2]; __shared__ u32 a_rh[RW / 2 + 2]; __shared__ u32 a_rn[RW / 2 + 2]; __shared__ u32 a_odd[RW / 2 + 2];
+        __shared__ u8 a_pen[RQ]; __shared__ u32 a_cnt[16][3];
+        s_rl = a_rl; s_rh = a_rh; s_rn = a_rn; s_odd = a_odd; s_pen = a_pen; s_cnt = a_cnt; s_c = nullptr;
+    }
+    __shared__ u8 s_pentab[128];
+    __shared__ __attribute__((aligned(16))) u32 s_x[W1 ? 1 : 2][X::WORDS];
     __shared__ u64 s_ii[2];
-    const int tid = threadIdx.x, nthr = blockDim.x, nwv = blockDim.x >> 6;
+    const int tid = threadIdx.x, nthr = W1 ? 64 : (int)blockDim.x, nwv = W1 ? 1 : (int)(blockDim.x >> 6);
     for (int i = tid; i < 128; i += nthr) s_pentab[i] = E.pen_tab[i];
+    if constexpr (W1) { if (tid < 2) s_c[tid] = 0; }
     u64 c_tot = 0, c_ign = 0;
     u64 N;
     { const u64 b0 = E.ctr->items_done, e0 = E.ctr->n_items < E.cap_items ? E.ctr->n_items : E.cap_items; N = e0 - b0; if (N > cap_xrec) N = cap_xrec; }
@@ -2082,7 +2094,6 @@
         s_ii[0] = resolve(atomicAdd(&E.ctr->ext_q[myq][0], 1ull));
         s_ii[1] = tried < EXT_Q ? resolve(atomicAdd(&E.ctr->ext_q[myq][0], 1ull)) : N;
     }
-    u16* const s_pend = reinterpret_cast<u16*>(s_hap + lds_recs + 1);
     const bool packed_acc = E.cap_items < (1ull << 24);
     __syncthreads();
     u64 pp = uniform_u64(s_ii[0]);
@@ -2099,7 +2110,7 @@
         u64 ticket = 0;
         if (tid == 0 && tried < EXT_Q) ticket = atomicAdd(&E.ctr->ext_q[myq][0], 1ull);
         asm volatile("" ::: "memory");
-        const u32* x = s_x[cur];
+        const u32* x = s_x[W1 ? 0 : cur];
         const uint4 h0 = *reinterpret_cast<const uint4*>(x), h1 = *reinterpret_cast<const uint4*>(x + 4), h2 = *reinterpret_cast<const uint4*>(x + 8), h3 = *reinterpret_cast<const uint4*>(x + 12);
         const u32 flags = __builtin_amdgcn_readfirstlane(h0.x);
         const u64 ii = (u64)(u32)__builtin_amdgcn_readfirstlane(x[31]);
@@ -2115,7 +2126,10 @@
         bool parked = false;
         auto park = [&]() {
             #pragma unroll
-            for (int k = 0; k < (X::WORDS + 63) / 64; k++) if (tid < 64 && tid + 64 * k < X::WORDS) s_x[cur ^ 1][tid + 64 * k] = pf[k];
+            for (int k = 0; k < (X::WORDS + 63) / 64; k++) {
+                if constexpr (W1) TIE1(pf[k]);
+                else if (tid < 64 && tid + 64 * k < X::WORDS) s_x[cur ^ 1][tid + 64 * k] = pf[k];
+            }
             if (tid == 0) s_ii[cur] = tried < EXT_Q ? resolve(ticket) : N;
             parked = true;
         };
@@ -2136,10 +2150,11 @@
             }
             if (valid) E.res[res_off + a] = r;
         };
+        auto cold_tid = [&]() -> int { int t = tid; if constexpr (W1) asm volatile("" : "+v"(t)); return t; };
         auto stage_old = [&]() {
             ItemDev it; it.res_off = res_off; it.ret = ret; it.locus = __builtin_amdgcn_readfirstlane(h1.x); it.diag = diag; it.strand = (flags & XF_STRAND) ? 1 : 0; it.votes = 0;
             __syncthreads();
-            stage_read_planes(E, P, it, n, s_rl, s_rh, s_rn, s_odd, s_pen, s_pentab, tid, nthr);
+            stage_read_planes(E, P, it, n, s_rl, s_rh, s_rn, s_odd, s_pen, s_pentab, cold_tid(), nthr);
             __syncthreads();
         };
         auto pairs_loop = [&](const bool only_marked) {
@@ -2151,7 +2166,7 @@
                 od[w] = __builtin_amdgcn_readfirstlane(s_odd[w]);
                 rn[w] = read_has_n ? __builtin_amdgcn_readfirstlane(s_rn[w]) : 0u;
             }
-            for (u32 a = tid; a < n_alleles; a += nthr) {
+            for (u32 a = (u32)cold_tid(); a < n_alleles; a += nthr) {
                 const bool valid = !only_marked || (E.res[res_off + a] & R_TRACK);
                 int m = (int)E.allele_len[a_begin + a];
                 int mm = 0, bs = 0, be = 0, best = P0;
@@ -2200,8 +2215,15 @@
             load_ids((u32)tid, Wn); load_ids((u32)tid + nthr, Wn2); load_ids((u32)tid + 2 * nthr, Wn3); load_ids((u32)tid + 3 * nthr, Wn4);
             const u32 ident = hb[NB + 1] - hb[0];
             u32 sbase[NB + 1], wid[NB + 1];
-            #pragma unroll
-            for (int t = 0; t <= NB; t++) { const bool present = hb[t + 1] != hb[t]; sbase[t] = present ? hb[t] - hb[0] : ident; wid[t] = present ? 16u : 0u; }
+            auto block_slots = [&]() {
+                u32 g[NB + 2];
+                #pragma unroll
+                for (int t = 0; t <= NB + 1; t++) g[t] = W1 ? (u32)__builtin_amdgcn_readfirstlane(x[X::HB + t]) : hb[t];
+                const u32 idn = g[NB + 1] - g[0];
+                #pragma unroll
+                for (int t = 0; t <= NB; t++) { const bool present = g[t + 1] != g[t]; sbase[t] = present ? g[t] - g[0] : idn; wid[t] = present ? 16u : 0u; }
+            };
+            if constexpr (!W1) block_slots();
             if (tid == 0) s_hap[ident] = make_int4(0, NEGP, NEGP, NEGP);
             if (special_any) lds_barrier();
             XT(1);
@@ -2225,6 +2247,7 @@
             }
             park();
             lds_barrier();
+            if constexpr (W1) block_slots();
             XT(2);
             auto compose = [&](const u32 (&w)[NR], int& best, int& mm) {
                 u32 wp[NB / 2 + 1];
@@ -2242,15 +2265,19 @@
                 best = v > best ? v : best;
                 mm = (-ts) & 0xFFFF;
             };
+            auto pen_col = [&](const int i) -> int {
+                if constexpr (W1) { const u8 qb = (E.ret_quals.g() + (u64)ret * RQ)[(flags & XF_STRAND) ? n - 1 - i : i]; return (qb >> 7) ? (int)(u8)P.n_penalty : (int)s_pentab[qb & 0x7F]; }
+                else return (int)s_pen[i];
+            };
             auto span_needs_dp = [&](const u32 (&w)[NR], const int mm, const int xm, const int score) -> bool {
                 const int MA = P.match_bonus << MLST_P_SHIFT, PD = (pen_def << MLST_P_SHIFT) + 1;
                 int cur = P0, best = P0, cs = 0, last = 0, blen = 0, overlap = 0, i1 = 0; bool first = true;
                 #pragma unroll
                 for (int t = 0; t <= NB; t++) {
-                    if (hb[t + 1] == hb[t]) continue;
-                    const u32 k = (u32)t + (odd16 >> 4);
-                    const u32 id = (w[k >> 1] >> (16u * (k & 1u))) & 0xFFFFu;
-                    const uint4 rc = *reinterpret_cast<GP<const uint4>::G*>(recs + hb[t] + id);
+                    if (W1 ? wid[t] == 0u : hb[t + 1] == hb[t]) continue;
+                    const u32 wp = __builtin_amdgcn_alignbit(t / 2 + 1 < NR ? w[t / 2 + 1 < NR ? t / 2 + 1 : 0] : 0u, w[t / 2], odd16);
+                    const u32 id = (wp >> (16u * ((u32)t & 1u))) & 0xFFFFu;
+                    const uint4 rc = *reinterpret_cast<GP<const uint4>::G*>(recs + (W1 ? x[X::HB + t] : hb[t]) + id);
                     const uint4 sp = *reinterpret_cast<const uint4*>(x + X::PL + 4 * t);
                     const u32 lm = rc.w >= 32u ? 0xFFFFFFFFu : ((1u << rc.w) - 1u), valid = x[X::VR + t] & lm;
                     if (!valid) continue;
@@ -2265,7 +2292,7 @@
                         cur += (i - last) * MA;
                         if (cur > best) { best = cur; blen = i - cs; }
                         int dec = PD;
-                        if ((special >> bit) & 1u) dec = ((((rc.z >> bit) & 1u) ? P.n_penalty : (int)s_pen[32 * t - (int)((u32)diag & 31u) + bit]) << MLST_P_SHIFT) + 1;
+                        if ((special >> bit) & 1u) dec = ((((rc.z >> bit) & 1u) ? P.n_penalty : pen_col(32 * t - (int)((u32)diag & 31u) + bit)) << MLST_P_SHIFT) + 1;
                         cur -= dec;
                         if (cur <= P0) { cur = P0; cs = i + 1; }
                         last = i + 1;
@@ -2315,15 +2342,17 @@
                     }
                     if (tid == 0) {
                         if (tot_rec) atomicAdd(&E.ret_nrec[ret], tot_rec);
-                        c_tot += tot_rec; c_ign += tot_rec - tot_acc;
+                        if constexpr (W1) { if (tot_rec) atomicAdd(&s_c[0], (u64)tot_rec); if (tot_rec - tot_acc) atomicAdd(&s_c[1], (u64)(tot_rec - tot_acc)); }
+                        else { c_tot += tot_rec; c_ign += tot_rec - tot_acc; }
                         E.item_state[ii] = (u8)((single ? IS_SINGLE : 0) | IS_DONE | (tot_acc ? IS_ACC : 0));
                     }
                     done_fast = true;
                 } else { slow = true; nrec = 0; ntrack = 0; }
             }
             if (slow) {
-                load_ids((u32)tid, Wn);
-                for (u32 a = tid; a < n_alleles; a += nthr) {
+                const u32 tid_c = (u32)cold_tid();
+                load_ids(tid_c, Wn);
+                for (u32 a = tid_c; a < n_alleles; a += nthr) {
                     u32 W[NR];
                     #pragma unroll
                     for (int j = 0; j < NR; j++) W[j] = Wn[j];
@@ -2347,15 +2376,18 @@
         }
         XT(3);
         if (!done_fast && use_hap) {
-        if ((tid & 63) == 0) { s_cnt[tid >> 6][0] = nrec; s_cnt[tid >> 6][1] = ndp; }
-        __syncthreads();
         u32 tot_rec = 0, tot_dp = 0;
-        for (int w = 0; w < nwv; w++) { tot_rec += s_cnt[w][0]; tot_dp += s_cnt[w][1]; }
+        if constexpr (W1) { tot_rec = __builtin_amdgcn_readfirstlane(nrec); tot_dp = __builtin_amdgcn_readfirstlane(ndp); }
+        else {
+            if ((tid & 63) == 0) { s_cnt[tid >> 6][0] = nrec; s_cnt[tid >> 6][1] = ndp; }
+            __syncthreads();
+            for (int w = 0; w < nwv; w++) { tot_rec += s_cnt[w][0]; tot_dp += s_cnt[w][1]; }
+        }
         if (tid == 0 && tot_rec) atomicAdd(&E.ret_nrec[ret], tot_rec);
         if (res_ok && tot_dp == 0 && ((flags & XF_SINGLE) || !P.quirk || tot_rec != 1)) {
             bool use_xo = P.quirk && tot_rec == 1;
             u32 acc = 0, ign = 0;
-            for (u32 a = tid; a < n_alleles; a += nthr) {
+            for (u32 a = (u32)cold_tid(); a < n_alleles; a += nthr) {
                 u32 r = E.res[res_off + a];
                 const bool rec = r & R_REC, ok = rec && accept_rec(P, r, n, use_xo);
                 if (ok) {
@@ -2364,13 +2396,15 @@
                 }
                 acc += (u32)__popcll(__ballot(ok)); ign += (u32)__popcll(__ballot(rec && !ok));
             }
-            __syncthreads();
-            if ((tid & 63) == 0) { s_cnt[tid >> 6][0] = acc; s_cnt[tid >> 6][1] = ign; }
-            __syncthreads();
+            if constexpr (!W1) {
+                __syncthreads();
+                if ((tid & 63) == 0) { s_cnt[tid >> 6][0] = acc; s_cnt[tid >> 6][1] = ign; }
+                __syncthreads();
+            }
             if (tid == 0) {
                 u32 A = 0, I = 0;
-                for (int w = 0; w < nwv; w++) { A += s_cnt[w][0]; I += s_cnt[w][1]; }
-                c_tot += tot_rec; c_ign += I;
+                if constexpr (W1) { A = acc; I = ign; if (tot_rec) atomicAdd(&s_c[0], (u64)tot_rec); if (I) atomicAdd(&s_c[1], (u64)I); }
+                else { for (int w = 0; w < nwv; w++) { A += s_cnt[w][0]; I += s_cnt[w][1]; } c_tot += tot_rec; c_ign += I; }
                 const u8 state = (u8)((flags & XF_SINGLE) ? IS_SINGLE : 0);
                 E.item_state[ii] = (u8)(state | IS_DONE | (A ? IS_ACC : 0));
             }
@@ -2379,18 +2413,24 @@
         XT(4);
         if (!parked) park();
         lds_barrier();
+        if constexpr (W1) {
+            if (tid < X::WORDS) s_x[0][tid] = pf[0];
+            lds_barrier();
+        }
         pp = pp_next; cur ^= 1;
         XT(5);
     }
     XT_FLUSH;
     if (tid == 0) {
+        if constexpr (W1) { c_tot = s_c[0]; c_ign = s_c[1]; }
         if (c_tot) atomicAdd(&E.ctr->cnt[MLST_CNT_TOTAL_RECORDS], c_tot);
         if (c_ign) atomicAdd(&E.ctr->cnt[MLST_CNT_IGNORED], c_ign);
     }
 }
 
-__global__ __launch_bounds__(1024) void k_extend_160(const EngineDev* __restrict__ Ep, KParams P, u32 lds_recs, u32 acc_cap, const u32* __restrict__ xrec, u64 cap_xrec) { extend_body<5>(Ep, P, lds_recs, acc_cap, xrec, cap_xrec); }
-__global__ __launch_bounds__(512) void k_extend_320(const EngineDev* __restrict__ Ep, KParams P, u32 lds_recs, u32 acc_cap, const u32* __restrict__ xrec, u64 cap_xrec) { extend_body<RW / 2>(Ep, P, lds_recs, acc_cap, xrec, cap_xrec); }
+__global__ __launch_bounds__(1024) void k_extend_160(const EngineDev* __restrict__ Ep, KParams P, u32 lds_recs, u32 acc_cap, const u32* __restrict__ xrec, u64 cap_xrec) { extend_body<5, 0>(Ep, P, lds_recs, acc_cap, xrec, cap_xrec); }
+__global__ __launch_bounds__(64) __attribute__((amdgpu_waves_per_eu(5))) void k_extend_160_w1(const EngineDev* __restrict__ Ep, KParams P, u32 lds_recs, u32 acc_cap, const u32* __restrict__ xrec, u64 cap_xrec) { extend_body<5, 64>(Ep, P, lds_recs, acc_cap, xrec, cap_xrec); }
+__global__ __launch_bounds__(512) void k_extend_320(const EngineDev* __restrict__ Ep, KParams P, u32 lds_recs, u32 acc_cap, const u32* __restrict__ xrec, u64 cap_xrec) { extend_body<RW / 2, 0>(Ep, P, lds_recs, acc_cap, xrec, cap_xrec); }
 
 template <int CTRL, int ROW_MASK = 0xF> __device__ inline int dpp_i32(int old, int src) {
     return __builtin_amdgcn_update_dpp(old, src, CTRL, ROW_MASK, 0xF, false);
@@ -3159,6 +3199,8 @@
     u64 reads_seen = 0;
     u32 max_wpr = 0;
     int ext_threads = 64, ext_blocks = 5120;
+    bool ext_occ = true, ext_blocks_fixed = false;
+    int ext_wg_per_cu[2] = {0, 0}, n_cu = 256;
     int extp_threads = 256, extp_blocks = 1792; u32 pair_loci = 0;
     int sieve_g_blocks = 256 * 5;
     u8* d_fq_text = nullptr;
@@ -3747,7 +3789,17 @@
     return -1;
 }
 
-static size_t ext_lds_bytes(const mlst_handle* h, int k) { return (size_t)(h->ext_lds_recs[k] + 1) * 16 + (size_t)h->ext_acc_cap * 2; }
+static bool ext_w1(const mlst_handle* h, int k) { return h->ext_occ && k == 0 && h->ext_threads == 64; }
+static u32 ext_recs_arg(const mlst_handle* h, int k) { return ext_w1(h, k) ? std::max<u32>(h->ext_lds_recs[k], (u32)(RW / 2 + 2) - 1u) : h->ext_lds_recs[k]; }
+static size_t ext_lds_bytes(const mlst_handle* h, int k) {
+    const size_t pend = (size_t)h->ext_acc_cap * 2;
+    return (size_t)(ext_recs_arg(h, k) + 1) * 16 + (ext_w1(h, k) ? std::max<size_t>(pend, 160) : pend);
+}
+static const void* ext_kernel(const mlst_handle* h, int k) { return k ? (const void*)k_extend_320 : ext_w1(h, k) ? (const void*)k_extend_160_w1 : (const void*)k_extend_160; }
+static int ext_grid(const mlst_handle* h, int k) {
+    if (h->ext_blocks_fixed || !h->ext_occ || h->ext_wg_per_cu[k] <= 0) return h->ext_blocks;
+    return std::max(1, h->ext_wg_per_cu[k] * (h->n_cu / std::max(1, h->cu_split)));
+}
 extern "C" int mlst_load_reference(mlst_handle* h, const uint8_t* ascii, const uint64_t* off, const uint32_t* locus_id,
                                    const uint32_t* species_id, const int32_t* allele_no, uint32_t n_alleles) {
     if (!h || !off || !locus_id) return fail(h, MLST_E_INVALID, "NULL argument");
@@ -3880,8 +3932,9 @@
         HIPCHK(h, hipMemcpy(h->d_loci, lc.data(), (u64)n_loci * sizeof(LocusDev), hipMemcpyHostToDevice));
         int thr = mx_hap <= 512 ? 64 : 256;
         const char* e1 = getenv("MLST_EXT_THREADS"); if (e1 && atoi(e1) >= 64 && atoi(e1) <= 1024 && atoi(e1) % 64 == 0) thr = atoi(e1);
+        const char* e8 = getenv("MLST_EXT_OCC"); h->ext_occ = !(e8 && atoi(e8) == 0);
         int blocks = 1280 * 256 / thr;
-        const char* e2 = getenv("MLST_EXT_BLOCKS"); if (e2 && atoi(e2) > 0) blocks = atoi(e2);
+        const char* e2 = getenv("MLST_EXT_BLOCKS"); h->ext_blocks_fixed = e2 && atoi(e2) > 0; if (h->ext_blocks_fixed) blocks = atoi(e2);
         h->ext_threads = thr; h->ext_blocks = blocks;
         int thr2 = mx_pair <= 512 ? 64 : 256;
         const char* e5 = getenv("MLST_EXTP_THREADS"); if (e5 && atoi(e5) >= 64 && atoi(e5) <= 1024 && atoi(e5) % 64 == 0) thr2 = atoi(e5);
@@ -3892,8 +3945,11 @@
         for (int k = 0; k < 2; k++) {
             h->ext_lds_recs[k] = h->hap_win_max[k];
             if (ext_lds_bytes(h, k) > 48u * 1024u)
-                HIPCHK(h, hipFuncSetAttribute(k ? (const void*)k_extend_320 : (const void*)k_extend_160, hipFuncAttributeMaxDynamicSharedMemorySize, (int)ext_lds_bytes(h, k)));
-        }
+                HIPCHK(h, hipFuncSetAttribute(ext_kernel(h, k), hipFuncAttributeMaxDynamicSharedMemorySize, (int)ext_lds_bytes(h, k)));
+            h->ext_wg_per_cu[k] = 0;
+            if (n_hap) HIPCHK(h, hipOccupancyMaxActiveBlocksPerMultiprocessor(&h->ext_wg_per_cu[k], ext_kernel(h, k), k ? std::min(thr, 512) : thr, ext_lds_bytes(h, k)));
+        }
+        { int n_cu_i = 0; HIPCHK(h, hipDeviceGetAttribute(&n_cu_i, hipDeviceAttributeMultiprocessorCount, h->device)); if (n_cu_i > 0) h->n_cu = n_cu_i; }
         const char* e3 = getenv("MLST_SIEVE_BLOCKS"); if (e3 && atoi(e3) > 0) h->sieve_g_blocks = atoi(e3);
         const char* e7 = getenv("MLST_RT_SLICE"); h->rt_slice = (e7 && atoll(e7) > 0) ? (u64)atoll(e7) : 0;
     }
@@ -4007,7 +4063,8 @@
     const int gs = phase ? 0 : graph_enter(h, h->g_submit, {(u64)(uintptr_t)d_packed, (u64)(uintptr_t)d_qrows, (u64)(uintptr_t)d_lens, (u64)n_reads, (u64)wpr,
                                                (u64)qstride, (u64)h->reads_seen, (u64)(uintptr_t)h->d_cand,
                                                (u64)(uintptr_t)h->d_bin_flags, (u64)(uintptr_t)h->d_rt_arena, (u64)(uintptr_t)h->d_rt_counts,
-                                               (u64)(uintptr_t)h->d_rt_emitted, (u64)h->rt_cap, (u64)h->rt_prod, (u64)h->rt_nw, (u64)paired, (u64)(uintptr_t)h->d_rt_trace, (u64)(uintptr_t)h->d_rt_parked, (u64)h->cap_rt_parked, (u64)h->rt_pf, rt_slice, (u64)h->rt_exam, (u64)h->rt_wo});
+                                               (u64)(uintptr_t)h->d_rt_emitted, (u64)h->rt_cap, (u64)h->rt_prod, (u64)h->rt_nw, (u64)paired, (u64)(uintptr_t)h->d_rt_trace, (u64)(uintptr_t)h->d_rt_parked, (u64)h->cap_rt_parked, (u64)h->rt_pf, rt_slice, (u64)h->rt_exam, (u64)h->rt_wo,
+                                               (u64)h->ext_occ, (u64)ext_grid(h, wpr <= 10 ? 0 : 1)});
     if (gs == 1) { h->reads_seen += n_reads; return MLST_OK; }
     if (phase != 2) { Prof pf(h, 0);
       if (h->sieve_kind == MLST_SIEVE_LDS) {
@@ -4069,8 +4126,9 @@
         if (wpr <= 10) hipLaunchKernelGGL(k_ext_prep<5>, dim3(2048), dim3(256), 0, h->stream, h->d_E, h->kp, h->d_xrec[0], h->cap_xrec[0]);
         else hipLaunchKernelGGL(k_ext_prep<RW / 2>, dim3(2048), dim3(256), 0, h->stream, h->d_E, h->kp, h->d_xrec[1], h->cap_xrec[1]); }
       { Prof pf(h, 2);
-        const int thr = h->ext_threads, blocks = h->ext_blocks;
-        if (wpr <= 10) hipLaunchKernelGGL(k_extend_160, dim3(blocks), dim3(thr), ext_lds_bytes(h, 0), h->stream, h->d_E, h->kp, h->ext_lds_recs[0], h->ext_acc_cap, h->d_xrec[0], h->cap_xrec[0]);
+        const int thr = h->ext_threads, blocks = ext_grid(h, wpr <= 10 ? 0 : 1);
+        if (wpr <= 10 && ext_w1(h, 0)) hipLaunchKernelGGL(k_extend_160_w1, dim3(blocks), dim3(64), ext_lds_bytes(h, 0), h->stream, h->d_E, h->kp, ext_recs_arg(h, 0), h->ext_acc_cap, h->d_xrec[0], h->cap_xrec[0]);
+        else if (wpr <= 10) hipLaunchKernelGGL(k_extend_160, dim3(blocks), dim3(thr), ext_lds_bytes(h, 0), h->stream, h->d_E, h->kp, h->ext_lds_recs[0], h->ext_acc_cap, h->d_xrec[0], h->cap_xrec[0]);
         else hipLaunchKernelGGL(k_extend_320, dim3(blocks), dim3(std::min(thr, 512)), ext_lds_bytes(h, 1), h->stream, h->d_E, h->kp, h->ext_lds_recs[1], h->ext_acc_cap, h->d_xrec[1], h->cap_xrec[1]); }
     }
     if (h->pair_loci) { Prof pf(h, 2);
@@ -6707,6 +6765,15 @@
     out[0] = h->n_hap_rec; out[1] = h->bytes_hap; out[2] = h->hap_loci; out[3] = h->hap_win_max[0]; out[4] = h->hap_win_max[1];
     out[5] = h->ext_lds_recs[0] ? (u64)ext_lds_bytes(h, 0) : 0; out[6] = h->ext_lds_recs[1] ? (u64)ext_lds_bytes(h, 1) : 0; out[7] = (u64)h->ext_threads; return MLST_OK;
 }
+extern "C" int mlst_debug_kernel_occupancy(mlst_handle* h, uint64_t out[8]) {
+    if (!h || !out || !h->have_ref) return fail(h, MLST_E_INVALID, "no reference loaded");
+    hipSetDevice(h->device);
+    hipFuncAttributes fa; HIPCHK(h, hipFuncGetAttributes(&fa, ext_kernel(h, 0)));
+    int per_cu = 0; HIPCHK(h, hipOccupancyMaxActiveBlocksPerMultiprocessor(&per_cu, ext_kernel(h, 0), h->ext_threads, ext_lds_bytes(h, 0)));
+    out[0] = (u64)fa.numRegs; out[1] = (u64)fa.localSizeBytes; out[2] = (u64)fa.sharedSizeBytes; out[3] = (u64)ext_lds_bytes(h, 0);
+    out[4] = (u64)per_cu; out[5] = (u64)h->ext_threads; out[6] = (u64)ext_grid(h, 0); out[7] = ext_w1(h, 0) ? 1 : 0;
+    return MLST_OK;
+}
 extern "C" void mlst_release_index_cache(void) { std::lock_guard<std::mutex> lk(g_index_mu); g_index_last.reset(); memset(g_index_key, 0, sizeof g_index_key); }
 extern "C" int mlst_get_route_trace(mlst_handle* h, uint64_t* out, uint64_t cap_words, uint64_t* n_words) {
     if (!h) return MLST_E_INVALID;
diff --git a/metamlst_amd/engine.py b/metamlst_amd/engine.py
--- a/metamlst_amd/engine.py
+++ b/metamlst_amd/engine.py
@@ -220,6 +220,7 @@
         "mlst_bam_reads_info": (C.c_int, [H, C.POINTER(C.c_uint64)]),
         "mlst_debug_last_packed": (C.c_int, [H, u32p, C.c_uint64, u8p, C.c_uint64, u16p, C.c_uint64, C.POINTER(C.c_uint64)]),
         "mlst_debug_fasta_info": (C.c_int, [H, C.POINTER(C.c_uint64)]),
+        "mlst_debug_kernel_occupancy": (C.c_int, [H, C.POINTER(C.c_uint64)]),
         "mlst_synchronize": (C.c_int, [H]),
     }
     tolerant = bool(os.environ.get("MLST_LIB_ALLOW_MISSING"))
@@ -560,6 +561,12 @@
             self._check(self.lib.mlst_debug_last_packed(self._h, _ptr(packed), packed.size, _ptr(qrows), qrows.size, _ptr(lens), lens.size, out),
                         "mlst_debug_last_packed")
         return packed, qrows, lens, wpr, qs
+
+    def kernel_occupancy(self) -> dict:
+        out = (C.c_uint64 * 8)()
+        self._check(self.lib.mlst_debug_kernel_occupancy(self._h, out), "mlst_debug_kernel_occupancy")
+        keys = ("regs", "scratch_bytes", "lds_static", "lds_dynamic", "workgroups_per_cu", "threads", "grid", "one_wave")
+        return {k: int(v) for k, v in zip(keys, out)}
 
     def fasta_info(self) -> tuple[int, int, int, int]:
         out = (C.c_uint64 * 4)()
```
